# bayesml/BayesML

Hardware: AMD Instinct MI355X
Metric: GMM-VB E+M samples/sec at K=64,D=128,N=1e7; 1/2/4/8-GPU scaling (higher is better)
Workload: dtype f64; 1 GPU; GMM-VB K=64 D=128 N=10000000 rows/GPU x 1 GPU, x stored f32, one VB iteration per step (c3 of BASELINE.json configs); classes=64, degree=128, rows_per_gpu=10000000, rows_total=10000000, x_storage=f32, parallelism=rows1, row_tiles=1

## Files before the change

bayesml_amd/_engine.py:

```python
from __future__ import annotations

import ctypes
import os

import torch

_HERE = os.path.dirname(os.path.abspath(__file__))
LIB_PATH = os.environ.get("BAYESML_AMD_LIB") or os.path.join(_HERE, "csrc", "libgmmvb.so")

GMMVB_F32, GMMVB_F64 = 0, 1
POLICY_LEN = 16
_STATUS = {0: "GMMVB_OK", 1: "GMMVB_EINVAL", 2: "GMMVB_EUNSUPPORTED", 3: "GMMVB_EHIP", 4: "GMMVB_ENOMEM",
           5: "GMMVB_ESTATE"}

_vp, _i64, _int = ctypes.c_void_p, ctypes.c_int64, ctypes.c_int
SYMBOLS = {
    "gmmvb_abi_version": (_int, []),
    "gmmvb_last_error": (ctypes.c_char_p, []),
    "gmmvb_stats_len": (_i64, [_int, _int]),
    "gmmvb_workspace_create": (_int, [_int, _int, _int, _i64, ctypes.POINTER(_vp)]),
    "gmmvb_workspace_create_tile": (_int, [_vp, _i64, ctypes.POINTER(_vp)]),
    "gmmvb_workspace_destroy": (_int, [_vp]),
    "gmmvb_workspace_bytes": (_i64, [_vp]),
    "gmmvb_set_pivot": (_int, [_vp, _vp, _vp]),
    "gmmvb_set_params": (_int, [_vp, _vp, _vp, _vp, _vp]),
    "gmmvb_set_drift": (_int, [_vp, _vp, _vp, _vp, ctypes.c_double, _vp]),
    "gmmvb_forget": (_int, [_vp]),
    "gmmvb_regroup_count": (_i64, [_vp]),
    "gmmvb_debug_record": (_int, [_vp, _i64, ctypes.POINTER(ctypes.c_double)]),
    "gmmvb_debug_proof": (_int, [_vp, _int, _i64, _vp, _vp, _vp]),
    "gmmvb_wants_drift": (_int, [_vp, _i64]),
    "gmmvb_prepare_rows": (_int, [_vp, _vp, _i64, _i64, _vp]),
    "gmmvb_estep": (_int, [_vp, _vp, _i64, _i64, _vp]),
    "gmmvb_load_responsibilities": (_int, [_vp, _vp, _i64, _vp]),
    "gmmvb_mstep": (_int, [_vp, _vp, _i64, _i64, _vp, _vp]),
    "gmmvb_estep_mstep": (_int, [_vp, _vp, _i64, _i64, _vp, _vp]),
    "gmmvb_responsibilities": (_int, [_vp, _i64, _i64, _vp, _vp]),
    "gmmvb_ln_rho": (_int, [_vp, _i64, _i64, _vp, _vp]),
    "gmmvb_argmax": (_int, [_vp, _i64, _i64, _vp, _vp]),
    "gmmvb_last_launch_info": (ctypes.c_char_p, [_vp]),
    "gmmvb_pass_counts": (_int, [_vp, ctypes.POINTER(_i64)]),
    "gmmvb_kside_factor": (_int, [_int, _int, _vp, _vp, _vp, _vp, _vp]),
    "gmmvb_kside_step": (_int, [_int, _int, _vp, _vp, _vp, _vp, _vp, _vp, _vp, _vp, _vp, _int, _vp, _vp, _vp, _vp, _vp, _vp]),
    "gmmvb_kside_drift": (_int, [_int, _int, _vp, _vp, _vp, _vp, _vp, _vp, _int, _int, _vp, _vp, _vp, _vp, _vp]),
    "gmmvb_last_sparsity": (ctypes.c_int, [_vp, _vp, ctypes.POINTER(ctypes.c_double), ctypes.POINTER(ctypes.c_double)]),
    "gmmvb_last_work": (ctypes.c_int, [_vp, ctypes.POINTER(ctypes.c_double)]),
    "gmmvb_comm_unique_id": (_int, [_vp]),
    "gmmvb_comm_create": (_int, [_vp, _int, _int, ctypes.POINTER(_vp)]),
    "gmmvb_comm_destroy": (_int, [_vp]),
    "gmmvb_allreduce_stats": (_int, [_vp, _vp, _i64, _vp]),
    "gmmvb_stats_packed_len": (_i64, [_int, _int]),
    "gmmvb_stats_pack": (_int, [_int, _int, _vp, _vp, _vp]),
    "gmmvb_stats_unpack": (_int, [_int, _int, _vp, _vp, _vp]),
    "gmmvb_set_shard": (_int, [_vp, _i64, _int]),
    "gmmvb_policy_export": (_int, [_vp, _vp, _vp]),
    "gmmvb_policy_import": (_int, [_vp, _vp, _vp]),
    "gmmvb_small_supported": (_int, [_int, _int, _i64]),
    "gmmvb_small_out_len": (_i64, [_int, _int, _int]),
    "gmmvb_small_fit": (_int, [_int, _int, _int, _vp, _i64, _i64, _vp, _vp, _int, _int, _vp, _int, ctypes.c_double, _vp, _vp, _vp]),
    "hmmvb_kside_dirichlet": (_int, [_int, _vp, _vp, ctypes.c_double, ctypes.c_double] + [_vp] * 18),
    "hmmvb_out_len": (_i64, [_int]),
    "hmmvb_enable": (_int, [_vp]),
    "hmmvb_forward_backward": (_int, [_vp, _i64, _vp, _vp, _vp, _vp]),
    "hmmvb_debug_readout": (_int, [_vp, _int, _i64, _i64, _vp, _vp]),
    "hmmvb_readout": (_int, [_vp, _int, _i64, _i64, _vp, _vp, _vp]),
    "hmmvb_emission_target": (_int, [_vp, _int, _vp]),
    "hmmvb_skip_h": (_int, [_vp, _int]),
    "hmmvb_last_boundary_pass": (_int, [_vp]),
    "hmmvb_last_viterbi_pass": (_int, [_vp]),
    "hmmvb_viterbi": (_int, [_vp, _i64, _vp, _vp, _vp, _vp]),
    "gmmvb_profile_enable": (_int, [_vp, _int]),
    "gmmvb_profile_last_ms": (_int, [_vp, ctypes.POINTER(ctypes.c_float), ctypes.POINTER(ctypes.c_float)]),
    "gmmvb_profile_spans": (_int, [_vp, ctypes.POINTER(ctypes.c_float), ctypes.POINTER(_int)]),
    "gmmvb_profile_span_name": (ctypes.c_char_p, [_int]),
    "gmmvb_policy_calibrate": (_int, [_vp, _int]),
    "gmmvb_policy_table": (_int, [_vp, ctypes.POINTER(ctypes.c_double)]),
    "gmmvb_sample_latent": (_int, [_int, _vp, ctypes.c_uint64, _i64, _i64, _vp, _vp]),
    "gmmvb_sample_chain_work_bytes": (_i64, [_int, _i64]),
    "gmmvb_sample_chain": (_int, [_int, _vp, _vp, ctypes.c_uint64, _i64, _vp, _vp, _i64, _vp]),
    "gmmvb_sample_emissions_work_bytes": (_i64, [_int, _i64]),
    "gmmvb_sample_emissions": (_int, [_int, _int, _vp, _vp, _vp, ctypes.c_uint64, _i64, _i64, _int, _vp, _i64, _vp, _i64, _vp]),
}


class EngineUnavailableError(RuntimeError):
    """The HIP extension or the GPU is missing; the product path has no fallback."""


class EngineError(RuntimeError):
    """A C-ABI call returned a non-zero status."""


class EngineLimitError(ValueError):
    """The model's shape is outside what this version of the engine supports (the reference has no such limit)."""


MAX_MFMA_DEGREE = 128
MAX_HMM_FAST_CLASSES = 64
MAX_HMM_CLASSES = 16 * 255
MAX_DEGREE = 19200


def check_limits(c_degree: int, c_num_classes: int = 1, hmm: bool = False):
    if c_degree > MAX_DEGREE:
        raise EngineLimitError(f"bayesml_amd supports c_degree <= {MAX_DEGREE} in this version (got {c_degree}); "
                               "bayesml itself has no such limit")
    if hmm and c_num_classes > MAX_HMM_CLASSES:
        raise EngineLimitError(f"bayesml_amd.hiddenmarkovnormal supports c_num_classes <= {MAX_HMM_CLASSES} in this "
                               f"version (got {c_num_classes}); bayesml itself has no such limit")


_lib = None


def load_library(path: str = LIB_PATH) -> ctypes.CDLL:
    global _lib
    if _lib is not None and path == LIB_PATH:
        return _lib
    if not os.path.exists(path):
        raise EngineUnavailableError(
            f"{path} not found: build it with `python -c 'import __graft_entry__ as g; g.build()'` "
            "(or `make -C bayesml_amd/csrc`). bayesml_amd has no CPU fallback for the data pass.")
    lib = ctypes.CDLL(path)
    for name, (res, args) in SYMBOLS.items():
        fn = getattr(lib, name)
        fn.restype = res
        fn.argtypes = args
    if path == LIB_PATH:
        _lib = lib
    return lib


def _check(lib, rc, what):
    if rc != 0:
        msg = lib.gmmvb_last_error()
        raise EngineError(f"{what}: {_STATUS.get(rc, rc)}: {msg.decode() if msg else ''}")


def _f64(t: torch.Tensor, shape, device) -> torch.Tensor:
    t = torch.as_tensor(t, dtype=torch.float64, device=device).contiguous()
    if tuple(t.shape) != tuple(shape):
        raise ValueError(f"expected shape {tuple(shape)}, got {tuple(t.shape)}")
    return t


class RcclComm:

    def __init__(self, rank: int, world: int, device, bootstrap=None, group=None):
        self.lib = load_library()
        self.device = torch.device(device)
        buf = (ctypes.c_ubyte * 128)()
        if rank == 0:
            _check(self.lib, self.lib.gmmvb_comm_unique_id(buf), "gmmvb_comm_unique_id")
        if bootstrap is None:
            import torch.distributed as dist
            t = torch.tensor(list(buf), dtype=torch.uint8)
            if dist.get_backend(group) == "nccl":
                t = t.to(self.device)
            dist.broadcast(t, src=dist.get_global_rank(group, 0) if group is not None else 0, group=group)
            raw = bytes(t.cpu().tolist())
        else:
            raw = bootstrap(bytes(buf))
        buf = (ctypes.c_ubyte * 128).from_buffer_copy(raw)
        handle = _vp()
        with torch.cuda.device(self.device):
            _check(self.lib, self.lib.gmmvb_comm_create(buf, int(world), int(rank), ctypes.byref(handle)), "gmmvb_comm_create")
        self._comm = handle

    def all_reduce_(self, t: torch.Tensor) -> torch.Tensor:
        if t.dtype != torch.float64 or not t.is_contiguous() or t.device != self.device:
            raise ValueError("the statistics block must be a contiguous float64 tensor on the communicator's device")
        with torch.cuda.device(self.device):
            st = _vp(torch.cuda.current_stream(self.device).cuda_stream)
            _check(self.lib, self.lib.gmmvb_allreduce_stats(self._comm, t.data_ptr(), t.numel(), st), "gmmvb_allreduce_stats")
        return t

    def close(self):
        if getattr(self, "_comm", None):
            torch.cuda.synchronize(self.device)
            self.lib.gmmvb_comm_destroy(self._comm)
            self._comm = None

    def __del__(self):
# ... 109 lines not shown
                rc = self.lib.gmmvb_workspace_create_tile(tile_of._ws, self.max_rows, ctypes.byref(handle))
            else:
                rc = self.lib.gmmvb_workspace_create(self.K, self.D, GMMVB_F64 if x_dtype == torch.float64 else GMMVB_F32,
                                                     self.max_rows, ctypes.byref(handle))
        _check(self.lib, rc, "gmmvb_workspace_create_tile" if tile_of is not None else "gmmvb_workspace_create")
        self._ws = handle
        self.emission_fused = False
        self._keep = []

    def close(self):
        if getattr(self, "_ws", None):
            torch.cuda.synchronize(self.device)
            self.lib.gmmvb_workspace_destroy(self._ws)
            self._ws = None

    def __del__(self):
        try:
            self.close()
        except Exception:
            pass

    def _stream(self):
        return _vp(torch.cuda.current_stream(self.device).cuda_stream)

    def _x(self, x: torch.Tensor):
        if x.device != self.device or x.dtype != self.x_dtype or x.dim() != 2 or x.shape[1] != self.D:
            raise ValueError(f"x must be a [{'*'}, {self.D}] {self.x_dtype} tensor on {self.device}")
        if x.stride(1) != 1:
            x = x.contiguous()
        return x, int(x.stride(0)) if x.shape[0] > 1 else self.D

    @property
    def workspace_bytes(self) -> int:
        return int(self.lib.gmmvb_workspace_bytes(self._ws))

    @property
    def launch_info(self) -> str:
        s = self.lib.gmmvb_last_launch_info(self._ws)
        return s.decode() if s else ""

    PASS_NAMES = ("estep_dense", "estep_bound", "estep_carried", "estep_fell_back_dense", "estep_sweep",
                  "mstep_dense", "mstep_list", "estep_gather")

    def pass_counts(self) -> dict:
        out = (_i64 * 8)()
        _check(self.lib, self.lib.gmmvb_pass_counts(self._ws, out), "gmmvb_pass_counts")
        return dict(zip(self.PASS_NAMES, (int(v) for v in out)))

    def sparsity(self):
        a, e = ctypes.c_double(), ctypes.c_double()
        with torch.cuda.device(self.device):
            _check(self.lib, self.lib.gmmvb_last_sparsity(self._ws, self._stream(), ctypes.byref(a), ctypes.byref(e)),
                   "gmmvb_last_sparsity")
        return float(a.value), float(e.value)

    def work(self) -> dict:
        out = (ctypes.c_double * 8)()
        _check(self.lib, self.lib.gmmvb_last_work(self._ws, out), "gmmvb_last_work")
        tiles = (self.rows + 255) // 256 if getattr(self, "rows", 0) else 0
        share = float(out[6]) / (tiles * self.K) if out[6] >= 0 and tiles else -1.0
        return dict(active=float(out[0]), evaluated=float(out[1]), accumulated=float(out[2]), settled_rows=float(out[3]),
                    early_exits=float(out[4]), proof_pairs=float(out[5]), sweep_share=share, table_left=float(out[7]))

    def policy_table(self) -> dict:
        out = (ctypes.c_double * 16)()
        _check(self.lib, self.lib.gmmvb_policy_table(self._ws, out), "gmmvb_policy_table")
        keys = ("dense_e_ns", "dense_m_ns", "bound_ns", "exact_ns", "proof_ns", "list_m_ns", "literal_dense_e_ns",
                "literal_dense_m_ns", "literal_bound_ns", "prune_below", "dense_again_above", "list_m_below")
        d = {k: float(out[i]) for i, k in enumerate(keys)}
        d.update(measured=int(out[12]), discarded=int(out[13]), calibrating=bool(out[14]))
        return d

    def profile(self, on: bool = True):
        _check(self.lib, self.lib.gmmvb_profile_enable(self._ws, int(on)), "gmmvb_profile_enable")

    def last_kernel_ms(self):
        e, m = ctypes.c_float(), ctypes.c_float()
        _check(self.lib, self.lib.gmmvb_profile_last_ms(self._ws, ctypes.byref(e), ctypes.byref(m)),
               "gmmvb_profile_last_ms")
        return float(e.value), float(m.value)

    def kernel_spans(self) -> dict:
        ms, cnt = (ctypes.c_float * 8)(), (_int * 8)()
        _check(self.lib, self.lib.gmmvb_profile_spans(self._ws, ms, cnt), "gmmvb_profile_spans")
        out = {}
        for i in range(8):
            name = self.lib.gmmvb_profile_span_name(i).decode()
            if name and cnt[i]:
                out[name] = (float(ms[i]), int(cnt[i]))
        return out

    def set_pivot(self, pivot):
        p = _f64(pivot, (self.D,), self.device)
        with torch.cuda.device(self.device):
            _check(self.lib, self.lib.gmmvb_set_pivot(self._ws, p.data_ptr(), self._stream()), "gmmvb_set_pivot")
        self.pivot = p

    def prepare_rows(self, x: torch.Tensor):
        x, ldx = self._x(x)
        with torch.cuda.device(self.device):
            _check(self.lib, self.lib.gmmvb_prepare_rows(self._ws, x.data_ptr(), ldx, x.shape[0], self._stream()),
                   "gmmvb_prepare_rows")

    def set_params(self, c, m, u):
        c = _f64(c, (self.K,), self.device)
        m = _f64(m, (self.K, self.D), self.device)
        u = _f64(u, (self.K, self.D, self.D), self.device)
        with torch.cuda.device(self.device):
            _check(self.lib, self.lib.gmmvb_set_params(self._ws, c.data_ptr(), m.data_ptr(), u.data_ptr(),
                                                       self._stream()), "gmmvb_set_params")
        self._keep = [c, m, u]

    def set_shard(self, global_rows: int, n_ranks: int):
        _check(self.lib, self.lib.gmmvb_set_shard(self._ws, int(global_rows), int(n_ranks)), "gmmvb_set_shard")

    def policy_export(self, tail: torch.Tensor):
        with torch.cuda.device(self.device):
            _check(self.lib, self.lib.gmmvb_policy_export(self._ws, tail.data_ptr(), self._stream()), "gmmvb_policy_export")

    def policy_import(self, tail: torch.Tensor):
        with torch.cuda.device(self.device):
            _check(self.lib, self.lib.gmmvb_policy_import(self._ws, tail.data_ptr(), self._stream()), "gmmvb_policy_import")

    def wants_drift(self, n_rows: int) -> bool:
        return bool(self.lib.gmmvb_wants_drift(self._ws, int(n_rows)))

    def set_drift(self, gamma, delta, big_gamma, typical_gamma: float = -1.0):
        g = _f64(gamma, (self.K,), self.device)
        d = _f64(delta, (self.K,), self.device)
        G = _f64(big_gamma, (self.K,), self.device)
        with torch.cuda.device(self.device):
            _check(self.lib, self.lib.gmmvb_set_drift(self._ws, g.data_ptr(), d.data_ptr(), G.data_ptr(),
                                                      float(typical_gamma), self._stream()), "gmmvb_set_drift")

    @property
    def regroup_count(self) -> int:
        return int(self.lib.gmmvb_regroup_count(self._ws))

    def debug_record(self, row: int) -> dict:
        out = (ctypes.c_double * 26)()
        _check(self.lib, self.lib.gmmvb_debug_record(self._ws, int(row), out), "gmmvb_debug_record")
        v = list(out)
        return dict(k=[int(x) for x in v[:8]], d=[round(x, 3) for x in v[8:16]], B=v[16], exact=int(v[17]), sel=int(v[18]),
                    flags=int(v[19]), khat=int(v[20]), lse=v[21], masks=[int(x) for x in v[22:26]])

    def debug_proof(self, k: int, n_rows: int):
        ub = torch.empty(n_rows, dtype=torch.float32, device=self.device)
        lb = torch.empty(n_rows, dtype=torch.float64, device=self.device)
        with torch.cuda.device(self.device):
            _check(self.lib, self.lib.gmmvb_debug_proof(self._ws, int(k), int(n_rows), ub.data_ptr(), lb.data_ptr(),
                                                        self._stream()), "gmmvb_debug_proof")
        return ub, lb

    def forget(self):
        _check(self.lib, self.lib.gmmvb_forget(self._ws), "gmmvb_forget")

    def estep(self, x: torch.Tensor):
        x, ldx = self._x(x)
        with torch.cuda.device(self.device):
            _check(self.lib, self.lib.gmmvb_estep(self._ws, x.data_ptr(), ldx, x.shape[0], self._stream()),
                   "gmmvb_estep")
        self.rows = x.shape[0]

    def load_responsibilities(self, r: torch.Tensor):
        r = torch.as_tensor(r, dtype=torch.float64, device=self.device).contiguous()
        if r.dim() != 2 or r.shape[1] != self.K:
            raise ValueError("r must be [n, K]")
        with torch.cuda.device(self.device):
            _check(self.lib, self.lib.gmmvb_load_responsibilities(self._ws, r.data_ptr(), r.shape[0], self._stream()),
                   "gmmvb_load_responsibilities")
        self.rows = r.shape[0]
        self._keep.append(r)

    def _stats_out(self, out):
        if out is None:
            return torch.empty(self.stats_len, dtype=torch.float64, device=self.device)
        if out.dtype != torch.float64 or out.numel() != self.stats_len or not out.is_contiguous() or out.device != self.device:
            raise ValueError("out must be a contiguous float64 tensor of stats_len elements on the engine's device")
        return out

    def mstep(self, x: torch.Tensor, out: torch.Tensor = None) -> torch.Tensor:
        x, ldx = self._x(x)
        stats = self._stats_out(out)
        with torch.cuda.device(self.device):
            _check(self.lib, self.lib.gmmvb_mstep(self._ws, x.data_ptr(), ldx, x.shape[0], stats.data_ptr(),
                                                  self._stream()), "gmmvb_mstep")
        return stats

    def estep_mstep(self, x: torch.Tensor, out: torch.Tensor = None) -> torch.Tensor:
        x, ldx = self._x(x)
        stats = self._stats_out(out)
        with torch.cuda.device(self.device):
            _check(self.lib, self.lib.gmmvb_estep_mstep(self._ws, x.data_ptr(), ldx, x.shape[0], stats.data_ptr(),
                                                        self._stream()), "gmmvb_estep_mstep")
        self.rows = x.shape[0]
        return stats

    def enable_hmm(self):
        with torch.cuda.device(self.device):
            _check(self.lib, self.lib.hmmvb_enable(self._ws), "hmmvb_enable")

    def hmm_skip_h(self, skip: bool = True):
        _check(self.lib, self.lib.hmmvb_skip_h(self._ws, 1 if skip else 0), "hmmvb_skip_h")

    def last_boundary_pass(self) -> int:
        return int(self.lib.hmmvb_last_boundary_pass(self._ws))

    def last_viterbi_pass(self) -> int:
        return int(self.lib.hmmvb_last_viterbi_pass(self._ws))

    def emission_target(self, fused: bool) -> bool:
        eff = ctypes.c_int(0)
        _check(self.lib, self.lib.hmmvb_emission_target(self._ws, 1 if fused else 0, ctypes.byref(eff)),
               "hmmvb_emission_target")
        self.emission_fused = bool(eff.value)
        return self.emission_fused

    def forward_backward(self, pi_tilde, a_tilde, out: torch.Tensor = None):
        K = self.K
        pi = _f64(pi_tilde, (K,), self.device)
        a = _f64(a_tilde, (K, K), self.device)
        n_out = int(self.lib.hmmvb_out_len(K))
        if out is None:
            out = torch.empty(n_out, dtype=torch.float64, device=self.device)
        elif out.dtype != torch.float64 or out.numel() != n_out or not out.is_contiguous() or out.device != self.device:
            raise ValueError("out must be a contiguous float64 tensor of hmmvb_out_len(K) elements on the engine's device")
        with torch.cuda.device(self.device):
            _check(self.lib, self.lib.hmmvb_forward_backward(self._ws, self.rows, pi.data_ptr(), a.data_ptr(),
                                                             out.data_ptr(), self._stream()), "hmmvb_forward_backward")
        self._keep = self._keep[-3:] + [pi, a]
        return out[:K * K].view(K, K), out[K * K:K * K + K], out[K * K + K:K * K + 2 * K], out[K * K + 2 * K]

    def viterbi(self, ln_pi_tilde, ln_a_tilde) -> torch.Tensor:
        K = self.K
        pi = _f64(ln_pi_tilde, (K,), self.device)
        a = _f64(ln_a_tilde, (K, K), self.device)
        z = torch.empty(self.rows, dtype=torch.int32, device=self.device)
        with torch.cuda.device(self.device):
            _check(self.lib, self.lib.hmmvb_viterbi(self._ws, self.rows, pi.data_ptr(), a.data_ptr(), z.data_ptr(),
                                                    self._stream()), "hmmvb_viterbi")
        torch.cuda.current_stream(self.device).synchronize()
        return z

    def hmm_readout(self, what: str, row0=0, n=None, a_tilde=None) -> torch.Tensor:
        code = {"alpha": 0, "beta": 1, "xi": 3}[what]
        n = self.rows - row0 if n is None else n
        K = self.K
        out = torch.empty((n, K, K) if code == 3 else (n, K), dtype=torch.float64, device=self.device)
        a = _f64(a_tilde, (K, K), self.device) if code == 3 else None
        with torch.cuda.device(self.device):
            _check(self.lib, self.lib.hmmvb_readout(self._ws, code, row0, n, a.data_ptr() if a is not None else None,
                                                    out.data_ptr(), self._stream()), "hmmvb_readout")
        if a is not None:
            torch.cuda.current_stream(self.device).synchronize()
        return out

    def hmm_debug(self, what, row0=0, n=None):
        n = self.rows - row0 if n is None else n
        Kp = 16 * ((self.K + 15) // 16)
        out = torch.empty((n, Kp) if what == 0 else (n,), dtype=torch.float64, device=self.device)
        with torch.cuda.device(self.device):
            _check(self.lib, self.lib.hmmvb_debug_readout(self._ws, what, row0, n, out.data_ptr(), self._stream()),
                   "hmmvb_debug_readout")
        if what == 0:
            pos = [(s & ~15) + 4 * ((s & 15) & 3) + ((s & 15) >> 2) for s in range(self.K)]
            out = out[:, pos]
        return out

    def split_stats(self, stats: torch.Tensor):
        K, D = self.K, self.D
        return (stats[:K], stats[K:2 * K], stats[2 * K:2 * K + K * D].view(K, D),
                stats[2 * K + K * D:].view(K, D, D))

    def _readout(self, fn, name, row0, n, dtype=torch.float64, cols=None):
        n = self.rows - row0 if n is None else n
        out = torch.empty((n, self.K) if cols is None else (n,), dtype=dtype, device=self.device)
        with torch.cuda.device(self.device):
            _check(self.lib, fn(self._ws, row0, n, out.data_ptr(), self._stream()), name)
        return out

    def responsibilities(self, row0=0, n=None) -> torch.Tensor:
        return self._readout(self.lib.gmmvb_responsibilities, "gmmvb_responsibilities", row0, n)

    def ln_rho(self, row0=0, n=None) -> torch.Tensor:
        return self._readout(self.lib.gmmvb_ln_rho, "gmmvb_ln_rho", row0, n)

    def argmax(self, row0=0, n=None) -> torch.Tensor:
        return self._readout(self.lib.gmmvb_argmax, "gmmvb_argmax", row0, n, dtype=torch.int32, cols=1)


class TiledDataPass:

    def __init__(self, K, D, x_dtype, n_rows, device, tile_rows, resident=False):
        self.K, self.D, self.x_dtype, self.max_rows = int(K), int(D), x_dtype, int(n_rows)
        self.tile_rows = int(min(tile_rows, n_rows))
        self.n_tiles = (self.max_rows + self.tile_rows - 1) // self.tile_rows
        self.resident = bool(resident)
        self.inner = DataPass(K, D, x_dtype, self.tile_rows, device)
        self.tiles = [self.inner]
        self.device, self.lib, self.stats_len = self.inner.device, self.inner.lib, self.inner.stats_len
        try:
            if self.resident:
                for t in range(1, self.n_tiles):
                    lo, hi = self._tile(t)
                    self.tiles.append(DataPass(K, D, x_dtype, hi - lo, device, tile_of=self.inner))
            self._tmp = torch.zeros(self.stats_len, dtype=torch.float64, device=self.device)
# ... 302 lines not shown
```

bayesml_amd/csrc/aux_kernels.h:

```cpp
#pragma once
#include "common.h"
#include "rec_common.h"

namespace gmmvb {

static __device__ __forceinline__ void pack_f64_image(const double* uk, int ld, const double* mk, int D, int T, int img_len,
                                                      double* __restrict__ im) {
    const int P = tri_pairs(T);
    for (int e = threadIdx.x; e < P * 256; e += blockDim.x) {
        const int p = e >> 8, h = (e >> 7) & 1, lane = (e >> 1) & 63, ee = e & 1;
        int jt = 0;
        while (tri_pairs(jt + 1) <= p) ++jt;
        const int b = p - tri_pairs(jt);
        const int jj = 16 * jt + (lane & 15), ii = 16 * b + 4 * (lane >> 4) + 2 * h + ee;
        im[e] = (jj < D && ii < D && ii <= jj) ? uk[(int64_t)jj * ld + ii] : 0.0;
    }
    for (int jj = threadIdx.x; jj < 16 * T; jj += blockDim.x) {
        double s = 0.0;
        if (jj < D)
            for (int ii = 0; ii <= jj; ++ii) s = fma(uk[(int64_t)jj * ld + ii], mk[ii], s);
        const int jt = jj >> 4, w = jj & 15, g = w & 3, r = w >> 2;
        im[P * 256 + (jt * 4 + g) * 4 + r] = -s;
    }
    for (int e = P * 256 + 16 * T + threadIdx.x; e < img_len; e += blockDim.x) im[e] = 0.0;
// ... 10 lines not shown
    pack_f64_image(u + (int64_t)k * D * D, D, m + (int64_t)k * D, D, T, img_len, img + (int64_t)k * img_len);
}

template <typename XT>
__global__ void center_rows_kernel(const XT* __restrict__ x, int64_t ldx, int64_t n_rows, int64_t pad_rows, int D,
                                   int Dp, const double* __restrict__ pivot, double* __restrict__ xc) {
    const int64_t e = (int64_t)blockIdx.x * blockDim.x + threadIdx.x;
    if (e >= pad_rows * Dp) return;
    const int64_t n = e / Dp;
    const int f = (int)(e - n * Dp);
    xc[e] = (n < n_rows && f < D) ? (double)x[n * ldx + f] - pivot[f] : 0.0;
}

constexpr int kLseRows = 1024;
static __global__ __launch_bounds__(256) void row_lse_kernel(const double* __restrict__ lnrho, int64_t npad, int64_t n_rows,
                                                      int K, double* __restrict__ lse, double* __restrict__ dpart,
                                                      double* __restrict__ apart, int stride) {
    __shared__ double wmax[4];
    __shared__ int wcnt[4];
    int active = 0;
    const int64_t base = (int64_t)blockIdx.x * stride * kLseRows + threadIdx.x;
    double l[4];
#pragma unroll
    for (int q = 0; q < 4; ++q) {
        const int64_t n = base + 256 * q;
        l[q] = 0.0;
        if (n >= n_rows) continue;
        double mx = lnrho[n], s = 1.0;
        for (int k = 1; k < K; ++k) {
            const double v = lnrho[(int64_t)k * npad + n];
            if (v > mx) {
                s = fma(s, exp(mx - v), 1.0);
                mx = v;
            } else {
                s += exp(v - mx);
            }
        }
        l[q] = mx + log(s);
        lse[n] = l[q];
    }
    if (!dpart) return;
    const double ninf = -__builtin_huge_val();
    for (int k = 0; k < K; ++k) {
        double d = ninf;
#pragma unroll
        for (int q = 0; q < 4; ++q) {
            const int64_t n = base + 256 * q;
            if (n < n_rows) {
                const double v = lnrho[(int64_t)k * npad + n] - l[q];
                d = (v > d || v != v) ? v : d;
                active += !(v < -kRelevanceNats);
            }
        }
#pragma unroll
        for (int o = 32; o > 0; o >>= 1) {
            const double v = __shfl_xor(d, o);
            d = (v > d || v != v) ? v : d;
        }
        if ((threadIdx.x & 63) == 0) wmax[threadIdx.x >> 6] = d;
        __syncthreads();
        if (threadIdx.x == 0) {
#pragma unroll
            for (int w = 1; w < 4; ++w) d = (wmax[w] > d || wmax[w] != wmax[w]) ? wmax[w] : d;
            dpart[(int64_t)blockIdx.x * K + k] = d;
        }
        __syncthreads();
    }
#pragma unroll
    for (int o = 32; o > 0; o >>= 1) active += __shfl_xor(active, o);
    if ((threadIdx.x & 63) == 0) wcnt[threadIdx.x >> 6] = active;
    __syncthreads();
    if (threadIdx.x == 0 && apart) apart[blockIdx.x] = (double)(wcnt[0] + wcnt[1] + wcnt[2] + wcnt[3]);
}

static __global__ __launch_bounds__(256) void thr_kernel(const double* __restrict__ dpart, const double* __restrict__ apart,
                                                  int blocks, int K, double* __restrict__ thr,
                                                  double* __restrict__ act_total) {
    __shared__ double part[256];
    const int k = blockIdx.x;
    if (k == K) {
        if (!apart) return;
        double a = 0.0;
        for (int b = threadIdx.x; b < blocks; b += 256) a += apart[b];
        part[threadIdx.x] = a;
        __syncthreads();
        if (threadIdx.x == 0) {
            double t = 0.0;
            for (int i = 0; i < 256; ++i) t += part[i];
            *act_total = t;
        }
        return;
    }
    if (!dpart) return;
    double d = -__builtin_huge_val();
    for (int b = threadIdx.x; b < blocks; b += 256) {
        const double v = dpart[(int64_t)b * K + k];
        d = (v > d || v != v) ? v : d;
    }
    part[threadIdx.x] = d;
    __syncthreads();
    if (threadIdx.x == 0) {
        for (int i = 1; i < 256; ++i) d = (part[i] > d || part[i] != part[i]) ? part[i] : d;
        thr[k] = d - kRelevanceNats;
    }
}

template <int MODE>
__global__ __launch_bounds__(kSelRows) void select_mask_kernel(const double* __restrict__ u, int64_t npad, int64_t n_rows,
                                                               int K, int* __restrict__ khat,
                                                               unsigned long long* __restrict__ masks ,
                                                               int* __restrict__ blk_cnt ) {
    static_assert(MODE == 0 || MODE == 3, "only the best-component modes exist");
    __shared__ int wcnt[4][256];
    const int64_t n = (int64_t)blockIdx.x * kSelRows + threadIdx.x;
    const bool valid = n < n_rows;
    const int W = (K + 63) / 64;
    const int wave = threadIdx.x >> 6;
    for (int k = threadIdx.x & 63; k < K; k += 64) wcnt[wave][k] = 0;
    int kh = -1;
    if (MODE == 3 && valid) kh = khat[n];
    if (MODE == 0) {
        int arg = 0;
        if (valid) {
            double best = u[n];
            for (int k = 1; k < K; ++k) {
                const double v = u[(int64_t)k * npad + n];
                const bool up = v > best;
                best = up ? v : best;
                arg = up ? k : arg;
            }
            khat[n] = arg;
        }
        kh = arg;
    }
    for (int w = 0; w < W; ++w) {
        unsigned long long mk = 0;
        if (valid) {
            if ((kh >> 6) == w) mk = 1ull << (kh & 63);
            masks[(int64_t)w * npad + n] = mk;
        }
        unsigned long long present = wave_or(mk);
        while (present) {
            const int b = __builtin_ctzll(present);
            present &= present - 1;
            const int c = __builtin_popcountll(__ballot((mk >> b) & 1ull));
            if ((threadIdx.x & 63) == 0) wcnt[wave][64 * w + b] = c;
        }
    }
    __syncthreads();
    for (int k = threadIdx.x; k < K; k += kSelRows)
        blk_cnt[blk_at(k, blockIdx.x, K)] = wcnt[0][k] + wcnt[1][k] + wcnt[2][k] + wcnt[3][k];
}

constexpr int kScanParts = 1024;
constexpr int kScanChunk = 32;

static __global__ __launch_bounds__(256) void scan_parts_kernel(const int* __restrict__ blk, int blocks, int K, int* __restrict__ parts) {
    __shared__ int sh[256];
    const int p = blockIdx.x;
    const int R = K <= 256 ? 256 / K : 1;
    const int t = threadIdx.x, k = t % K, r = t / K;
    const int per = (blocks + kScanParts - 1) / kScanParts;
    const int b0 = p * per, b1 = b0 + per < blocks ? b0 + per : blocks;
    int s = 0;
    if (t < R * K)
        for (int b = b0 + r; b < b1; b += R) s += blk[blk_at(k, b, K)];
    sh[t] = s;
    __syncthreads();
    if (t < K) {
        int tot = 0;
        for (int q = 0; q < R; ++q) tot += sh[q * K + t];
        parts[p * K + t] = tot;
    }
}

static __global__ __launch_bounds__(256) void scan_mid_kernel(int* __restrict__ parts, int K, int* __restrict__ counts) {
    static_assert(kScanParts == 32 * kScanChunk, "256 threads = 8 components x 32 chunks");
    __shared__ int sh[32][8];
    const int t = threadIdx.x, kk = t & 7, c = t >> 3;
    const int k = blockIdx.x * 8 + kk;
    int v[kScanChunk];
    int s = 0;
#pragma unroll
    for (int i = 0; i < kScanChunk; ++i) {
        v[i] = k < K ? parts[(int64_t)(c * kScanChunk + i) * K + k] : 0;
        s += v[i];
    }
    sh[c][kk] = s;
    __syncthreads();
    int run = 0;
    for (int q = 0; q < c; ++q) run += sh[q][kk];
    if (k < K) {
#pragma unroll
        for (int i = 0; i < kScanChunk; ++i) {
            parts[(int64_t)(c * kScanChunk + i) * K + k] = run;
            run += v[i];
        }
        if (c == 31) counts[k] = run;
    }
}

static __global__ __launch_bounds__(256) void scan_apply_kernel(int* __restrict__ blk, int blocks, int K, const int* __restrict__ parts) {
    __shared__ int sh[256];
    const int p = blockIdx.x;
    const int R = K <= 256 ? 256 / K : 1;
    const int t = threadIdx.x, k = t % K, r = t / K;
    const bool on = t < R * K;
    const int per = (blocks + kScanParts - 1) / kScanParts;
    const int b0 = p * per, b1 = b0 + per < blocks ? b0 + per : blocks;
    int run = on ? parts[p * K + k] : 0;
    if (R == 1) {
        for (int c0 = b0; c0 < b1; c0 += 8) {
            int v[8];
#pragma unroll
            for (int i = 0; i < 8; ++i) v[i] = (on && c0 + i < b1) ? blk[blk_at(k, c0 + i, K)] : 0;
#pragma unroll
            for (int i = 0; i < 8; ++i) {
                if (on && c0 + i < b1) blk[blk_at(k, c0 + i, K)] = run;
                run += v[i];
            }
        }
        return;
    }
    for (int c0 = b0; c0 < b1; c0 += R) {
        const int b = c0 + r;
        const int v = (on && b < b1) ? blk[blk_at(k, b, K)] : 0;
        __syncthreads();
        sh[t] = v;
        __syncthreads();
        if (on) {
            int before = 0, all = 0;
            for (int q = 0; q < R; ++q) {
                const int w = sh[q * K + k];
                before += q < r ? w : 0;
                all += w;
            }
            if (b < b1) blk[blk_at(k, b, K)] = run + before;
            run += all;
        }
    }
}

inline void launch_scan_counts(hipStream_t st, int* blk, int blocks, int K, int* counts, int* parts ) {
    hipLaunchKernelGGL(scan_parts_kernel, dim3(kScanParts), dim3(256), 0, st, blk, blocks, K, parts);
    hipLaunchKernelGGL(scan_mid_kernel, dim3((K + 7) / 8), dim3(256), 0, st, parts, K, counts);
    hipLaunchKernelGGL(scan_apply_kernel, dim3(kScanParts), dim3(256), 0, st, blk, blocks, K, parts);
}

static __global__ __launch_bounds__(kSelRows) void fill_lists_kernel(const unsigned long long* __restrict__ masks, int64_t npad,
                                                              int64_t n_rows, int K, const int* __restrict__ blk_base,
                                                              int* __restrict__ lists, int64_t cap,
                                                              unsigned char* __restrict__ lock = nullptr,
                                                              const unsigned char* __restrict__ lcomp = nullptr,
                                                              const double* __restrict__ block_total = nullptr
                                                              ) {
    if (block_total != nullptr && block_total[blockIdx.x] == 0.0) return;
    __shared__ int wcnt[4][256];
    const int64_t n = (int64_t)blockIdx.x * kSelRows + threadIdx.x;
    const bool valid = n < n_rows;
    const int W = (K + 63) / 64;
    const int wave = threadIdx.x >> 6, lane = threadIdx.x & 63;
    for (int k = lane; k < K; k += 64) wcnt[wave][k] = 0;
    const int base_pre = (int)threadIdx.x < K ? blk_base[blk_at((int)threadIdx.x, blockIdx.x, K)] : 0;
    unsigned long long mkw[4] = {0ull, 0ull, 0ull, 0ull}, prw[4] = {0ull, 0ull, 0ull, 0ull};
#pragma unroll
    for (int w = 0; w < 4; ++w) {
        if (w >= W) break;
        const unsigned long long mk = valid ? masks[(int64_t)w * npad + n] : 0ull;
        mkw[w] = mk;
        unsigned long long present = wave_or(mk);
        prw[w] = present;
        while (present) {
            const int b = __builtin_ctzll(present);
            present &= present - 1;
            const int c = __builtin_popcountll(__ballot((mk >> b) & 1ull));
            if (lane == 0) wcnt[wave][64 * w + b] = c;
        }
    }
    __syncthreads();
    for (int k = threadIdx.x; k < K; k += kSelRows) {
        const int c0 = wcnt[0][k], c1 = wcnt[1][k], c2 = wcnt[2][k], c3 = wcnt[3][k];
        if (c0 + c1 + c2 + c3 > 0) {
            const int base = k == (int)threadIdx.x ? base_pre : blk_base[blk_at(k, blockIdx.x, K)];
            wcnt[0][k] = base;
            wcnt[1][k] = base + c0;
            wcnt[2][k] = base + c0 + c1;
            wcnt[3][k] = base + c0 + c1 + c2;
        }
    }
    __syncthreads();
    const unsigned lk0 = (lock && valid) ? lock[n] : 0u;
    const int kh0 = (lock && valid) ? (int)lcomp[n] : 0;
    if (lk0 >= 2u) lock[n] = lk0 == 2u ? 0 : 1;
#pragma unroll
    for (int w = 0; w < 4; ++w) {
        if (w >= W) break;
        const unsigned long long mk = mkw[w];
        unsigned long long present = prw[w];
        while (present) {
            const int b = __builtin_ctzll(present);
            present &= present - 1;
            const int k = 64 * w + b;
            const unsigned long long bal = __ballot((mk >> b) & 1ull);
            const int off = wcnt[wave][k];
            if ((mk >> b) & 1ull) {
                int entry = (int)n;
                if (lock) {
                    const bool leaves = lk0 == 2u || (lk0 == 4u && kh0 != k);
                    entry = leaves ? (int)((unsigned)entry | 0x80000000u) : entry;
                }
                lists[(int64_t)k * cap + off + __builtin_popcountll(bal & ((1ull << lane) - 1ull))] = entry;
            }
        }
    }
}

static __global__ __launch_bounds__(kSelRows) void lse_mask_kernel(const double* __restrict__ lnrho, int64_t npad, int64_t n_rows,
                                                            int K, const double* __restrict__ thr, double* __restrict__ lse,
                                                            unsigned long long* __restrict__ masks,
                                                            int* __restrict__ blk_cnt, double* __restrict__ apart,
                                                            int* __restrict__ khat ) {
    __shared__ int wcnt[4][256];
    __shared__ int wact[4];
    const int64_t n = (int64_t)blockIdx.x * kSelRows + threadIdx.x;
    const bool valid = n < n_rows;
    const int W = (K + 63) / 64;
    const int wave = threadIdx.x >> 6;
    for (int k = threadIdx.x & 63; k < K; k += 64) wcnt[wave][k] = 0;
    double l = 0.0;
    if (valid) {
        double mx = lnrho[n], s = 1.0;
        int arg = 0;
        for (int k = 1; k < K; ++k) {
            const double v = lnrho[(int64_t)k * npad + n];
            if (v > mx) {
                s = fma(s, exp(mx - v), 1.0);
                mx = v;
                arg = k;
            } else {
                s += exp(v - mx);
            }
        }
        l = mx + log(s);
        lse[n] = l;
        if (khat) khat[n] = arg;
    }
    int active = 0;
    for (int w = 0; w < W; ++w) {
        unsigned long long mk = 0;
        if (valid) {
            const int kend = K - 64 * w < 64 ? K - 64 * w : 64;
            for (int b = 0; b < kend; ++b) {
                const double t = lnrho[(int64_t)(64 * w + b) * npad + n] - l;
                mk |= (unsigned long long)(!(t < thr[64 * w + b])) << b;
                active += !(t < -kRelevanceNats);
            }
            masks[(int64_t)w * npad + n] = mk;
        }
        unsigned long long present = wave_or(mk);
        while (present) {
            const int b = __builtin_ctzll(present);
            present &= present - 1;
            const int c = __builtin_popcountll(__ballot((mk >> b) & 1ull));
            if ((threadIdx.x & 63) == 0) wcnt[wave][64 * w + b] = c;
        }
    }
#pragma unroll
    for (int o = 32; o > 0; o >>= 1) active += __shfl_xor(active, o);
    if ((threadIdx.x & 63) == 0) wact[wave] = active;
    __syncthreads();
    for (int k = threadIdx.x; k < K; k += kSelRows)
        blk_cnt[blk_at(k, blockIdx.x, K)] = wcnt[0][k] + wcnt[1][k] + wcnt[2][k] + wcnt[3][k];
    if (threadIdx.x == 0) apart[blockIdx.x] = (double)(wact[0] + wact[1] + wact[2] + wact[3]);
}

static __global__ void load_r_kernel(const double* __restrict__ r, int64_t n_rows, int K, double* __restrict__ buf,
                              int64_t npad, double* __restrict__ lse, const int* __restrict__ iperm) {
    const int64_t n = (int64_t)blockIdx.x * blockDim.x + threadIdx.x;
    if (n >= n_rows) return;
    const int64_t m = iperm ? iperm[n] : n;
    for (int k = 0; k < K; ++k) buf[(int64_t)k * npad + m] = r[n * K + k];
    lse[m] = 0.0;
}

static __global__ void readout_kernel(const double* __restrict__ buf, const double* __restrict__ lse, int64_t npad,
                               int64_t row0, int64_t n_rows, int K, int mode, int direct_r,
                               double* __restrict__ out, const int* __restrict__ iperm) {
    const int64_t e = (int64_t)blockIdx.x * blockDim.x + threadIdx.x;
    if (e >= n_rows * K) return;
    const int64_t n = e / K;
    const int k = (int)(e - n * K);
    const int64_t m = iperm ? iperm[row0 + n] : row0 + n;
    const double v = buf[(int64_t)k * npad + m];
    out[e] = (mode == 0 || direct_r) ? v : exp(v - lse[m]);
}

static __global__ void gather_int_kernel(const int* __restrict__ src, int64_t row0, int64_t n_rows, const int* __restrict__ iperm,
                                  int32_t* __restrict__ z) {
    const int64_t n = (int64_t)blockIdx.x * blockDim.x + threadIdx.x;
    if (n < n_rows) z[n] = src[iperm ? iperm[row0 + n] : row0 + n];
}

static __global__ void argmax_kernel(const double* __restrict__ buf, int64_t npad, int64_t row0, int64_t n_rows, int K,
                              int32_t* __restrict__ z, const int* __restrict__ iperm) {
    const int64_t n = (int64_t)blockIdx.x * blockDim.x + threadIdx.x;
    if (n >= n_rows) return;
    const int64_t m = iperm ? iperm[row0 + n] : row0 + n;
    double best = buf[m];
    int arg = 0;
    for (int k = 1; k < K; ++k) {
        const double v = buf[(int64_t)k * npad + m];
        if (v > best) {
            best = v;
            arg = k;
        }
    }
    z[n] = arg;
}

static __global__ void reduce_stats_kernel(const double* __restrict__ slabs, int S, int K, int D, int T,
                                    double* __restrict__ stats) {
    const int k = blockIdx.y;
    const int e = blockIdx.x * blockDim.x + threadIdx.x;
    const int P = tri_pairs(T);
    const int L = slab_len(T);
    if (e >= P * 256 + 16 * T + 2) return;
    double v = 0.0;
    int s = 0;
    for (; s + 16 <= S; s += 16) {
        double t[16];
#pragma unroll
        for (int u = 0; u < 16; ++u) t[u] = slabs[((int64_t)(s + u) * K + k) * L + e];
#pragma unroll
        for (int u = 0; u < 16; ++u) v += t[u];
    }
    for (; s < S; ++s) v += slabs[((int64_t)s * K + k) * L + e];
    double* ns = stats;
    double* h = stats + K;
    double* a = stats + 2 * (int64_t)K;
    double* B = a + (int64_t)K * D;
    if (e < P * 256) {
        const int p = e >> 8, r = (e >> 6) & 3, lane = e & 63;
        int t2 = 0;
        while (tri_pairs(t2 + 1) <= p) ++t2;
        const int t1 = p - tri_pairs(t2);
        const int col = lane & 15, row = (lane >> 4) + 4 * r;
        const int f1 = T * row + t1, f2 = T * col + t2;
        if (f1 >= D || f2 >= D) return;
        if (t1 == t2 && row > col) return;
        B[((int64_t)k * D + f1) * D + f2] = v;
        B[((int64_t)k * D + f2) * D + f1] = v;
    } else if (e < P * 256 + 16 * T) {
        const int f = e - P * 256;
        if (f < D) a[(int64_t)k * D + f] = v;
    } else if (e == P * 256 + 16 * T) {
        ns[k] = v;
    } else {
        h[k] = v;
    }
}

static __global__ void reduce_chunks_kernel(const double* __restrict__ slabs, const int* __restrict__ plan, int K, int D, int T,
                                     double* __restrict__ stats, int accumulate = 0, const double* __restrict__ add = nullptr,
                                     const int* __restrict__ counts = nullptr, int runs = 0) {
// ... 140 lines not shown
```

bayesml_amd/csrc/capi.hip:

```cpp
#include "capi_internal.h"

namespace {
thread_local std::string g_err;
}

namespace gmmvb {
int fail(int code, const char* what, hipError_t e) {
    g_err = what;
    if (e != hipSuccess) {
        g_err += ": ";
        g_err += hipGetErrorString(e);
    }
    return code;
}
}

namespace {
KernelSizes kernel_sizes(int K, int D) {
    KernelSizes ks;
    ks.max_tiles = kMaxTiles;
    ks.t1_splits = GMMVB_T1_SPLITS;
    ks.sel_rows = kSelRows;
    ks.lse_rows = kLseRows;
    ks.scan_parts = kScanParts;
// ... 153 lines not shown
            hipError_t rc = hipEventCreate(&e);
            if (rc != hipSuccess) return fail(GMMVB_EHIP, "hipEventCreate", rc);
        }
        for (auto& e : ws->span_ev) {
            hipError_t rc = hipEventCreate(&e);
            if (rc != hipSuccess) return fail(GMMVB_EHIP, "hipEventCreate", rc);
        }
    }
    ws->prof = on != 0;
    ws->prof_light = on == 2;
    ws->span_open = false;
    ws->ev_e = ws->ev_m = false;
    ws->n_spans = 0;
    return GMMVB_OK;
}

const char* gmmvb_profile_span_name(int slot) { return (slot >= 0 && slot < kSpanSlots) ? kSpanNames[slot] : ""; }

int gmmvb_profile_spans(gmmvb_workspace* ws, float* ms , int* launches ) {
    if (!ws || !ms || !launches) return fail(GMMVB_EINVAL, "null argument");
    for (int i = 0; i < kSpanSlots; ++i) {
        ms[i] = 0.0f;
        launches[i] = 0;
    }
    for (int i = 0; i < ws->n_spans; ++i) {
        float t = 0.0f;
        hipError_t rc = hipEventSynchronize(ws->span_ev[2 * i + 1]);
        if (rc == hipSuccess) rc = hipEventElapsedTime(&t, ws->span_ev[2 * i], ws->span_ev[2 * i + 1]);
        if (rc != hipSuccess) return fail(GMMVB_EHIP, "event timing (span)", rc);
        ms[ws->span_slot[i]] += t;
        ++launches[ws->span_slot[i]];
    }
    return GMMVB_OK;
}

int gmmvb_profile_last_ms(gmmvb_workspace* ws, float* estep_ms, float* mstep_ms) {
    if (!ws || !estep_ms || !mstep_ms) return fail(GMMVB_EINVAL, "null argument");
    *estep_ms = *mstep_ms = -1.0f;
    if (ws->ev_e) {
        hipError_t rc = hipEventSynchronize(ws->ev[1]);
        if (rc == hipSuccess) rc = hipEventElapsedTime(estep_ms, ws->ev[0], ws->ev[1]);
        if (rc != hipSuccess) return fail(GMMVB_EHIP, "event timing (estep)", rc);
    }
    if (ws->ev_m) {
        hipError_t rc = hipEventSynchronize(ws->ev[3]);
        if (rc == hipSuccess) rc = hipEventElapsedTime(mstep_ms, ws->ev[2], ws->ev[3]);
        if (rc != hipSuccess) return fail(GMMVB_EHIP, "event timing (mstep)", rc);
    }
    return GMMVB_OK;
}

int gmmvb_set_pivot(gmmvb_workspace* ws, const double* pivot_dev, void* stream) {
    if (!ws || !pivot_dev) return fail(GMMVB_EINVAL, "null argument");
    hipError_t e = hipMemcpyAsync(ws->pivot, pivot_dev, (size_t)ws->D * sizeof(double), hipMemcpyDeviceToDevice,
                                  (hipStream_t)stream);
    if (e != hipSuccess) return fail(GMMVB_EHIP, "hipMemcpyAsync(pivot)", e);
    ws->xc_src = nullptr;
    ws->xq_src = nullptr;
    ++ws->pivot_gen;
    drop_settled_rows(ws);
    return GMMVB_OK;
}

int gmmvb_wants_drift(const gmmvb_workspace* ws, int64_t n_rows) {
    if (!ws || ws->prune == 0 || ws->estep_variant != kEstepLds8 || ws->hmm != nullptr || !ws->rec_k) return 0;
    if (ws->opt_carry_off) return 0;
    if (ws->sharded) n_rows = ws->shard_rows / ws->shard_ranks;
    return (ws->prune == 2 || n_rows * (int64_t)ws->K >= (int64_t(1) << 23)) ? 1 : 0;
}

namespace {
__global__ void set_drift_kernel(const double* __restrict__ gamma, const double* __restrict__ delta, const double* __restrict__ big_gamma,
                                 const double* __restrict__ cvec, int K, double* __restrict__ drift) {
    const int k = blockIdx.x * blockDim.x + threadIdx.x;
    if (k >= K) return;
    drift[k] = gamma[k];
    drift[K + k] = delta[k];
    drift[2 * K + k] = cvec[k];
    drift[3 * K + k] = big_gamma[k];
}
}

int gmmvb_set_drift(gmmvb_workspace* ws, const double* gamma_dev, const double* delta_dev, const double* big_gamma_dev,
                    double typical_gamma, void* stream) {
    if (!ws || !gamma_dev || !delta_dev || !big_gamma_dev) return fail(GMMVB_EINVAL, "null argument");
    ws->typical_gamma = typical_gamma;
    hipStream_t st = (hipStream_t)stream;
    hipLaunchKernelGGL(set_drift_kernel, dim3((unsigned)((ws->K + 255) / 256)), dim3(256), 0, st, gamma_dev, delta_dev, big_gamma_dev,
                       ws->cvec, ws->K, ws->drift);
    const hipError_t e = hipGetLastError();
    if (e != hipSuccess) return fail(GMMVB_EHIP, "set_drift_kernel", e);
    ws->have_drift = ws->have_params && ws->params_used;
    return GMMVB_OK;
}

int gmmvb_debug_record(gmmvb_workspace* ws, int64_t row, double* out ) {
    if (!ws || !out || !ws->rec_k || row < 0 || row >= ws->npad) return fail(GMMVB_EINVAL, "bad argument");
    hipError_t e = hipDeviceSynchronize();
    auto get = [&e](void* dst, const void* src, size_t n) {
        if (e == hipSuccess) e = hipMemcpy(dst, src, n, hipMemcpyDeviceToHost);
    };
    for (int j = 0; j < kRecSlots; ++j) {
        unsigned short k = 0;
        float d = 0.0f;
        get(&k, ws->rec_k + (int64_t)j * ws->npad + row, sizeof(k));
        get(&d, ws->rec_d + (int64_t)j * ws->npad + row, sizeof(d));
        out[j] = k == kRecEmpty ? -1.0 : (double)k;
        out[8 + j] = d;
    }
    float B = 0.0f;
    unsigned char ex = 0, sel = 0, fl = 0;
    int kh = 0;
    get(&B, ws->rec_B + row, sizeof(B));
    get(&ex, ws->rec_exact + row, 1);
    get(&sel, ws->rec_sel + row, 1);
    get(&fl, ws->rec_flags + row, 1);
    get(&kh, ws->khat + row, sizeof(kh));
    get(out + 21, ws->lse + row, sizeof(double));
    out[16] = B;
    out[17] = ex;
    out[18] = sel;
    out[19] = fl;
    out[20] = kh;
    for (int w = 0; w < 4; ++w) {
        unsigned long long m = 0;
        if (w < (ws->K + 63) / 64) get(&m, ws->masks + (int64_t)w * ws->npad + row, sizeof(m));
        out[22 + w] = (double)m;
    }
    if (e != hipSuccess) return fail(GMMVB_EHIP, "reading a record back", e);
    return GMMVB_OK;
}

int64_t gmmvb_regroup_count(const gmmvb_workspace* ws) { return ws ? ws->sorts : -1; }

namespace {
__global__ void debug_all_rows_kernel(int* __restrict__ list, int* __restrict__ counts, int K, int k, int64_t n_rows) {
    const int64_t i = (int64_t)blockIdx.x * blockDim.x + threadIdx.x;
    if (i < n_rows) list[i] = (int)i;
    if (i < K) counts[i] = (int)(i == k ? n_rows : 0);
}
}

int gmmvb_debug_proof(gmmvb_workspace* ws, int k, int64_t n_rows, float* ub_dev, double* lb_dev, void* stream) {
    if (!ws || !ub_dev || !lb_dev || k < 0 || k >= ws->K) return fail(GMMVB_EINVAL, "bad argument");
    if (!ws->xq || !ws->img_i8b || ws->xq_src == nullptr || ws->xq_rows != n_rows || ws->xq_gen != ws->img_gen || !ws->have_params)
        return fail(GMMVB_ESTATE, "no digit planes for these rows: gmmvb_set_pivot, gmmvb_prepare_rows, gmmvb_set_params first");
    claim_scratch(ws);
    hipStream_t st = (hipStream_t)stream;
    ws->tmeta_valid = false;
    drop_settled_rows(ws);
    const unsigned grid = (unsigned)((std::max<int64_t>(n_rows, ws->K) + 255) / 256);
    hipLaunchKernelGGL(debug_all_rows_kernel, dim3(grid), dim3(256), 0, st, ws->lists + (int64_t)k * ws->npad, ws->counts, ws->K, k,
                       n_rows);
    hipLaunchKernelGGL(gather_plan_kernel, dim3(1), dim3(64), 0, st, ws->counts, ws->K, estep_i8_pairs_per_chunk(), ws->plan);
    hipError_t e = launch_estep_i8_proof(ws->D, ws->num_cu, st, ws->xq, ws->xqe, ws->img_i8b, ws->cvec, ws->K, ws->lists, ws->npad,
                                         ws->counts, ws->plan, ws->ub32, ws->lnrho, ws->npad);
    if (e == hipSuccess) e = hipMemcpyAsync(ub_dev, ws->ub32 + (int64_t)k * ws->npad, (size_t)n_rows * sizeof(float),
                                            hipMemcpyDeviceToDevice, st);
    if (e == hipSuccess) e = hipMemcpyAsync(lb_dev, ws->lnrho + (int64_t)k * ws->npad, (size_t)n_rows * sizeof(double),
                                            hipMemcpyDeviceToDevice, st);
    if (e != hipSuccess) return fail(GMMVB_EHIP, "proof kernel (diagnostic)", e);
    ws->e_state = 0;
    ws->lost_estep = false;
    ws->bounds_rows = 0;
    ws->rec_valid = ws->dense_valid = ws->rec_live = false;
    ws->active_lists = ws->blk_fresh = false;
    ws->lag.valid = false;
    return GMMVB_OK;
}

int gmmvb_forget(gmmvb_workspace* ws) {
    if (!ws) return fail(GMMVB_EINVAL, "null argument");
    ws->forget = true;
    ws->have_drift = false;
    drop_settled_rows(ws);
    return GMMVB_OK;
}

int gmmvb_set_params(gmmvb_workspace* ws, const double* c_dev, const double* m_dev, const double* u_dev,
                     void* stream) {
    if (!ws || !c_dev || !m_dev || !u_dev) return fail(GMMVB_EINVAL, "null argument");
    hipStream_t st = (hipStream_t)stream;
    hipError_t e = hipSuccess;
    if (ws->generic) {
        e = hipMemcpyAsync(ws->cvec, c_dev, (size_t)ws->K * sizeof(double), hipMemcpyDeviceToDevice, st);
        if (e != hipSuccess) return fail(GMMVB_EHIP, "hipMemcpyAsync(c)", e);
        e = hipMemcpyAsync(ws->gen_m, m_dev, (size_t)ws->K * ws->D * sizeof(double), hipMemcpyDeviceToDevice, st);
        if (e == hipSuccess)
            e = hipMemcpyAsync(ws->gen_u, u_dev, (size_t)ws->K * ws->D * ws->D * sizeof(double), hipMemcpyDeviceToDevice, st);
        if (e != hipSuccess) return fail(GMMVB_EHIP, "hipMemcpyAsync(m, u)", e);
        ws->have_params = true;
        ws->params_used = false;
        return GMMVB_OK;
    }
    if (ws->wide) {
        if (ws->pivot_i8) return fail(GMMVB_EUNSUPPORTED, "gmmvb_set_params: int8 images past D = 128");
        hipLaunchKernelGGL(pack_params_kernel, dim3(ws->K), dim3(256), 0, st, u_dev, m_dev, ws->K, ws->D, ws->T, ws->img_len, ws->img,
                           c_dev, ws->cvec, nullptr, nullptr);
        e = hipGetLastError();
        if (e != hipSuccess) return fail(GMMVB_EHIP, "pack_params_kernel", e);
    } else {
        e = launch_pack_images(u_dev, m_dev, c_dev, ws->pivot, ws->K, ws->D, ws->T, ws->img_len, ws->img, ws->cvec, ws->pivot_i8,
                               ws->pivot_i8 ? ws->img_i8 : nullptr, ws->pivot_i8 ? ws->img_i8b : nullptr, st);
        if (e != hipSuccess) return fail(GMMVB_EHIP, "pack_images_kernel", e);
        if (ws->pivot_i8) ws->img_gen = ws->pivot_gen;
    }
    if (ws->tri) {
        e = launch_pack_tri16(u_dev, m_dev, ws->K, ws->D, ws->tri, st);
        if (e != hipSuccess) return fail(GMMVB_EHIP, "pack_tri16_kernel", e);
    }
    ws->proj_table = false;
    if (ws->gimg && ws->opt_project != 0 && ws->sorted && ws->tile_ref_valid && ws->have_drift && ws->xq_gen == ws->pivot_gen &&
        !ws->opt_carry_off) {
        e = launch_proj_table(u_dev, m_dev, c_dev, ws->pivot, ws->K, ws->D, ws->gimg, ws->gconst, st);
        if (e != hipSuccess) return fail(GMMVB_EHIP, "proj_table_kernel", e);
        ws->proj_table = true;
    }
    ws->have_params = true;
    ws->params_used = false;
    return GMMVB_OK;
}

int fetch_counters(gmmvb_workspace* ws) {
    if (ws->ctr_pending) {
        hipError_t e = hipEventSynchronize(ws->ctr_ev);
        if (e != hipSuccess) return fail(GMMVB_EHIP, "waiting for the E-step counters", e);
        ws->lag.act = ws->ctr_host[0];
        if (ws->pend_mode == 0) {
            ws->lag.eval = (double)ws->pend_rows * ws->K;
            ws->lag.over = 0.0;
            ws->lag.settled = 0.0;
            ws->lag.listed = ws->lag.accum = ws->lag.act;
            ws->lag.exits = 0.0;
            ws->lag.cols = -1.0;
            ws->lag.left = -1.0;
            ws->lag_quiet = ws->lag_skipped = -1.0;
            ws->lag.proof = 0.0;
            ws->lag.moved = 0.0;
        } else {
            ws->lag.proof = ws->ctr_host[7];
            ws->lag.exits = (ws->exit_host && ws->gather_exit) ? (double)ws->exit_host[0] : 0.0;
            ws->lag.cols = (ws->exit_host && ws->pend_lazy) ? (double)ws->exit_host[1] : -1.0;
            ws->lag.left = (ws->exit_host && ws->pend_proj) ? (double)ws->exit_host[2] : -1.0;
            ws->lag_quiet = (ws->exit_host && ws->pend_quiet) ? (double)(ws->exit_host[3] & 0xFFFFFFFFull) : -1.0;
            ws->lag_skipped = (ws->exit_host && ws->pend_quiet) ? (double)(ws->exit_host[3] >> 32) : -1.0;
            ws->lag.settled = ws->ctr_host[4];
            ws->lag.listed = ws->ctr_host[5];
            ws->lag.accum = ws->ctr_host[6];
            ws->lag.eval = ws->ctr_host[1] + ((ws->pend_mode == 1 || ws->pend_mode == 3) ? ws->pend_round0 : 0.0);
            ws->lag.over = ws->ctr_host[2];
            ws->lag.moved = ws->ctr_host[3];
            if (!ws->sharded && ws->sorted && !ws->pend_first_sorted) ws->moved_since_sort += ws->lag.moved;
        }
        ws->lag.rows = (double)ws->pend_rows;
        ws->lag.mode = ws->pend_mode;
        ws->lag.valid = true;
        ws->ctr_pending = false;
    }
    return GMMVB_OK;
}

void poll_counters(gmmvb_workspace* ws) {
    if (ws->ctr_pending && hipEventQuery(ws->ctr_ev) == hipSuccess) (void)fetch_counters(ws);
}

namespace {
__global__ void policy_export_kernel(const double* __restrict__ ctr, const unsigned long long* __restrict__ exits, int mode,
                                     double rows, int K, double round0, int counted, int use_exits, double* __restrict__ out) {
    if (threadIdx.x != 0 || blockIdx.x != 0) return;
    const bool dense = mode == 0;
    const double act = counted ? ctr[0] : 0.0;
    out[0] = act;
    out[1] = dense ? rows * K : ctr[1] + ((mode == 1 || mode == 3) ? round0 : 0.0);
    out[2] = dense ? 0.0 : ctr[2];
    out[3] = dense ? 0.0 : ctr[3];
    out[4] = dense ? 0.0 : ctr[4];
    out[5] = dense ? act : ctr[5];
    out[6] = dense ? act : ctr[6];
    out[7] = dense ? 0.0 : ctr[7];
    out[8] = (dense || !use_exits || !exits) ? 0.0 : (double)*exits;
    out[9] = rows;
    out[10] = 1.0;
    out[11] = counted ? 1.0 : 0.0;
    out[12] = (double)mode;
    for (int i = 13; i < GMMVB_POLICY_LEN; ++i) out[i] = 0.0;
}
}

int gmmvb_set_shard(gmmvb_workspace* ws, int64_t global_rows, int n_ranks) {
    if (!ws || global_rows < 1 || n_ranks < 1) return fail(GMMVB_EINVAL, "bad argument");
    ws->sharded = n_ranks > 1;
    ws->shard_rows = global_rows;
    ws->shard_ranks = n_ranks;
    ws->pol.valid = false;
    if (ws->sharded && !ws->pol_host) {
        hipError_t e = hipHostMalloc((void**)&ws->pol_host, GMMVB_POLICY_LEN * sizeof(double), hipHostMallocDefault);
        if (e == hipSuccess) e = hipEventCreateWithFlags(&ws->pol_ev, hipEventDisableTiming);
        if (e != hipSuccess) return fail(GMMVB_EHIP, "policy buffers", e);
    }
    return GMMVB_OK;
}

int gmmvb_policy_export(gmmvb_workspace* ws, double* out_dev, void* stream) {
    if (!ws || !out_dev) return fail(GMMVB_EINVAL, "null argument");
    if (ws->e_state != 1) return fail(GMMVB_ESTATE, "no E-step output in the workspace");
    hipLaunchKernelGGL(policy_export_kernel, dim3(1), dim3(64), 0, (hipStream_t)stream, ws->ctr, ws->exit_ctr, ws->prev_pass,
                       (double)ws->e_rows, ws->K, ws->pend_round0, ws->exp_counted ? 1 : 0, ws->gather_exit ? 1 : 0, out_dev);
    hipError_t e = hipGetLastError();
    if (e != hipSuccess) return fail(GMMVB_EHIP, "policy export", e);
    return GMMVB_OK;
}

int gmmvb_policy_import(gmmvb_workspace* ws, const double* in_dev, void* stream) {
    if (!ws || !in_dev) return fail(GMMVB_EINVAL, "null argument");
    if (!ws->sharded) return GMMVB_OK;
    hipStream_t st = (hipStream_t)stream;
    hipError_t e = hipMemcpyAsync(ws->pol_host, in_dev, GMMVB_POLICY_LEN * sizeof(double), hipMemcpyDeviceToHost, st);
    if (e == hipSuccess) e = hipEventRecord(ws->pol_ev, st);
    if (e != hipSuccess) return fail(GMMVB_EHIP, "policy import", e);
    ws->pol_pending = true;
    ws->pol_mode = ws->prev_pass;
// ... 148 lines not shown
```

bayesml_amd/csrc/capi_estep.hip:

```cpp
#include "capi_internal.h"

namespace {

struct Pass {
    gmmvb_workspace* ws;
    const void* x_dev;
    int64_t ldx, n_rows;
    hipStream_t st;
    int is64;
    bool vec;
    int sel_grid;
    double pairs;
    EstepArgs a{};
    EstepI8Args a8{};
    RecArrays rec{};
    bool i8 = false;
    bool prunable = false;
    bool prev_lists = false, can_project = false, own_known = false, tmeta_was_valid = false;
    bool quiet_was_valid = false;
    int mode = kPassDense;
    bool settle = false, proof_capable = false;
    double skip_margin = -1.0;
    bool counted = false, proof_ran = false, tmeta_kept = false, projected = false, filtered = false, emission_to_hmm = false,
         sorted_now = false;
    bool quiet_swept = false;
    bool phase_closed = false;
    const char* name = "";
    int rpw = 0;
    int64_t grid = 0;

    PassFacts facts();
    int apply(const PassFacts& f, const PassPlan& plan);
    int run_generic();
    int run_dense();
    int run_bound();
    int run_sweep();
    int run_sweep_over_lists();
    int run_sweep_from_best();
    int sweep_bounds(bool proof, bool own_round);
    int run_candidates();
    int finish(const char* latch_what);
};

hipError_t regroup_rows(gmmvb_workspace* ws, const void* x_dev, int64_t ldx, int64_t n_rows, hipStream_t st, bool keep_state,
                        bool margin_ok) {
    const int sel_grid = (int)((n_rows + kSelRows - 1) / kSelRows);
    const unsigned cgrid = (unsigned)((n_rows + 255) / 256);
    const int* key = ws->khat;
    const int* perm_in = ws->sorted ? ws->perm : nullptr;
    const bool by_margin = ws->opt_regroup_margin && margin_ok && ws->K >= kMarginBuckets;
    if (by_margin) {
        int* bucket = ws->perm_tmp;
        hipLaunchKernelGGL(margin_bucket_kernel, dim3(cgrid), dim3(256), 0, st, ws->lnrho, ws->npad, n_rows, ws->lse, ws->khat,
                           keep_state ? ws->lock : nullptr, bucket);
        hipLaunchKernelGGL(select_mask_kernel<3>, dim3(sel_grid), dim3(kSelRows), 0, st, ws->lnrho, ws->npad, n_rows,
                           kMarginBuckets, bucket, ws->masks, ws->blk);
        scan_and_fill(ws, st, ws->masks, ws->blk, sel_grid, n_rows, kMarginBuckets);
        int* key1 = reinterpret_cast<int*>(ws->rec_d);
        hipLaunchKernelGGL(perm_compose_kernel, dim3(cgrid, kMarginBuckets), dim3(256), 0, st, ws->lists, ws->npad, ws->counts,
                           ws->khat, key1);
        hipLaunchKernelGGL(perm_compose_kernel, dim3(cgrid, kMarginBuckets), dim3(256), 0, st, ws->lists, ws->npad, ws->counts,
                           perm_in, ws->perm_tmp);
        key = key1;
        perm_in = ws->perm_tmp;
    }
    hipLaunchKernelGGL(select_mask_kernel<3>, dim3(sel_grid), dim3(kSelRows), 0, st, ws->lnrho, ws->npad, n_rows, ws->K,
                       const_cast<int*>(key), ws->masks, ws->blk);
    scan_and_fill(ws, st, ws->masks, ws->blk, sel_grid, n_rows, ws->K);
    ws->tile_ref_valid = false;
    if (ws->tile_ref) {
        if (launch_proj_tile_ref(ws->counts, ws->K, sel_grid, ws->tile_ref, st) == hipSuccess) ws->tile_ref_valid = true;
    }
    if (by_margin) {
        hipLaunchKernelGGL(perm_compose_kernel, dim3(cgrid, ws->K), dim3(256), 0, st, ws->lists, ws->npad, ws->counts, perm_in,
                           ws->khat);
        int* new_perm = ws->khat;
        ws->khat = ws->perm_tmp;
        ws->perm_tmp = ws->perm;
        ws->perm = new_perm;
    } else {
        hipLaunchKernelGGL(perm_compose_kernel, dim3(cgrid, ws->K), dim3(256), 0, st, ws->lists, ws->npad, ws->counts, perm_in,
                           ws->perm_tmp);
        std::swap(ws->perm, ws->perm_tmp);
    }
    if (keep_state) {
        hipLaunchKernelGGL(regroup_state_kernel, dim3((unsigned)((n_rows + 255) / 256)), dim3(256), 0, st, ws->perm,
                           ws->sorted ? ws->iperm : nullptr, n_rows, ws->lock, ws->lcomp, ws->dlock, ws->rec_sel, ws->rec_flags,
                           ws->rthr);
        std::swap(ws->lock, ws->rec_sel);
        std::swap(ws->lcomp, ws->rec_flags);
        std::swap(ws->dlock, ws->rthr);
    }
    hipLaunchKernelGGL(perm_invert_kernel, dim3((unsigned)((n_rows + 255) / 256)), dim3(256), 0, st, ws->perm, n_rows, ws->iperm);
    const int64_t total = n_rows * ws->D;
    const unsigned pg = (unsigned)((total + 255) / 256);
    const int64_t esz = ws->x_dtype == GMMVB_F64 ? 8 : 4;
    if ((ws->D * esz) % 16 == 0 && (ldx * esz) % 16 == 0 && (uintptr_t)x_dev % 16 == 0) {
        const int p16 = (int)(ws->D * esz / 16);
        hipLaunchKernelGGL(permute_rows16_kernel, dim3((unsigned)((n_rows * p16 + 255) / 256)), dim3(256), 0, st,
                           (const uint4*)x_dev, ldx * esz / 16, n_rows, p16, ws->perm, (uint4*)ws->xp);
    } else if (ws->x_dtype == GMMVB_F64)
        hipLaunchKernelGGL(permute_rows_kernel<double>, dim3(pg), dim3(256), 0, st, (const double*)x_dev, ldx, n_rows, ws->D,
                           ws->perm, (double*)ws->xp);
    else
        hipLaunchKernelGGL(permute_rows_kernel<float>, dim3(pg), dim3(256), 0, st, (const float*)x_dev, ldx, n_rows, ws->D,
                           ws->perm, (float*)ws->xp);
    ws->xc_stale = ws->xc != nullptr;
    if (ws->xq && ws->xq_src == x_dev) {
        hipError_t eq = launch_x_digits(ws->xp, ws->x_dtype == GMMVB_F64, ws->D, n_rows, ws->D, ws->pivot, ws->xq, ws->xqe, st);
        if (eq != hipSuccess) return eq;
        ws->xq_gen = ws->pivot_gen;
    }
    ws->sorted = true;
    ++ws->sorts;
    return hipGetLastError();
}

hipError_t launch_bound_pass(gmmvb_workspace* ws, const EstepI8Args& a8, int is64, bool vec, hipStream_t st,
                             const char** name, int* rpw_out, int64_t* grid_out) {
    const int rpw = estep_i8_rows_per_wg();
    int64_t grid = (a8.n_rows + rpw - 1) / rpw;
    if (grid > (1 << 20)) grid = 1 << 20;
    *rpw_out = rpw;
    *grid_out = grid;
    EstepI8Args ab = a8;
    ab.img = ws->img_i8b;
    ab.khat = ws->khat;
    ab.ub = ws->ub32;
    return launch_estep_i8_bound(is64, vec, ws->bound.tb, (int)grid, st, ab, name);
}

hipError_t lists_and_gather(gmmvb_workspace* ws, const EstepArgs& a, int is64, bool vec, int sel_grid, hipStream_t st,
                            const float* thr = nullptr, const double* block_total = nullptr ) {
    if (thr) {
        hipError_t em = hipMemsetAsync(ws->exit_ctr, 0, sizeof(unsigned long long), st);
        if (em != hipSuccess) return em;
    }
    span_begin(ws, kSpanSelect, st);
    scan_and_fill(ws, st, ws->masks, ws->blk, sel_grid, a.n_rows, ws->K, block_total);
    hipLaunchKernelGGL(gather_plan_kernel, dim3(1), dim3(64), 0, st, ws->counts, ws->K,
                       estep_gather_rows_per_wg(ws->T, is64), ws->plan);
    hipError_t e = hipGetLastError();
    span_end(ws, st);
    if (e != hipSuccess) return e;
    span_begin(ws, kSpanGather, st);
    e = launch_estep_gather_dev(ws->T, is64, vec, 2 * ws->num_cu, st, a, ws->lists, ws->npad, ws->counts, ws->plan, thr,
                                thr ? ws->exit_ctr : nullptr, 0.0f);
    span_end(ws, st);
    ++ws->passes[7];
    return e;
}

}

extern "C" {


bool cal_wanted(gmmvb_workspace* ws, int what, double pairs) {
    return ws->opt_calibrate && ws->cal_ev[0] != nullptr && !((ws->pt.measured >> what) & 1) && ws->cal_pairs[what] == 0.0 &&
           pairs >= (double)(int64_t(1) << 23) && ws->hmm == nullptr;
}
void cal_mark(gmmvb_workspace* ws, int what, double pairs, hipStream_t st) {
    note_hip(ws, hipEventRecord(ws->cal_ev[2 * what + 1], st));
    ws->cal_pairs[what] = pairs;
}
void cal_poll(gmmvb_workspace* ws) {
    for (int what = 0; what < 3; ++what) {
        if (ws->cal_pairs[what] <= 0.0 || hipEventQuery(ws->cal_ev[2 * what + 1]) != hipSuccess) continue;
        float ms = 0.0f;
        if (hipEventElapsedTime(&ms, ws->cal_ev[2 * what], ws->cal_ev[2 * what + 1]) == hipSuccess) {
            double ns = (double)ms * 1e6 / ws->cal_pairs[what];
            if (what == 2) ns += 0.010 * tri_pairs(ws->T) / 36.0;
            const bool took = ws->pt.take(what, ns);
            if (ws->opt_debug)
                std::fprintf(stderr, "[gmmvb] policy table: %s %.4f ns per pair %s (prune below %.3f, dense again above %.3f, list M below %.3f)\n",
                             what == 0 ? "dense E" : (what == 1 ? "dense M" : "bound pass"), ns, took ? "taken" : "out of range: literal kept",
                             ws->pt.prune_below(), ws->pt.dense_again_above(), ws->pt.list_m_below());
            if (!took) ws->pt.measured |= 8 << what;
            ws->cal_pairs[what] = (took || ++ws->cal_tries[what] >= 3) ? -1.0 : 0.0;
        } else {
            ws->cal_pairs[what] = -1.0;
        }
    }
}

}

namespace {

hipError_t proof_round(gmmvb_workspace* ws, hipStream_t st, const int* blk_base, int sel_grid, int64_t n_rows, float* ub) {
    if (ws->opt_proof_blocked && ws->slabs &&
        estep_i8_proof_work_bytes(ws->K, n_rows) <= ws->scratch->bytes[kBuf_slabs])
        return launch_estep_i8_proof_blocked(ws->D, ws->num_cu, st, ws->xq, ws->xqe, ws->img_i8b, ws->cvec, ws->K, ws->lists,
                                             ws->npad, ws->counts, blk_base, sel_grid, ws->slabs, ub, ws->lnrho, ws->npad);
    hipLaunchKernelGGL(gather_plan_kernel, dim3(1), dim3(64), 0, st, ws->counts, ws->K, estep_i8_pairs_per_chunk(), ws->plan);
    return launch_estep_i8_proof(ws->D, ws->num_cu, st, ws->xq, ws->xqe, ws->img_i8b, ws->cvec, ws->K, ws->lists, ws->npad,
                                 ws->counts, ws->plan, ub, ws->lnrho, ws->npad);
}

int Pass::run_generic() {
    const int R = generic_rows(ws->D);
    const dim3 g((unsigned)((n_rows + R - 1) / R), (unsigned)ws->K);
    const size_t lds = (size_t)ws->D * R * sizeof(double);
    span_begin(ws, kSpanEstepMain, st);
    if (is64)
        hipLaunchKernelGGL(estep_generic_kernel<double>, g, dim3(64), lds, st, (const double*)x_dev, ldx, n_rows, ws->D,
                           ws->gen_u, ws->gen_m, ws->cvec, R, ws->lnrho, ws->npad);
    else
        hipLaunchKernelGGL(estep_generic_kernel<float>, g, dim3(64), lds, st, (const float*)x_dev, ldx, n_rows, ws->D,
                           ws->gen_u, ws->gen_m, ws->cvec, R, ws->lnrho, ws->npad);
    span_end(ws, st);
    if (phase_events(ws)) {
        note_hip(ws, hipEventRecord(ws->ev[1], st));
        ws->ev_e = true;
    }
    phase_closed = true;
    span_begin(ws, kSpanLse, st);
    hipLaunchKernelGGL(row_lse_kernel, dim3((unsigned)((n_rows + kLseRows - 1) / kLseRows)), dim3(256), 0, st, ws->lnrho,
                       ws->npad, n_rows, ws->K, ws->lse, nullptr, nullptr, 1);
    span_end(ws, st);
    hipError_t eg = hipGetLastError();
    if (eg != hipSuccess) return fail(GMMVB_EHIP, "estep_generic launch", eg);
    ++ws->passes[0];
    ws->rec_live = ws->rec_valid = false;
    ws->evaluated = pairs;
    std::snprintf(ws->info, sizeof(ws->info), "estep_generic_f64<D=%d> grid=%ux%ux64 rows/workgroup=%d", ws->D, g.x, g.y, R);
    name = nullptr;
    return GMMVB_OK;
}

int Pass::run_dense() {
    const bool valu16 = ws->estep_variant == kEstepValu16 && ws->tri != nullptr;
    emission_to_hmm = ws->T == 1 && !ws->wide && !i8 && !ws->sorted && hmm_fused_emission(ws->hmm);
    rpw = ws->wide ? estep_rows_rows_per_wg()
                     : (i8 ? estep_i8_rows_per_wg() : (valu16 ? estep_rows16_rows_per_wg() : estep_rows_per_wg(ws->estep_variant, ws->T, is64)));
    grid = (n_rows + rpw - 1) / rpw;
    if (grid > (1 << 20)) grid = 1 << 20;
    span_begin(ws, kSpanEstepMain, st);
    const bool cal_e = !ws->wide && !i8 && !emission_to_hmm && !valu16 && cal_wanted(ws, 0, pairs);
    if (cal_e) note_hip(ws, hipEventRecord(ws->cal_ev[0], st));
    hipError_t e = ws->wide ? launch_estep_rows(ws->T, is64, (int)grid, st, a, &name)
                            : (i8 ? launch_estep_i8(is64, vec, (int)grid, st, a8, &name)
                                  : (emission_to_hmm ? hmm_launch_emission16(ws->hmm, is64, vec, st, a, &name)
                                     : (valu16 ? launch_estep_rows16(is64, vec, (int)grid, st, a, ws->tri, &name)
                                            : launch_estep(ws->estep_variant, ws->T, is64, vec, (int)grid, st, a, &name))));
    if (cal_e) cal_mark(ws, 0, pairs, st);
    span_end(ws, st);
    if (e != hipSuccess) return fail(GMMVB_EHIP, "estep launch", e);
    ++ws->passes[0];
    const int lse_blocks = (int)((n_rows + kLseRows - 1) / kLseRows);
    const bool count_pairs = ws->sparse && ws->masks && ws->hmm == nullptr && n_rows * (int64_t)ws->K >= (int64_t(1) << 18);
    span_begin(ws, kSpanLse, st);
    if (count_pairs) {
        const int stride = lse_blocks >= 64 ? 16 : 1;
        const int sampled = (lse_blocks + stride - 1) / stride;
        hipLaunchKernelGGL(row_lse_kernel, dim3((unsigned)sampled), dim3(256), 0, st, ws->lnrho, ws->npad, n_rows, ws->K,
                           ws->lse, ws->dpart, nullptr, stride);
        hipLaunchKernelGGL(thr_kernel, dim3((unsigned)ws->K), dim3(256), 0, st, ws->dpart, nullptr, sampled, ws->K, ws->thr,
                           ws->ctr);
        hipLaunchKernelGGL(lse_mask_kernel, dim3((unsigned)sel_grid), dim3(kSelRows), 0, st, ws->lnrho, ws->npad, n_rows,
                           ws->K, ws->thr, ws->lse, ws->masks, ws->blk, ws->apart, ws->khat);
        hipLaunchKernelGGL(sum_parts_kernel, dim3(1), dim3(1024), 0, st, ws->apart, nullptr, nullptr, nullptr, nullptr, nullptr,
                           nullptr, nullptr, sel_grid, ws->ctr);
        if (prunable)
            hipLaunchKernelGGL(rec_build_kernel<false>, dim3((unsigned)((n_rows + 255) / 256)), dim3(256), 0, st, ws->lnrho,
                               ws->npad, n_rows, ws->K, ws->cvec, nullptr, rec, ws->ub32);
        e = hipGetLastError();
        if (e != hipSuccess) return fail(GMMVB_EHIP, "row_lse / lse_mask launch", e);
        counted = true;
        ws->rec_valid = prunable;
    } else if (ws->hmm != nullptr) {
        ws->lse_stale = true;
        ws->rec_valid = false;
    } else {
        hipLaunchKernelGGL(row_lse_kernel, dim3((unsigned)lse_blocks), dim3(256), 0, st, ws->lnrho, ws->npad, n_rows, ws->K,
                           ws->lse, nullptr, nullptr, 1);
        e = hipGetLastError();
        if (e != hipSuccess) return fail(GMMVB_EHIP, "row_lse launch", e);
        ws->rec_valid = false;
    }
    span_end(ws, st);
    ws->rec_live = false;
    ws->evaluated = pairs;
    return GMMVB_OK;
}

int Pass::run_bound() {
    span_begin(ws, kSpanEstepMain, st);
    const bool cal_b = ws->bound.tb == (ws->D + 31) / 32 && cal_wanted(ws, 2, pairs);
    if (cal_b) note_hip(ws, hipEventRecord(ws->cal_ev[4], st));
    hipError_t e = launch_bound_pass(ws, a8, is64, vec, st, &name, &rpw, &grid);
    if (cal_b) cal_mark(ws, 2, pairs, st);
    span_end(ws, st);
    if (e != hipSuccess) return fail(GMMVB_EHIP, "estep_bound launch", e);
    ++ws->passes[1];
    span_begin(ws, kSpanSelect, st);
    hipLaunchKernelGGL(select_mask_kernel<3>, dim3(sel_grid), dim3(kSelRows), 0, st, ws->lnrho, ws->npad, n_rows, ws->K, ws->khat,
                       ws->masks, ws->blk);
    span_end(ws, st);
    e = lists_and_gather(ws, a, is64, vec, sel_grid, st);
    if (e != hipSuccess) return fail(GMMVB_EHIP, "E-step best-component evaluation", e);
    span_begin(ws, kSpanSelect, st);
    hipLaunchKernelGGL(rec_build_kernel<true>, dim3((unsigned)((n_rows + 255) / 256)), dim3(256), 0, st, ws->lnrho, ws->npad,
                       n_rows, ws->K, ws->cvec, ws->khat, rec, ws->ub32);
    hipLaunchKernelGGL(rec_select_kernel, dim3(sel_grid), dim3(kSelRows), 0, st, rec, n_rows, ws->K, ws->cvec, ws->masks,
                       ws->npad, ws->blk, ws->epart, ws->opart, ws->rthr);
    if (proof_capable) {
        scan_and_fill(ws, st, ws->masks, ws->blk, sel_grid, n_rows, ws->K, ws->epart);
        span_end(ws, st);
        span_begin(ws, kSpanProof, st);
        e = proof_round(ws, st, ws->blk, sel_grid, n_rows, ws->ub32);
        span_end(ws, st);
        if (e != hipSuccess) return fail(GMMVB_EHIP, "proof round (bound pass)", e);
        span_begin(ws, kSpanSelect, st);
        hipLaunchKernelGGL(rec_prune_kernel, dim3(sel_grid), dim3(kSelRows), 0, st, rec, ws->masks, ws->npad, n_rows, ws->K,
                           ws->cvec, ws->ub32, ws->rthr, ws->blk, ws->epart, ws->ppart);
        proof_ran = true;
    }
    span_end(ws, st);
    return GMMVB_OK;
}

int Pass::sweep_bounds(bool proof, bool own_round) {
    unsigned char* lock = settle ? ws->lock : nullptr;
    unsigned long long* pmask = proof ? ws->rmask : nullptr;
    const int proof_all = ws->opt_proof_all ? 1 : 0, own_fresh = own_round ? 1 : 0;
    int* tile_loose = can_project ? nullptr : ws->tile_loose();
    unsigned long long* quiet_ctr = (tile_loose && ws->opt_debug) ? ws->exit_ctr + 3 : nullptr;
    if (quiet_ctr) note_hip(ws, hipMemsetAsync(quiet_ctr, 0, sizeof(unsigned long long), st));
    if (can_project && ws->opt_project == 2) {
        note_hip(ws, hipMemsetAsync(ws->exit_ctr + 2, 0, sizeof(unsigned long long), st));
        hipError_t e = launch_rec_project(sel_grid, st, project_args(ws, n_rows, lock, pmask, proof_all, own_fresh));
        if (e != hipSuccess) return fail(GMMVB_EHIP, "rec_project launch", e);
        name = "estep_sweep_projected";
        projected = true;
    } else if (ws->tmeta) {
        note_hip(ws, hipMemsetAsync(ws->exit_ctr + 1, 0, sizeof(unsigned long long), st));
        const int run = sweep_run_length(ws->K, ws->opt_sweep_run);
        dispatch_mask_words(ws->K, [&](auto wc) {
            dispatch_sweep_run(run, [&](auto rr) {
                constexpr int WC = decltype(wc)::value, R = WC <= 2 ? decltype(rr)::value : 1;
                hipLaunchKernelGGL((rec_sweep_kernel<true, true, WC, R>), dim3((sel_grid + R - 1) / R), dim3(kSelRows), 0, st,
                                   ws->ub32, ws->lnrho, ws->npad, n_rows, ws->K, ws->drift, ws->cvec, ws->khat, rec, ws->masks,
                                   ws->blk, ws->epart, ws->opart, lock, ws->dlock, ws->rthr, ws->lcomp, pmask, ws->rblk, proof_all,
                                   own_fresh, ws->tmeta, tmeta_was_valid ? 0 : 1, ws->exit_ctr + 1, ws->ppart, tile_loose, quiet_ctr);
            });
        });
        tmeta_kept = true;
        quiet_swept = tile_loose != nullptr;
    } else {
        hipLaunchKernelGGL(rec_sweep_kernel<true>, dim3(sel_grid), dim3(kSelRows), 0, st, ws->ub32, ws->lnrho, ws->npad, n_rows,
                           ws->K, ws->drift, ws->cvec, ws->khat, rec, ws->masks, ws->blk, ws->epart, ws->opart, lock, ws->dlock,
                           ws->rthr, ws->lcomp, pmask, ws->rblk, proof_all, own_fresh, nullptr, 0, nullptr, ws->ppart, tile_loose,
                           quiet_ctr);
        quiet_swept = tile_loose != nullptr;
    }
    return GMMVB_OK;
}

int Pass::run_sweep_over_lists() {
    span_begin(ws, kSpanSelect, st);
    if (!ws->active_lists)
        scan_and_fill(ws, st, ws->masks, ws->blk, sel_grid, n_rows, ws->K, ws->prev_pass != 0 ? ws->gpart : nullptr);
    hipLaunchKernelGGL(gather_plan_kernel, dim3(1), dim3(64), 0, st, ws->counts, ws->K, estep_gather_rows_per_wg(ws->T, is64),
                       ws->plan);
    span_end(ws, st);
    span_begin(ws, kSpanGather, st);
    hipError_t e = launch_estep_gather_dev(ws->T, is64, vec, 2 * ws->num_cu, st, a, ws->lists, ws->npad, ws->counts, ws->plan);
    span_end(ws, st);
    ++ws->passes[7];
    if (e != hipSuccess) return fail(GMMVB_EHIP, "E-step active-pair evaluation", e);
    const bool proof = proof_capable && (ws->skip_used || ws->opt_proof_all);
    const bool own_round = proof && ws->skip_used && !(ws->typical_gamma >= ws->pt.own_round_below);
    if (own_round) {
        span_begin(ws, kSpanSelect, st);
        hipLaunchKernelGGL(settled_mask_kernel, dim3(sel_grid), dim3(kSelRows), 0, st, ws->lock, ws->masks, ws->lcomp, ws->npad,
                           n_rows, ws->K, ws->rmask, ws->rblk, ws->drift, ws->spart, quiet_was_valid ? ws->tile_quiet() : nullptr);
        scan_and_fill(ws, st, ws->rmask, ws->rblk, sel_grid, n_rows, ws->K, ws->spart);
        span_end(ws, st);
        span_begin(ws, kSpanProof, st);
        e = proof_round(ws, st, ws->rblk, sel_grid, n_rows, nullptr);
        span_end(ws, st);
        if (e != hipSuccess) return fail(GMMVB_EHIP, "proof round (settled rows' own pairs)", e);
    }
    span_begin(ws, kSpanSelect, st);
    int rc = sweep_bounds(proof, own_round);
    if (rc) return rc;
    if (proof && can_project && !projected) {
        note_hip(ws, hipMemsetAsync(ws->exit_ctr + 2, 0, sizeof(unsigned long long), st));
        e = launch_proj_filter(sel_grid, st, project_args(ws, n_rows, ws->lock, ws->rmask, 0, 0));
        if (e != hipSuccess) return fail(GMMVB_EHIP, "proj_filter launch", e);
        filtered = true;
    }
    if (proof) {
        scan_and_fill(ws, st, ws->rmask, ws->rblk, sel_grid, n_rows, ws->K, projected ? nullptr : ws->ppart);
        span_end(ws, st);
        span_begin(ws, kSpanProof, st);
        e = proof_round(ws, st, ws->rblk, sel_grid, n_rows, ws->ub32);
        span_end(ws, st);
        if (e != hipSuccess) return fail(GMMVB_EHIP, "proof round", e);
        span_begin(ws, kSpanSelect, st);
        hipLaunchKernelGGL(rec_proof_decide_kernel, dim3(sel_grid), dim3(kSelRows), 0, st, rec, ws->rmask, ws->masks, ws->npad,
                           n_rows, ws->K, ws->cvec, ws->ub32, ws->lnrho, ws->lcomp, ws->dlock, ws->rthr, ws->blk, ws->epart,
                           ws->ppart, own_round ? ws->spart : nullptr, quiet_swept ? ws->tile_loose() : nullptr);
        proof_ran = true;
    }
    span_end(ws, st);
    return GMMVB_OK;
}

int Pass::run_sweep_from_best() {
    span_begin(ws, kSpanSelect, st);
    hipLaunchKernelGGL(select_mask_kernel<3>, dim3(sel_grid), dim3(kSelRows), 0, st, ws->lnrho, ws->npad, n_rows, ws->K, ws->khat,
                       ws->masks, ws->blk);
    span_end(ws, st);
    hipError_t e = lists_and_gather(ws, a, is64, vec, sel_grid, st);
    if (e != hipSuccess) return fail(GMMVB_EHIP, "E-step best-component evaluation", e);
    span_begin(ws, kSpanSelect, st);
    hipLaunchKernelGGL(rec_sweep_kernel<false>, dim3(sel_grid), dim3(kSelRows), 0, st, ws->ub32, ws->lnrho, ws->npad, n_rows, ws->K,
                       ws->drift, ws->cvec, ws->khat, rec, ws->masks, ws->blk, ws->epart, ws->opart,
                       settle ? ws->lock : nullptr, ws->dlock, ws->rthr, ws->lcomp, nullptr, nullptr, 0, 0, nullptr, 0);
    span_end(ws, st);
    return GMMVB_OK;
}

int Pass::run_sweep() {
    rpw = kSelRows;
    grid = sel_grid;
    name = "estep_sweep_bounds";
    ++ws->passes[4];
    ++ws->sweeps;
    const int rc = prev_lists ? run_sweep_over_lists() : run_sweep_from_best();
    if (rc) return rc;
    ws->sweep_prev = prev_lists;
    return GMMVB_OK;
}

int Pass::run_candidates() {
    hipError_t e = lists_and_gather(ws, a, is64, vec, sel_grid, st, ws->gather_exit ? ws->rthr : nullptr, ws->epart);
    if (e != hipSuccess) return fail(GMMVB_EHIP, "E-step candidate evaluation", e);
    span_begin(ws, kSpanLse, st);
    hipLaunchKernelGGL(rec_finish_kernel, dim3(sel_grid), dim3(kSelRows), 0, st, rec, ws->lnrho, ws->npad, n_rows, ws->K,
                       ws->cvec, ws->lse, ws->khat, ws->masks, ws->blk, ws->apart, ws->mpart, ws->ub32,
                       settle ? ws->lock : nullptr, ws->dlock, skip_margin, settle ? ws->dmask : nullptr,
                       settle ? ws->dblk : nullptr, ws->mmask, ws->mblk, ws->spart, ws->gpart, ws->qpart, ws->rthr, ws->lcomp,
                       quiet_swept ? ws->tile_loose() : nullptr, quiet_swept ? ws->tile_quiet() : nullptr, quiet_was_valid ? 1 : 0,
                       (quiet_swept && ws->opt_debug) ? ws->exit_ctr + 3 : nullptr);
    if (!proof_ran) note_hip(ws, hipMemsetAsync(ws->ctr + 7, 0, sizeof(double), st));
    hipLaunchKernelGGL(sum_parts_kernel, dim3(proof_ran ? 8 : 7), dim3(1024), 0, st, ws->apart, ws->epart, ws->opart, ws->mpart,
                       ws->spart, ws->gpart, ws->qpart, ws->ppart, sel_grid, ws->ctr);
    e = hipGetLastError();
    span_end(ws, st);
    if (e != hipSuccess) return fail(GMMVB_EHIP, "rec_finish launch", e);
    counted = true;
    ws->rec_valid = true;
    ws->rec_live = true;
    ws->evaluated = -1.0;
    ws->quiet_valid = quiet_swept;
    if (settle) {
        ws->lock_live = true;
        ws->delta_pending = true;
    }
    return GMMVB_OK;
}

int Pass::finish(const char* latch_what) {
    ws->tmeta_valid = tmeta_kept;
    ws->pend_lazy = tmeta_kept;
    ws->pend_proj = projected || filtered;
    ws->pend_quiet = quiet_swept && ws->opt_debug;
    if (!phase_closed && phase_events(ws)) {
        note_hip(ws, hipEventRecord(ws->ev[1], st));
        ws->ev_e = true;
    }
    if (counted) {
        hipError_t e = hipMemcpyAsync(ws->ctr_host, ws->ctr, 8 * sizeof(double), hipMemcpyDeviceToHost, st);
        if (e == hipSuccess && ws->exit_ctr && mode != kPassDense)
            e = hipMemcpyAsync(ws->exit_host, ws->exit_ctr, 4 * sizeof(unsigned long long), hipMemcpyDeviceToHost, st);
        if (e == hipSuccess) e = hipEventRecord(ws->ctr_ev, st);
        if (e != hipSuccess) return fail(GMMVB_EHIP, "E-step counters", e);
        ws->ctr_pending = true;
        ws->pend_mode = mode;
        ws->pend_rows = n_rows;
        ws->pend_first_sorted = sorted_now;
        ws->pend_round0 = (mode == kPassSweep && ws->sweep_prev && own_known) ? ws->lag.listed : (double)n_rows;
        ws->act_rows = n_rows;
    } else {
        ws->ctr_pending = false;
        ws->lag.valid = false;
        ws->act_rows = 0;
    }
    ws->exp_counted = counted;
    ws->pol.valid = false;
    ws->act_host = -1.0;
    ws->active_lists = false;
    ws->mlists_done = ws->mlists_lost = false;
    if (skip_margin >= 0.0) ws->skip_used = true;
    ws->blk_fresh = counted;
    ws->e_state = emission_to_hmm ? 4 : 1;
    ws->hmm_no_lnrho = emission_to_hmm;
    ws->lost_estep = false;
    ws->e_rows = n_rows;
    ws->params_used = true;
    ws->have_drift = false;
    ws->bounds_rows = n_rows;
    ws->bounds_x = x_dev;
    ws->bounds_ldx = ldx;
    ws->prev_pass = mode;
    ws->dense_valid = !projected;
    if (mode == kPassDense || mode == kPassBound) ws->sweeps = 0;
    if (name)
        std::snprintf(ws->info, sizeof(ws->info), "%s grid=%lldx%d rows/workgroup=%d", name, (long long)grid,
                      (i8 || mode != kPassDense) ? 512 : estep_threads(ws->estep_variant), rpw);
    return take_hip(ws, latch_what);
}

PassFacts Pass::facts() {
    PassFacts f;
    f.L = ws->sharded ? ws->pol : ws->lag;
    f.prune = ws->prune;
    f.xc_of_x = xc_is_of(ws, x_dev, ldx, n_rows);
    f.has_xc = ws->xc != nullptr;
    f.can_prune = ws->prune != 0 && ws->estep_variant == kEstepLds8 && ws->hmm == nullptr && ws->rec_k != nullptr && f.has_xc &&
                  f.xc_of_x;
    const int64_t size_rows = ws->sharded ? ws->shard_rows / ws->shard_ranks : n_rows;
    f.big = ws->prune == 2 || size_rows * (int64_t)ws->K >= (int64_t(1) << 23);
    f.same_rows = ws->bounds_rows == n_rows && ws->bounds_x == x_dev && ws->bounds_ldx == ldx;
    f.known = f.L.valid && (ws->sharded || (f.L.rows == (double)n_rows && !ws->ctr_pending));
    own_known = ws->lag.valid && ws->lag.rows == (double)n_rows && !ws->ctr_pending;
    f.after_estep = ws->e_state == 1 || ws->lost_estep;
    f.prev_lists = (ws->active_lists || ws->blk_fresh) && f.after_estep && ws->act_rows == n_rows && f.same_rows;
    f.xq_of_x = xq_is_of(ws, x_dev, ldx, n_rows);
    f.can_project = ws->proj_table && ws->gimg != nullptr && ws->sorted && ws->tile_ref_valid && f.prev_lists && f.xq_of_x &&
                    ws->xq_gen == ws->pivot_gen && ws->lock != nullptr;
    f.forget = ws->forget;
    f.have_drift = ws->have_drift;
    f.opt_carry_off = ws->opt_carry_off;
    f.dense_valid = ws->dense_valid;
    f.opt_project = ws->opt_project;
    f.typical_gamma = ws->typical_gamma;
    f.bound_fail_act = ws->bound_fail_act;
    f.bound_tb = ws->bound.tb;
    f.T = ws->T, f.K = ws->K, f.D = ws->D;
    f.n_rows = n_rows;
    f.sort_rows = ws->sort_rows, f.has_xp = ws->xp != nullptr, f.sorted = ws->sorted;
    f.sorts = ws->sorts;
    f.moved_since_sort = ws->moved_since_sort;
    f.hmm = ws->hmm != nullptr;
    f.has_lock = ws->lock != nullptr, f.lock_reset = ws->lock_reset, f.lock_live = ws->lock_live;
    f.delta_pending = ws->delta_pending, f.cache_on = ws->cache_on, f.sparse = ws->sparse, f.has_masks = ws->masks != nullptr;
    f.opt_proof = ws->opt_proof, f.has_bound_images = ws->img_i8b != nullptr, f.xq_current = ws->xq_gen == ws->img_gen;
    f.settle_margin = ws->settle_margin;
    prunable = f.can_prune && f.big;
    prev_lists = f.prev_lists;
    can_project = f.can_project;
    return f;
}

int Pass::apply(const PassFacts& f, const PassPlan& plan) {
    if (plan.spare_set) ws->spare_last = plan.spare_last;
    if (plan.fell_back) ++ws->passes[3];
    ws->bound_fail_act = plan.bound_fail_act;
    ws->forget = false;
    if (ws->lock) {
        if (plan.reset_cache) {
            hipError_t e = hipMemsetAsync(ws->lock, 0, (size_t)ws->npad, st);
            if (e == hipSuccess) e = hipMemsetAsync(ws->cache, 0, (size_t)gmmvb_stats_len(ws->K, ws->D) * sizeof(double), st);
            if (e != hipSuccess) return fail(GMMVB_EHIP, "resetting the cache of single-component rows", e);
            ws->lock_live = false;
            ws->skip_used = false;
            ws->quiet_valid = false;
        }
        ws->lock_reset = false;
        ws->delta_pending = false;
    }
    ws->settled_fresh = false;
    mode = plan.mode;
    settle = plan.settle;
    proof_capable = plan.proof_capable;
    skip_margin = plan.skip_margin;
    if (ws->opt_debug) {
        const gmmvb_pass_counters& L = f.L;
        const double rows_l = f.rows_l();
        std::fprintf(stderr, "[gmmvb] estep: mode=%d known=%d lag(mode=%d act=%.3g eval=%.3g over=%.3g settled=%.3g listed=%.3g) gamma=%.3f rec_valid=%d drift=%d settle=%d quiet=%.0f/%lld skipped=%.0f\n",
                     plan.mode, (int)f.known, L.mode, L.act / rows_l, L.eval / rows_l, L.over / rows_l, L.settled / rows_l,
                     L.listed / rows_l, ws->typical_gamma, (int)ws->rec_valid, (int)ws->have_drift, (int)plan.settle,
                     ws->lag.valid ? ws->lag_quiet : -1.0, (long long)((n_rows + kSelRows - 1) / kSelRows),
                     ws->lag.valid ? ws->lag_skipped : -1.0);
    }
    const bool wants_drift = gmmvb_wants_drift(ws, n_rows) != 0;
    ws->bound.choose(plan.mode, ws->img_i8b != nullptr, f.L, f.known, wants_drift && ws->have_drift, wants_drift, ws->pt, ws->T,
                     ws->D, ws->K);
    return GMMVB_OK;
}

}

extern "C" {

int gmmvb_estep(gmmvb_workspace* ws, const void* x_dev, int64_t ldx, int64_t n_rows, void* stream) {
    bool vec = false;
    int rc = check_x(ws, x_dev, ldx, n_rows, &vec);
    if (rc) return rc;
// ... 59 lines not shown
```

bayesml_amd/csrc/capi_internal.h:

```cpp
#pragma once
#include "workspace.h"

#include <cstdio>
#include <algorithm>
#include <cstdlib>
#include <cstring>
#include <new>
#include <string>
#include <type_traits>

#include "aux_kernels.h"
#include "generic.h"
#include "launch.h"
#include "records.h"

using namespace gmmvb;

#ifndef GMMVB_T1_SPLITS
#define GMMVB_T1_SPLITS 24
#endif

template <int W = 1, typename F>
static inline void dispatch_mask_words(int K, F&& f) {
    if constexpr (W < 4) {
        if ((K + 63) / 64 == W) return f(std::integral_constant<int, W>{});
        return dispatch_mask_words<W + 1>(K, f);
    } else {
        return f(std::integral_constant<int, 4>{});
    }
}

extern "C" {

enum { kSpanEstepMain = 0, kSpanSelect = 1, kSpanGather = 2, kSpanLse = 3, kSpanLists = 4, kSpanMstepMain = 5,
       kSpanReduce = 6, kSpanProof = 7, kSpanSlots = 8 };
static const char* const kSpanNames[kSpanSlots] = {"estep_main", "estep_select", "estep_gather", "estep_lse_mask",
                                                   "mstep_lists", "mstep_main", "mstep_reduce", "estep_proof"};
static inline void note_hip(gmmvb_workspace* ws, hipError_t e) {
    if (e != hipSuccess && ws->hip_err == hipSuccess) ws->hip_err = e;
}
static inline int take_hip(gmmvb_workspace* ws, const char* what) {
    if (ws->hip_err == hipSuccess) return GMMVB_OK;
    const hipError_t e = ws->hip_err;
    ws->hip_err = hipSuccess;
    return fail(GMMVB_EHIP, what, e);
}
static inline bool span_kept(const gmmvb_workspace* ws, int slot) {
    return !ws->prof_light || slot == kSpanEstepMain || slot == kSpanGather || slot == kSpanMstepMain;
}
static inline void span_begin(gmmvb_workspace* ws, int slot, hipStream_t st) {
    ws->span_open = false;
    if (!ws->prof || ws->n_spans >= gmmvb_workspace::kMaxSpans || !span_kept(ws, slot)) return;
    ws->span_slot[ws->n_spans] = slot;
    ws->span_open = true;
    note_hip(ws, hipEventRecord(ws->span_ev[2 * ws->n_spans], st));
}
static inline void span_end(gmmvb_workspace* ws, hipStream_t st) {
    if (!ws->span_open) return;
    ws->span_open = false;
    note_hip(ws, hipEventRecord(ws->span_ev[2 * ws->n_spans + 1], st));
    ++ws->n_spans;
}
static inline bool phase_events(const gmmvb_workspace* ws) { return ws->prof && !ws->prof_light; }
static inline void drop_settled_rows(gmmvb_workspace* ws) {
    ws->quiet_valid = false;
    if (ws->lock_live) {
        ws->lock_live = false;
        ws->lock_reset = true;
    }
}

static inline bool xc_is_of(const gmmvb_workspace* ws, const void* x_dev, int64_t ldx, int64_t n_rows) {
    return ws->xc_src == x_dev && ws->xc_rows == n_rows && ws->xc_ldx == ldx;
}
static inline bool xq_is_of(const gmmvb_workspace* ws, const void* x_dev, int64_t ldx, int64_t n_rows) {
    return ws->xq != nullptr && ws->xq_src == x_dev && ws->xq_rows == n_rows && ws->xq_ldx == ldx;
}
static inline void scan_and_fill(gmmvb_workspace* ws, hipStream_t st, const unsigned long long* masks, int* blk, int nblk,
                                 int64_t n_rows, int K, const double* block_total = nullptr, unsigned char* lock = nullptr,
                                 const unsigned char* lcomp = nullptr) {
    launch_scan_counts(st, blk, nblk, K, ws->counts, ws->scan_parts);
    hipLaunchKernelGGL(fill_lists_kernel, dim3(nblk), dim3(kSelRows), 0, st, masks, ws->npad, n_rows, K, blk, ws->lists, ws->npad,
                       lock, lcomp, block_total);
}
static inline ProjectArgs project_args(const gmmvb_workspace* ws, int64_t n_rows, unsigned char* lock, unsigned long long* pmask,
                                       int proof_all, int own_fresh) {
    return ProjectArgs{ws->xq, ws->xqe, ws->gimg, ws->gconst, ws->tile_ref, ws->lnrho, ws->npad, n_rows, ws->K, ws->D, ws->drift,
                       ws->cvec, ws->rec_k, ws->rec_d, ws->rec_B, ws->rec_exact, ws->rec_sel, ws->rec_flags, ws->masks, ws->blk,
                       ws->epart, ws->opart, lock, ws->dlock, ws->rthr, ws->lcomp, pmask, ws->rblk, proof_all, own_fresh,
                       ws->exit_ctr + 2};
}

static inline void yield_scratch(gmmvb_workspace* w) {
    w->quiet_valid = false;
    w->lost_estep = w->e_state == 1;
    w->e_state = 0;
    w->active_lists = false;
    if (w->mlists_done) w->mlists_lost = true;
    w->mlists_done = false;
    w->rec_live = false;
    w->settled_fresh = false;
    if (w->xc_src) w->xc_stale = true;
}
static inline void claim_scratch(gmmvb_workspace* ws) {
    gmmvb_scratch* s = ws->scratch;
    if (!s || s->owner == ws) return;
    if (s->owner) yield_scratch(s->owner);
    s->owner = ws;
}
int fetch_counters(gmmvb_workspace* ws);
void poll_counters(gmmvb_workspace* ws);
int take_policy(gmmvb_workspace* ws);
int check_x(const gmmvb_workspace* ws, const void* x_dev, int64_t ldx, int64_t n_rows, bool* vec);
hipError_t recenter_rows(gmmvb_workspace* ws, int64_t n_rows, hipStream_t st);
bool cal_wanted(gmmvb_workspace* ws, int what, double pairs);
void cal_mark(gmmvb_workspace* ws, int what, double pairs, hipStream_t st);
void cal_poll(gmmvb_workspace* ws);

}
```

bayesml_amd/csrc/capi_readout.hip:

```cpp
#include "capi_internal.h"

extern "C" {

static int refresh_settled(gmmvb_workspace* ws, hipStream_t st) {
    if (!ws->params_used) return fail(GMMVB_ESTATE, "the parameters changed after the E-step whose settled rows are read");
    const int64_t n_rows = ws->e_rows;
    const int sel_grid = (int)((n_rows + kSelRows - 1) / kSelRows);
    if (!ws->rmask || !ws->rblk) return fail(GMMVB_ESTATE, "the list buffers of the pruned E-step are not allocated");
    const int is64 = ws->x_dtype == GMMVB_F64;
    bool vec = false;
    int rc = check_x(ws, ws->bounds_x, ws->bounds_ldx, n_rows, &vec);
    if (rc) return rc;
    EstepArgs a{ws->bounds_x, ws->bounds_ldx, n_rows, ws->D, ws->img, ws->cvec, ws->K, ws->lnrho, ws->npad};
    if (ws->sorted) {
        a.x = ws->xp;
        a.ldx = ws->D;
        vec = ws->D % 16 == 0;
    }
    hipLaunchKernelGGL(settled_mask_kernel, dim3(sel_grid), dim3(kSelRows), 0, st, ws->lock, ws->masks, ws->lcomp, ws->npad, n_rows,
                       ws->K, ws->rmask, ws->rblk);
    scan_and_fill(ws, st, ws->rmask, ws->rblk, sel_grid, n_rows, ws->K);
    hipLaunchKernelGGL(gather_plan_kernel, dim3(1), dim3(64), 0, st, ws->counts, ws->K, estep_gather_rows_per_wg(ws->T, is64),
                       ws->plan);
    hipError_t e = launch_estep_gather_dev(ws->T, is64, vec, 2 * ws->num_cu, st, a, ws->lists, ws->npad, ws->counts, ws->plan);
    if (e != hipSuccess) return fail(GMMVB_EHIP, "settled-row evaluation", e);
    hipLaunchKernelGGL(settled_lse_kernel, dim3((unsigned)((n_rows + 255) / 256)), dim3(256), 0, st, ws->lock, ws->masks, ws->lcomp,
                       ws->lnrho, ws->npad, n_rows, ws->K, ws->lse);
    e = hipGetLastError();
    if (e != hipSuccess) return fail(GMMVB_EHIP, "settled-row read-out", e);
    ws->active_lists = false;
    if (ws->mlists_done) ws->mlists_lost = true;
    ws->mlists_done = false;
    ws->settled_fresh = true;
    return GMMVB_OK;
}

static int readout(gmmvb_workspace* ws, int64_t row0, int64_t n_rows, double* out, void* stream, int mode) {
    if (!ws || !out) return fail(GMMVB_EINVAL, "null argument");
    if (ws->e_state == 0 || ws->e_state == 4) return fail(GMMVB_ESTATE, "no E-step output in the workspace");
    if (row0 < 0 || n_rows < 1 || row0 + n_rows > ws->e_rows) return fail(GMMVB_EINVAL, "row range outside the last E-step");
    if (mode == 0 && ws->e_state == 2) return fail(GMMVB_ESTATE, "ln rho is undefined after gmmvb_load_responsibilities");
    if (mode == 0 && ws->e_state == 3 && ws->hmm_no_lnrho)
        return fail(GMMVB_ESTATE, "the last gmmvb_estep formed no ln rho array (hmmvb_emission_target 1)");
    const int64_t total = n_rows * ws->K;
    const bool hmm_gamma = ws->e_state == 3 && mode == 1;
    if (ws->e_state == 1 && ws->rec_live) {
        if (ws->lock_live && ws->skip_used && !ws->settled_fresh) {
            const int rc = refresh_settled(ws, (hipStream_t)stream);
            if (rc) return rc;
        }
        const RecArrays rec{ws->rec_k, ws->rec_d, ws->rec_B, ws->rec_exact, ws->rec_sel, ws->rec_flags, ws->npad};
        hipLaunchKernelGGL(rec_readout_kernel, dim3((unsigned)((total + 255) / 256)), dim3(256), 0, (hipStream_t)stream, rec,
                           ws->masks, ws->lnrho, ws->lse, ws->cvec, ws->npad, row0, n_rows, ws->K, mode, out,
                           ws->sorted ? ws->iperm : nullptr, ws->lock_live ? ws->lock : nullptr, ws->lcomp);
        hipError_t er = hipGetLastError();
        if (er != hipSuccess) return fail(GMMVB_EHIP, "rec_readout launch", er);
        return GMMVB_OK;
    }
    if (ws->lse_stale && mode == 1 && ws->e_state == 1) {
        hipLaunchKernelGGL(row_lse_kernel, dim3((unsigned)((ws->e_rows + kLseRows - 1) / kLseRows)), dim3(256), 0,
                           (hipStream_t)stream, ws->lnrho, ws->npad, ws->e_rows, ws->K, ws->lse, nullptr, nullptr, 1);
        ws->lse_stale = false;
    }
    if (hmm_gamma && hmm_ensure_gamma_cm(ws->hmm, (hipStream_t)stream) != hipSuccess) return fail(GMMVB_EHIP, "gamma transpose launch");
    hipLaunchKernelGGL(readout_kernel, dim3((unsigned)((total + 255) / 256)), dim3(256), 0, (hipStream_t)stream,
                       hmm_gamma ? hmm_gamma_cm(ws->hmm) : ws->lnrho, ws->lse, ws->npad, row0, n_rows, ws->K, mode,
                       (ws->e_state == 2 || hmm_gamma) ? 1 : 0, out, ws->sorted ? ws->iperm : nullptr);
    hipError_t e = hipGetLastError();
    if (e != hipSuccess) return fail(GMMVB_EHIP, "readout launch", e);
    return GMMVB_OK;
}

int gmmvb_responsibilities(gmmvb_workspace* ws, int64_t row0, int64_t n_rows, double* r_dev, void* stream) {
    return readout(ws, row0, n_rows, r_dev, stream, 1);
}

int gmmvb_ln_rho(gmmvb_workspace* ws, int64_t row0, int64_t n_rows, double* out_dev, void* stream) {
    return readout(ws, row0, n_rows, out_dev, stream, 0);
}

int gmmvb_argmax(gmmvb_workspace* ws, int64_t row0, int64_t n_rows, int32_t* z_dev, void* stream) {
    if (!ws || !z_dev) return fail(GMMVB_EINVAL, "null argument");
    if (ws->e_state == 0 || ws->e_state == 4) return fail(GMMVB_ESTATE, "no E-step output in the workspace");
    if (row0 < 0 || n_rows < 1 || row0 + n_rows > ws->e_rows) return fail(GMMVB_EINVAL, "row range outside the last E-step");
    hipError_t e;
    const int* iperm = ws->sorted ? ws->iperm : nullptr;
    if (ws->e_state == 1 && ws->rec_live) {
        hipLaunchKernelGGL(gather_int_kernel, dim3((unsigned)((n_rows + 255) / 256)), dim3(256), 0, (hipStream_t)stream,
                           ws->khat, row0, n_rows, iperm, z_dev);
        e = hipGetLastError();
        if (e != hipSuccess) return fail(GMMVB_EHIP, "argmax read-out", e);
        return GMMVB_OK;
    }
    if (ws->e_state == 3 && hmm_ensure_gamma_cm(ws->hmm, (hipStream_t)stream) != hipSuccess) return fail(GMMVB_EHIP, "gamma transpose launch");
    hipLaunchKernelGGL(argmax_kernel, dim3((unsigned)((n_rows + 255) / 256)), dim3(256), 0, (hipStream_t)stream,
                       ws->e_state == 3 ? hmm_gamma_cm(ws->hmm) : ws->lnrho, ws->npad, row0, n_rows, ws->K, z_dev, iperm);
    e = hipGetLastError();
    if (e != hipSuccess) return fail(GMMVB_EHIP, "argmax launch", e);
    return GMMVB_OK;
}

}
```

bayesml_amd/csrc/records.h:

```cpp
#pragma once
#include <type_traits>
#include "aux_kernels.h"

namespace gmmvb {

__device__ __forceinline__ void rec_insert(float (&ds)[kRecSlots], unsigned short (&ks)[kRecSlots], float (&vs)[kRecSlots],
                                           float& rest, float cd, unsigned short ck, float cv) {
    if (!(cd < ds[kRecSlots - 1])) {
        if (ck != kRecEmpty && !(ck & kRecListed)) rest = (cv > rest || cv != cv) ? cv : rest;
        return;
    }
#pragma unroll
    for (int j = 0; j < kRecSlots; ++j) {
        const bool lt = cd < ds[j];
        const float td = lt ? ds[j] : cd, tv = lt ? vs[j] : cv;
        const unsigned short tk = lt ? ks[j] : ck;
        ds[j] = lt ? cd : ds[j];
        vs[j] = lt ? cv : vs[j];
        ks[j] = lt ? ck : ks[j];
        cd = td;
        cv = tv;
        ck = tk;
    }
    if (ck != kRecEmpty && !(ck & kRecListed)) rest = (cv > rest || cv != cv) ? cv : rest;
// ... 770 lines not shown
                        if (!((double)uf[q] < thr)) {
                            kept[w] |= 1ull << b[q];
                            any = true;
                        } else {
                            done_max = fmaxf(done_max, uf[q]);
                        }
                    }
                }
            }
            if (!any && l > -__builtin_huge_val()) {
                rec.flags[n] = 4;
                back = true;
                dlock[n] = f32_up(dist_of(cvec[kset], l) * (1.0 + 1e-9));
            } else {
                kept[kset >> 6] |= 1ull << (kset & 63);
                unsigned sel = 0;
                int in_slots = 0, total = 0;
#pragma unroll
                for (int j = 0; j < kRecSlots; ++j) {
                    const unsigned short k = rec.k[(int64_t)j * rec.npad + n];
                    if (k != kRecEmpty && ((kept[k >> 6] >> (k & 63)) & 1ull)) {
                        sel |= 1u << j;
                        ++in_slots;
                    }
                }
                for (int w = 0; w < W; ++w) {
                    mk[w] = kept[w];
                    total += __builtin_popcountll(kept[w]);
                    masks[(int64_t)w * npad + n] = kept[w];
                }
                rec.sel[n] = (unsigned char)sel;
                rec.exact[n] = 0;
                rec.flags[n] = (unsigned char)(total > in_slots ? 2 : 0);
                const float Bn = rec.B[n];
                if (done_max > Bn) rec.B[n] = done_max;
                rthr[n] = -__builtin_huge_valf();
            }
        }
        for (int w = 0; w < W; ++w) {
            mk[w] &= ~old[w];
            listed += __builtin_popcountll(mk[w]);
        }
    }
    for (int w = 0; w < W; ++w) count_word(mk[w], w, wave, wcnt);
    const int back_w = __builtin_popcountll(__builtin_amdgcn_ballot_w64(back));
#pragma unroll
    for (int o = 32; o > 0; o >>= 1) {
        listed += __shfl_xor(listed, o);
        proved += __shfl_xor(proved, o);
    }
    if ((tid & 63) == 0) {
        wsum[0][wave] = listed;
        wsum[1][wave] = proved;
        wsum[2][wave] = back_w;
    }
    __syncthreads();
    const int joined = wsum[0][0] + wsum[0][1] + wsum[0][2] + wsum[0][3];
    if (joined != 0)
        for (int k = tid; k < K; k += kSelRows) {
            const int c = wcnt[0][k] + wcnt[1][k] + wcnt[2][k] + wcnt[3][k];
            if (c != 0) blk_cnt[blk_at(k, blockIdx.x, K)] += c;
        }
    if (tid == 0) {
        if (joined != 0) epart[blockIdx.x] += (double)joined;
        ppart[blockIdx.x] = (double)(wsum[1][0] + wsum[1][1] + wsum[1][2] + wsum[1][3]) + (own_part ? own_part[blockIdx.x] : 0.0);
        const int returned = wsum[2][0] + wsum[2][1] + wsum[2][2] + wsum[2][3];
        if (tile_loose && returned != 0) tile_loose[blockIdx.x] -= returned;
    }
}

static __global__ __launch_bounds__(kSelRows) void rec_prune_kernel(RecArrays rec, unsigned long long* __restrict__ masks, int64_t npad,
                                                             int64_t n_rows, int K, const double* __restrict__ cvec,
                                                             const float* __restrict__ ub32, const float* __restrict__ rthr,
                                                             int* __restrict__ blk_cnt, double* __restrict__ epart,
                                                             double* __restrict__ ppart) {
    __shared__ int wcnt[4][256];
    __shared__ int wsum[2][4];
    const int tid = threadIdx.x, wave = tid >> 6;
    const int W = (K + 63) / 64;
    for (int k = tid & 63; k < K; k += 64) wcnt[wave][k] = 0;
    const int64_t n = (int64_t)blockIdx.x * kSelRows + tid;
    const bool valid = n < n_rows;
    unsigned long long mk[4] = {0ull, 0ull, 0ull, 0ull};
    int listed = 0, proved = 0;
    if (valid) {
        for (int w = 0; w < W; ++w) mk[w] = masks[(int64_t)w * npad + n];
        const unsigned fl = rec.flags[n];
        if (fl != 1u && (mk[0] | mk[1] | mk[2] | mk[3]) != 0ull) {
            const double thr = (double)rthr[n];
            unsigned long long inslot[4] = {0ull, 0ull, 0ull, 0ull};
            unsigned sel = rec.sel[n];
            float rest = rec.B[n];
            bool changed = false;
#pragma unroll
            for (int j = 0; j < kRecSlots; ++j) {
                const unsigned short k = rec.k[(int64_t)j * rec.npad + n];
                if (k == kRecEmpty) continue;
                inslot[k >> 6] |= 1ull << (k & 63);
                if (!((sel >> j) & 1u)) continue;
                const float u = ub32[(int64_t)k * npad + n];
                if ((double)u < thr) {
                    sel &= ~(1u << j);
                    mk[k >> 6] &= ~(1ull << (k & 63));
                    rec.d[(int64_t)j * rec.npad + n] = dist_lower_f32(cvec[k], (double)u);
                    changed = true;
                }
                ++proved;
            }
            int extra = 0;
            for (int w = 0; w < W; ++w) {
                unsigned long long m = mk[w] & ~inslot[w];
                while (m) {
                    const int b = __builtin_ctzll(m);
                    m &= m - 1;
                    const float u = ub32[(int64_t)(64 * w + b) * npad + n];
                    ++proved;
                    if ((double)u < thr) {
                        mk[w] &= ~(1ull << b);
                        rest = (u > rest) ? u : rest;
                        changed = true;
                    } else {
                        ++extra;
                    }
                }
            }
            if (changed) {
                for (int w = 0; w < W; ++w) masks[(int64_t)w * npad + n] = mk[w];
                rec.sel[n] = (unsigned char)sel;
                rec.B[n] = rest;
                rec.flags[n] = (unsigned char)(extra > 0 ? 2 : 0);
            }
        }
        for (int w = 0; w < W; ++w) listed += __builtin_popcountll(mk[w]);
    }
    for (int w = 0; w < W; ++w) count_word(mk[w], w, wave, wcnt);
#pragma unroll
    for (int o = 32; o > 0; o >>= 1) {
        listed += __shfl_xor(listed, o);
        proved += __shfl_xor(proved, o);
    }
    if ((tid & 63) == 0) {
        wsum[0][wave] = listed;
        wsum[1][wave] = proved;
    }
    __syncthreads();
    for (int k = tid; k < K; k += kSelRows)
        blk_cnt[blk_at(k, blockIdx.x, K)] = wcnt[0][k] + wcnt[1][k] + wcnt[2][k] + wcnt[3][k];
    if (tid == 0) {
        epart[blockIdx.x] = (double)(wsum[0][0] + wsum[0][1] + wsum[0][2] + wsum[0][3]);
        ppart[blockIdx.x] = (double)(wsum[1][0] + wsum[1][1] + wsum[1][2] + wsum[1][3]);
    }
}

static __global__ void gather_plan_kernel(const int* __restrict__ counts, int K, int per_wg, int* __restrict__ first) {
    __shared__ int sc[1025];
    if (blockIdx.x != 0) return;
    if (K > 1024) {
        if (threadIdx.x != 0) return;
        int total = 0;
        for (int k = 0; k < K; ++k) {
            first[k] = total;
            total += (counts[k] + per_wg - 1) / per_wg;
        }
        first[K] = total;
        return;
    }
    for (int k = threadIdx.x; k < K; k += blockDim.x) sc[k] = (counts[k] + per_wg - 1) / per_wg;
    __syncthreads();
    if (threadIdx.x == 0) {
        int total = 0;
        for (int k = 0; k < K; ++k) {
            const int c = sc[k];
            sc[k] = total;
            total += c;
        }
        sc[K] = total;
    }
    __syncthreads();
    for (int k = threadIdx.x; k <= K; k += blockDim.x) first[k] = sc[k];
}

static __global__ __launch_bounds__(kSelRows) void rec_finish_kernel(RecArrays rec, const double* __restrict__ lnrho, int64_t npad,
                                                              int64_t n_rows, int K, const double* __restrict__ cvec,
                                                              double* __restrict__ lse, int* __restrict__ khat,
                                                              unsigned long long* __restrict__ masks,
                                                              int* __restrict__ blk_cnt, double* __restrict__ apart,
                                                              double* __restrict__ mpart ,
                                                              float* __restrict__ ub32 ,
                                                              unsigned char* __restrict__ lock ,
                                                              float* __restrict__ dlock, double settle_margin ,
                                                              unsigned long long* __restrict__ dmask, int* __restrict__ dblk,
                                                              unsigned long long* __restrict__ mmask, int* __restrict__ mblk,
                                                              double* __restrict__ spart, double* __restrict__ gpart,
                                                              double* __restrict__ qpart ,
                                                              const float* __restrict__ rthr ,
                                                              unsigned char* __restrict__ lcomp ,
                                                              const int* __restrict__ tile_loose = nullptr ,
                                                              int* __restrict__ tile_quiet = nullptr ,
                                                              int quiet_valid = 0 ,
                                                              unsigned long long* __restrict__ quiet_ctr = nullptr ) {
    __shared__ int wcnt[4][256];
    __shared__ int dcnt[4][256];
    __shared__ int mcnt[4][256];
    __shared__ int wact[4], wmov[4], wset[4], wlist[4], wacc[4];
    const int tid = threadIdx.x, wave = tid >> 6;
    const int loose = tile_loose ? tile_loose[blockIdx.x] : -1;
    if (quiet_valid && loose == 0 && tile_quiet[blockIdx.x] == 1) {
        for (int k = tid; k < K; k += kSelRows) {
            blk_cnt[blk_at(k, blockIdx.x, K)] = 0;
            if (dblk) dblk[blk_at(k, blockIdx.x, K)] = mblk[blk_at(k, blockIdx.x, K)] = 0;
        }
        if (tid == 0) {
            const int64_t left = n_rows - (int64_t)blockIdx.x * kSelRows;
            const double rows = (double)(left < kSelRows ? left : (int64_t)kSelRows);
            apart[blockIdx.x] = spart[blockIdx.x] = rows;
            mpart[blockIdx.x] = gpart[blockIdx.x] = qpart[blockIdx.x] = 0.0;
            if (quiet_ctr) atomicAdd(quiet_ctr, 1ull << 32);
        }
        return;
    }
    const int W = (K + 63) / 64;
    for (int k = tid & 63; k < K; k += 64) wcnt[wave][k] = dcnt[wave][k] = mcnt[wave][k] = 0;
    const int64_t n = (int64_t)blockIdx.x * kSelRows + tid;
    const bool valid = n < n_rows;
    unsigned long long mk[4] = {0ull, 0ull, 0ull, 0ull};
    unsigned long long dm[4] = {0ull, 0ull, 0ull, 0ull};
    int active = 0, settled_i = 0;
    const int khat_before = valid ? khat[n] : 0;
    const unsigned fl = valid ? rec.flags[n] : 0u;
    double row_l = 0.0, row_best = 0.0, row_second = __builtin_huge_val();
    int row_arg = -1;
    const double thr_row = valid ? (double)rthr[n] : 0.0;
    if (valid && fl == 4u) {
        active = 1;
        settled_i = 1;
    } else if (valid && fl == 2u) {
        const unsigned live = (unsigned)rec.sel[n] | (unsigned)rec.exact[n];
        float ds[kRecSlots], vs[kRecSlots];
        unsigned short ks[kRecSlots];
#pragma unroll
        for (int j = 0; j < kRecSlots; ++j) {
            ds[j] = __builtin_huge_valf();
            vs[j] = -__builtin_huge_valf();
            ks[j] = kRecEmpty;
        }
        float rest = rec.B[n];
        unsigned long long cand[4] = {0ull, 0ull, 0ull, 0ull}, ev[4] = {0ull, 0ull, 0ull, 0ull};
        for (int w = 0; w < W; ++w) cand[w] = masks[(int64_t)w * npad + n];
        double mx = -__builtin_huge_val(), ssum = 0.0;
        int arg = 0x7fffffff;
        bool nan = false;
        auto take_exact = [&](int k) {
            const double x = lnrho[(int64_t)k * npad + n];
            ub32[(int64_t)k * npad + n] = f32_up(x);
            ev[k >> 6] |= 1ull << (k & 63);
            nan = nan || x != x;
            if (x > mx) {
                ssum = fma(ssum, exp(mx - x), 1.0);
                arg = k;
                mx = x;
            } else {
                if (x == mx && k < arg) arg = k;
                ssum += exp(x - mx);
            }
            rec_insert(ds, ks, vs, rest, f32_down(dist_of(cvec[k], x)),
                       (unsigned short)(k | (x < thr_row ? 0 : kRecExactBit)), f32_up(x));
        };
#pragma unroll
        for (int j = 0; j < kRecSlots; ++j) {
            const unsigned short k = rec.k[(int64_t)j * rec.npad + n];
            if (k == kRecEmpty) continue;
            cand[k >> 6] &= ~(1ull << (k & 63));
            if ((live >> j) & 1u) {
                take_exact(k);
            } else {
                const float d = rec.d[(int64_t)j * rec.npad + n];
                rec_insert(ds, ks, vs, rest, d, k, f32_up(cvec[k] - 0.5 * (double)d * (double)d));
            }
        }
        for (int w = 0; w < W; ++w) {
            unsigned long long m = cand[w];
            while (m) {
                const int b = __builtin_ctzll(m);
                m &= m - 1;
                take_exact(64 * w + b);
            }
        }
        double l = mx + log(ssum);
        if (nan) l = __builtin_nan("");
        lse[n] = l;
        khat[n] = arg == 0x7fffffff ? 0 : arg;
        unsigned ex = 0;
#pragma unroll
        for (int j = 0; j < kRecSlots; ++j) {
            const bool e1 = ks[j] != kRecEmpty && (ks[j] & kRecExactBit);
            rec.k[(int64_t)j * rec.npad + n] = ks[j] == kRecEmpty ? kRecEmpty : (unsigned short)(ks[j] & kRecCompMask);
            rec.d[(int64_t)j * rec.npad + n] = ds[j];
            ex |= e1 ? (1u << j) : 0u;
        }
        rec.B[n] = rest;
        rec.exact[n] = (unsigned char)ex;
        for (int w = 0; w < W; ++w) {
            unsigned long long m = ev[w];
            while (m) {
                const int b = __builtin_ctzll(m);
                m &= m - 1;
                const double t = lnrho[(int64_t)(64 * w + b) * npad + n] - l;
                if (!(t < -kRelNats)) {
                    mk[w] |= 1ull << b;
                    ++active;
                }
            }
        }
        if (!nan) {
            float sec = rest;
#pragma unroll
            for (int j = 0; j < kRecSlots; ++j)
                if (ks[j] != kRecEmpty && (int)(ks[j] & kRecCompMask) != arg) sec = (vs[j] > sec || vs[j] != vs[j]) ? vs[j] : sec;
            row_l = l;
            row_best = mx;
            row_arg = arg == 0x7fffffff ? -1 : arg;
            row_second = (double)sec;
        }
    } else if (valid && fl == 0u) {
        unsigned live = (unsigned)rec.sel[n] | (unsigned)rec.exact[n];
        unsigned bounds_only = 0;
        double v[kRecSlots];
        unsigned short kk[kRecSlots];
        double mx = -__builtin_huge_val();
        int arg = 0x7fffffff;
        bool nan = false;
#pragma unroll
// ... 34 lines not shown
                ++active;
            }
        }
        if (!nan) {
            row_l = l;
            row_best = mx;
            row_arg = arg == 0x7fffffff ? -1 : arg;
        }
        if (!nan && active == 1 && settle_margin >= 0.0 && lock != nullptr) {
            double sec = (double)rec.B[n];
#pragma unroll
            for (int j = 0; j < kRecSlots; ++j) {
                if (kk[j] == kRecEmpty || (int)kk[j] == arg) continue;
                double o = v[j];
                if (!((live >> j) & 1u)) {
                    const double d = (double)rec.d[(int64_t)j * rec.npad + n];
                    o = cvec[kk[j]] - 0.5 * d * d * (1.0 - 1e-6);
                }
                sec = (o > sec || o != o) ? o : sec;
            }
            row_second = sec;
        }
    } else if (valid) {
        float ds[kRecSlots], vs[kRecSlots];
        unsigned short ks[kRecSlots];
#pragma unroll
        for (int j = 0; j < kRecSlots; ++j) {
            ds[j] = __builtin_huge_valf();
            vs[j] = -__builtin_huge_valf();
            ks[j] = kRecEmpty;
        }
        float rest = -__builtin_huge_valf();
        double mx = lnrho[n], s = 1.0;
        int arg = 0;
        ub32[n] = f32_up(mx);
        rec_insert(ds, ks, vs, rest, f32_down(dist_of(cvec[0], mx)), 0, f32_up(mx));
        for (int k = 1; k < K; ++k) {
            const double x = lnrho[(int64_t)k * npad + n];
            ub32[(int64_t)k * npad + n] = f32_up(x);
            rec_insert(ds, ks, vs, rest, f32_down(dist_of(cvec[k], x)), (unsigned short)k, f32_up(x));
            if (x > mx) {
                s = fma(s, exp(mx - x), 1.0);
                mx = x;
                arg = k;
            } else {
                s += exp(x - mx);
            }
        }
        const double l = mx + log(s);
        lse[n] = l;
        khat[n] = arg;
        row_l = l;
        row_best = mx;
        row_arg = (l == l) ? arg : -1;
        unsigned ex = 0;
#pragma unroll
        for (int j = 0; j < kRecSlots; ++j) {
            rec.k[(int64_t)j * rec.npad + n] = ks[j];
            rec.d[(int64_t)j * rec.npad + n] = ds[j];
            ex |= (ks[j] != kRecEmpty) ? (1u << j) : 0u;
        }
        rec.B[n] = rest;
        rec.exact[n] = (unsigned char)ex;
        rec.sel[n] = (unsigned char)ex;
        for (int k = 0; k < K; ++k) {
            const double t = lnrho[(int64_t)k * npad + n] - l;
            if (!(t < -kRelNats)) {
                mk[k >> 6] |= 1ull << (k & 63);
                ++active;
            }
        }
    }
    unsigned long long mm[4] = {mk[0], mk[1], mk[2], mk[3]};
    int in_lists = 0, m_pairs = 0;
    if (valid && lock != nullptr && fl != 4u) {
        const unsigned lk = lock[n];
        const bool single = row_arg >= 0 && active == 1;
        if (lk == 1u) {
            const int was = lcomp[n];
            if (!(single && row_arg == was)) {
                dm[was >> 6] |= 1ull << (was & 63);
                if (single) dm[row_arg >> 6] |= 1ull << (row_arg & 63);
                lock[n] = single ? 4 : 2;
            }
        } else if (single) {
            dm[row_arg >> 6] |= 1ull << (row_arg & 63);
            lock[n] = 3;
        }
        if (single) {
            lcomp[n] = (unsigned char)row_arg;
            mm[row_arg >> 6] &= ~(1ull << (row_arg & 63));
            if (settle_margin >= 1e300 || (settle_margin >= 0.0 && row_second < row_l - kRelNats - settle_margin)) {
                dlock[n] = f32_up(dist_of(cvec[row_arg], row_best) * (1.0 + 1e-9));
                mk[row_arg >> 6] &= ~(1ull << (row_arg & 63));
            }
        }
    }
    if (valid) {
        for (int w = 0; w < W; ++w) {
            masks[(int64_t)w * npad + n] = mk[w];
            in_lists += __builtin_popcountll(mk[w]);
            m_pairs += __builtin_popcountll(mm[w]) + __builtin_popcountll(dm[w]);
            if (dmask) {
                dmask[(int64_t)w * npad + n] = dm[w];
                mmask[(int64_t)w * npad + n] = mm[w];
            }
        }
    }
    for (int w = 0; w < W; ++w) {
        count_word<false>(mk[w], w, wave, wcnt);
        if (dmask) {
            count_word<false>(dm[w], w, wave, dcnt);
            count_word<false>(mm[w], w, wave, mcnt);
        }
    }
    int moved = (valid && khat[n] != khat_before) ? 1 : 0;
#pragma unroll
    for (int o = 32; o > 0; o >>= 1) {
        active += __shfl_xor(active, o);
        moved += __shfl_xor(moved, o);
        settled_i += __shfl_xor(settled_i, o);
        in_lists += __shfl_xor(in_lists, o);
        m_pairs += __shfl_xor(m_pairs, o);
    }
    if ((tid & 63) == 0) {
        wact[wave] = active;
        wmov[wave] = moved;
        wset[wave] = settled_i;
        wlist[wave] = in_lists;
        wacc[wave] = m_pairs;
    }
    __syncthreads();
    for (int k = tid; k < K; k += kSelRows) {
        blk_cnt[blk_at(k, blockIdx.x, K)] = wcnt[0][k] + wcnt[1][k] + wcnt[2][k] + wcnt[3][k];
        if (dblk) {
            dblk[blk_at(k, blockIdx.x, K)] = dcnt[0][k] + dcnt[1][k] + dcnt[2][k] + dcnt[3][k];
            mblk[blk_at(k, blockIdx.x, K)] = mcnt[0][k] + mcnt[1][k] + mcnt[2][k] + mcnt[3][k];
        }
    }
    if (tid == 0) {
        apart[blockIdx.x] = (double)(wact[0] + wact[1] + wact[2] + wact[3]);
        mpart[blockIdx.x] = (double)(wmov[0] + wmov[1] + wmov[2] + wmov[3]);
        spart[blockIdx.x] = (double)(wset[0] + wset[1] + wset[2] + wset[3]);
        gpart[blockIdx.x] = (double)(wlist[0] + wlist[1] + wlist[2] + wlist[3]);
        qpart[blockIdx.x] = (double)(wacc[0] + wacc[1] + wacc[2] + wacc[3]);
        if (tile_quiet) tile_quiet[blockIdx.x] = loose == 0 ? 1 : 0;
    }
}

static __global__ __launch_bounds__(1024) void sum_parts_kernel(const double* __restrict__ apart, const double* __restrict__ epart,
                                                         const double* __restrict__ opart, const double* __restrict__ mpart,
                                                         const double* __restrict__ spart, const double* __restrict__ gpart,
                                                         const double* __restrict__ qpart, const double* __restrict__ ppart,
                                                         int blocks, double* __restrict__ ctr) {
    __shared__ double part[16];
    const double* src = blockIdx.x == 0 ? apart : (blockIdx.x == 1 ? epart : (blockIdx.x == 2 ? opart :
                        (blockIdx.x == 3 ? mpart : (blockIdx.x == 4 ? spart : (blockIdx.x == 5 ? gpart :
                        (blockIdx.x == 6 ? qpart : ppart))))));
    if (!src) return;
    double a = 0.0;
    for (int b = threadIdx.x; b < blocks; b += 1024) a += src[b];
#pragma unroll
    for (int o = 32; o > 0; o >>= 1) a += __shfl_xor(a, o);
    if ((threadIdx.x & 63) == 0) part[threadIdx.x >> 6] = a;
    __syncthreads();
    if (threadIdx.x == 0) {
        double t = 0.0;
        for (int i = 0; i < 16; ++i) t += part[i];
        ctr[blockIdx.x] = t;
    }
}

__device__ __forceinline__ bool row_settled(const unsigned char* __restrict__ lock,
                                            const unsigned long long* __restrict__ emask, int64_t npad, int W, int64_t n) {
    if (lock[n] != 1) return false;
    unsigned long long any = 0ull;
    for (int w = 0; w < W; ++w) any |= emask[(int64_t)w * npad + n];
    return any == 0ull;
}

static __global__ __launch_bounds__(kSelRows) void settled_mask_kernel(const unsigned char* __restrict__ lock,
                                                                const unsigned long long* __restrict__ emask,
                                                                const unsigned char* __restrict__ lcomp, int64_t npad, int64_t n_rows,
                                                                int K, unsigned long long* __restrict__ masks,
                                                                int* __restrict__ blk_cnt,
                                                                const double* __restrict__ drift = nullptr ,
                                                                double* __restrict__ listed_part = nullptr ,
                                                                const int* __restrict__ tile_quiet = nullptr ) {
    __shared__ int wcnt[4][256];
    const int64_t n = (int64_t)blockIdx.x * kSelRows + threadIdx.x;
    const bool valid = n < n_rows;
    const int W = (K + 63) / 64;
    const int wave = threadIdx.x >> 6;
    for (int k = threadIdx.x & 63; k < K; k += 64) wcnt[wave][k] = 0;
    const int64_t nn = valid ? n : 0;
    const int lc = (int)lcomp[nn];
    unsigned lk = 1u;
    unsigned long long any = 0ull;
    if (!(tile_quiet && tile_quiet[blockIdx.x] == 1)) {
        lk = lock[nn];
        for (int w = 0; w < W; ++w) any |= emask[(int64_t)w * npad + nn];
    }
    int kh = (valid && lk == 1u && any == 0ull) ? lc : -1;
    if (kh >= 0 && drift != nullptr && !own_first(drift[3 * K + kh], drift[K + kh])) kh = -1;
    for (int w = 0; w < W; ++w) {
        const unsigned long long mk = (kh >= 0 && (kh >> 6) == w) ? 1ull << (kh & 63) : 0ull;
        if (valid) masks[(int64_t)w * npad + n] = mk;
        count_word(mk, w, wave, wcnt);
    }
    __syncthreads();
    int tot = 0;
    for (int k = threadIdx.x; k < K; k += kSelRows) {
        const int c = wcnt[0][k] + wcnt[1][k] + wcnt[2][k] + wcnt[3][k];
        blk_cnt[blk_at(k, blockIdx.x, K)] = c;
        tot += c;
    }
    if (listed_part) {
        __shared__ int wtot[4];
#pragma unroll
        for (int o = 32; o > 0; o >>= 1) tot += __shfl_xor(tot, o);
        if ((threadIdx.x & 63) == 0) wtot[wave] = tot;
        __syncthreads();
        if (threadIdx.x == 0) listed_part[blockIdx.x] = (double)(wtot[0] + wtot[1] + wtot[2] + wtot[3]);
    }
}

static __global__ void settled_lse_kernel(const unsigned char* __restrict__ lock, const unsigned long long* __restrict__ emask,
                                   const unsigned char* __restrict__ lcomp, const double* __restrict__ lnrho, int64_t npad,
                                   int64_t n_rows, int K, double* __restrict__ lse) {
    const int64_t n = (int64_t)blockIdx.x * blockDim.x + threadIdx.x;
    if (n < n_rows && row_settled(lock, emask, npad, (K + 63) / 64, n)) lse[n] = lnrho[(int64_t)lcomp[n] * npad + n];
}

static __global__ void rec_readout_kernel(RecArrays rec, const unsigned long long* __restrict__ masks,
                                   const double* __restrict__ lnrho, const double* __restrict__ lse,
                                   const double* __restrict__ cvec, int64_t npad, int64_t row0, int64_t n_rows, int K,
                                   int mode, double* __restrict__ out, const int* __restrict__ iperm,
                                   const unsigned char* __restrict__ lock, const unsigned char* __restrict__ lcomp) {
    const int64_t e = (int64_t)blockIdx.x * blockDim.x + threadIdx.x;
    if (e >= n_rows * K) return;
    const int64_t n = iperm ? iperm[row0 + e / K] : row0 + e / K;
    const int k = (int)(e % K);
    bool exact = ((masks[(int64_t)(k >> 6) * npad + n] >> (k & 63)) & 1ull) != 0 || (rec.flags[n] & 1) != 0;
    if (lock && (lock[n] == 1 || lock[n] >= 3) && (int)lcomp[n] == k) exact = true;
    if (mode == 1) {
        out[e] = exact ? exp(lnrho[(int64_t)k * npad + n] - lse[n]) : 0.0;
        return;
    }
    const bool no_record = rec.flags[n] == 4;
    double ub = no_record ? __builtin_huge_val() : (double)rec.B[n];
    if (!exact && !no_record) {
        const unsigned live = rec.exact[n];
#pragma unroll
        for (int j = 0; j < kRecSlots; ++j) {
            if (rec.k[(int64_t)j * rec.npad + n] == k) {
                exact = (live >> j) & 1u;
                const double d = (double)rec.d[(int64_t)j * rec.npad + n];
                ub = cvec[k] - 0.5 * d * d;
            }
        }
    }
    if (!exact) {
        const double cap = lse[n] - kRelNats;
        ub = cap < ub ? cap : ub;
    }
    out[e] = exact ? lnrho[(int64_t)k * npad + n] : ub;
}

}
```

bayesml_amd/csrc/workspace_plan.h:

```cpp
#pragma once
#include <stdint.h>

#include <algorithm>
#include <cstdlib>
#include <cstring>
#include <type_traits>
#include <vector>

#include "../../include/gmmvb.h"

namespace gmmvb {

enum EstepVariant { kEstepLds = 0, kEstepDirect = 1, kEstepLds8 = 2, kEstepI8 = 3, kEstepValu16 = 4 };
inline int64_t round_up(int64_t v, int64_t m) { return (v + m - 1) / m * m; }

inline bool not_zero(const char* v) { return !(v && std::strcmp(v, "0") == 0); }
inline bool is(const char* v, const char* word) { return v && std::strcmp(v, word) == 0; }
template <typename Lookup>
inline const char* dev_switch(Lookup&& lookup, const char* name) {
    const char* on = lookup("GMMVB_DEBUG");
    return (on && on[0] != '\0' && on[0] != '0') ? lookup(name) : nullptr;
}

struct WorkspaceOptions {
    bool sparse = true;
    int prune = 1;
    int variant_asked = -1;
    bool sort_rows = true;
    double settle_margin = 1e300;
    bool opt_proof = true;
    bool opt_proof_all = true;
    bool opt_proof_blocked = true;
    bool opt_lazy = true;
    int opt_project = 0;
    bool opt_regroup_margin = true;
    bool gather_exit = true;
    bool cache_on = true;
    bool opt_carry_off = false;
    bool opt_hmm_mstep_dense = false;
    bool opt_calibrate = true;
    bool opt_quiet_tiles = true;
    bool opt_mlist_xc = false;
    int opt_mlist_runs = 0;
    int opt_sweep_run = 0;
    bool opt_debug = false;

    template <typename Lookup>
    static WorkspaceOptions read(Lookup&& lookup) {
        auto dev = [&lookup](const char* name) { return dev_switch(lookup, name); };
        WorkspaceOptions o;
        o.sparse = not_zero(lookup("GMMVB_MSTEP_SPARSE"));
        o.prune = is(lookup("GMMVB_ESTEP_PRUNE"), "0") ? 0 : (is(lookup("GMMVB_ESTEP_PRUNE"), "force") ? 2 : 1);
        const char* variant = dev("GMMVB_ESTEP_VARIANT");
        o.variant_asked = is(variant, "lds8") ? kEstepLds8 : is(variant, "direct") ? kEstepDirect : is(variant, "lds4") ? kEstepLds
                          : is(variant, "i8") ? kEstepI8 : -1;
        o.sort_rows = not_zero(dev("GMMVB_SORT_ROWS"));
        if (const char* v = dev("GMMVB_SETTLE_MARGIN")) o.settle_margin = std::atof(v);
        o.opt_proof = not_zero(dev("GMMVB_PROOF"));
        o.opt_proof_all = !is(dev("GMMVB_PROOF"), "settled");
        o.opt_proof_blocked = not_zero(dev("GMMVB_PROOF_BLOCKED"));
        o.opt_lazy = not_zero(dev("GMMVB_SWEEP_LAZY"));
        o.opt_project = is(dev("GMMVB_PROJECT"), "filter") ? 1 : (is(dev("GMMVB_PROJECT"), "only") ? 2 : 0);
        o.opt_regroup_margin = not_zero(dev("GMMVB_REGROUP_MARGIN"));
        o.gather_exit = not_zero(dev("GMMVB_GATHER_EXIT"));
        o.cache_on = not_zero(dev("GMMVB_MSTEP_CACHE"));
        o.opt_carry_off = dev("GMMVB_ESTEP_CARRY_OFF") != nullptr;
        o.opt_hmm_mstep_dense = dev("GMMVB_HMM_MSTEP_DENSE") != nullptr;
        o.opt_calibrate = not_zero(dev("GMMVB_POLICY_CALIBRATE"));
        o.opt_quiet_tiles = not_zero(dev("GMMVB_QUIET_TILES"));
        if (const char* v = dev("GMMVB_MLIST_XC")) o.opt_mlist_xc = v[0] == '1';
        if (const char* v = dev("GMMVB_MLIST_RUNS")) o.opt_mlist_runs = std::max(0, std::atoi(v));
        if (const char* v = dev("GMMVB_SWEEP_RUN")) o.opt_sweep_run = std::max(0, std::atoi(v));
        o.opt_debug = lookup("GMMVB_DEBUG") && lookup("GMMVB_DEBUG")[0] == '2';
        return o;
    }
};

constexpr int kSweepRunDefault = 2;
inline int sweep_run_length(int K, int asked) {
    if (K > 128) return 1;
    const int want = asked > 0 ? asked : kSweepRunDefault;
    return want >= 4 ? 4 : (want >= 2 ? 2 : 1);
}
template <typename F>
inline void dispatch_sweep_run(int run, F&& f) {
    if (run == 4) return f(std::integral_constant<int, 4>{});
    if (run == 2) return f(std::integral_constant<int, 2>{});
    return f(std::integral_constant<int, 1>{});
}

struct KernelSizes {
    int max_tiles = 0, t1_splits = 0, sel_rows = 0, lse_rows = 0, scan_parts = 0, rec_slots = 0;
    int mstep_components_per_wg = 0;
    int slab_len = 0, estep_image_doubles = 0, estep_tri_image_doubles = 0, estep_bound_blocks = 0;
    int estep_i8_image_bytes = 0, estep_i8_bound_image_bytes = 0;
    int64_t estep_i8_digit_row_bytes = 0, proj_image_len = 0, proj_const_len = 0;
    int generic_rows = 0;
};

inline bool wide_features(int D, int max_tiles) { return D > 16 * max_tiles && D <= 32 * max_tiles; }
inline int feature_tiles(int D, int max_tiles) {
    const int T = (D + 15) / 16;
    return wide_features(D, max_tiles) ? 2 * ((T + 1) / 2) : T;
}

struct WorkspaceShape : WorkspaceOptions {
    int K = 0, D = 0, x_dtype = 0, num_cu = 0, T = 0;
    int64_t max_rows = 0, npad = 0;
    bool wide = false;
    bool generic = false;
    int KG = 0, S_cap = 0, img_len = 0, estep_variant = 0, gen_S = 1, img_i8_len = 0, img_i8b_len = 0;
    int64_t split_rows = 0, xc_len = 0;
    bool has_lists = false;
};

inline WorkspaceShape make_shape(int K, int D, int x_dtype, int64_t max_rows, int num_cu, const WorkspaceOptions& opt,
                                 const KernelSizes& ks) {
    WorkspaceShape s;
    s.K = K;
    s.D = D;
    s.x_dtype = x_dtype;
    s.max_rows = max_rows;
    s.num_cu = num_cu;
    s.T = feature_tiles(D, ks.max_tiles);
    s.wide = wide_features(D, ks.max_tiles);
    s.generic = D > 32 * ks.max_tiles;
    s.npad = round_up(max_rows, 64);
    if (s.generic) {
        s.sparse = s.sort_rows = s.cache_on = false;
        s.prune = 0;
        s.gen_S = (int)std::min<int64_t>(64, std::max<int64_t>(1, max_rows / 16384));
        return s;
    }
    static_cast<WorkspaceOptions&>(s) = opt;
    s.KG = (K + ks.mstep_components_per_wg - 1) / ks.mstep_components_per_wg;
    s.S_cap = std::max(8, (int)round_up(((int64_t)(s.T == 1 ? ks.t1_splits : 4) * num_cu + s.KG - 1) / s.KG, 8));
    s.split_rows = round_up(std::max<int64_t>(64, (16 << 20) / (16 * s.T * 8)), 64);
    s.S_cap = (int)std::max<int64_t>(s.S_cap, round_up((max_rows + s.split_rows - 1) / s.split_rows, 8));
    s.img_len = ks.estep_image_doubles;
    s.estep_variant = s.T == 1 ? kEstepValu16 : kEstepLds8;
    if (!s.wide && opt.variant_asked >= 0) s.estep_variant = opt.variant_asked;
    if (max_rows > 2000000000 || s.wide || K == 1) s.sparse = false;
    if (max_rows > 2000000000) s.sort_rows = false;
    if (!s.sparse || ks.estep_bound_blocks == 0 || K > 256) s.prune = 0;
    s.xc_len = (K == 1 && !s.wide) ? 0 : (s.npad + 64) * 16 * (int64_t)s.T;
    s.has_lists = s.sparse && K <= 256;
    if (s.estep_variant == kEstepI8) s.img_i8_len = ks.estep_i8_image_bytes;
    if (s.prune != 0) s.img_i8b_len = ks.estep_i8_bound_image_bytes;
    return s;
}

#define GMMVB_WORKSPACE_BUFFERS(X)                                                                                             \
    X(tri) X(img_i8) X(img_i8b) X(pivot_i8) X(lnrho) X(lse) X(img) X(cvec) X(pivot) X(slabs) X(xc) X(dpart) X(thr) X(apart)     \
    X(ctr) X(drift) X(lists) X(khat) X(counts) X(plan) X(plan_m) X(blk) X(scan_parts) X(masks) X(lock) X(lcomp) X(dlock)       \
    X(rthr) X(exit_ctr) X(exit_host) X(dmask) X(dblk) X(mmask) X(rmask) X(rblk) X(mblk) X(cache) X(spart) X(gpart) X(qpart)    \
    X(epart) X(opart) X(mpart) X(ppart) X(xq) X(xqe) X(gimg) X(gconst) X(tile_ref) X(rec_k) X(rec_d) X(rec_B) X(rec_exact)    \
    X(rec_sel) X(rec_flags) X(ub32) X(tmeta) X(xp) X(perm) X(iperm) X(perm_tmp) X(gen_u) X(gen_m) X(gen_first) X(gen_second)  \
    X(ctr_host)
#define GMMVB_X(name) kBuf_##name,
enum BufferId { GMMVB_WORKSPACE_BUFFERS(GMMVB_X) kBufCount };
#undef GMMVB_X
#define GMMVB_X(name) #name,
inline const char* buffer_name(int id) {
    static const char* const names[kBufCount] = {GMMVB_WORKSPACE_BUFFERS(GMMVB_X)};
    return names[id];
}
#undef GMMVB_X

enum : unsigned {
    kZeroed = 1,
    kZeroedLast = 8,
    kPinned = 2,
    kScratch = 4,
};
struct BufferSpec {
    int id;
    int64_t bytes;
    unsigned flags;
    int code;
    const char* what;
    bool counted() const { return (flags & kPinned) == 0; }
};

struct BufferPlan : std::vector<BufferSpec> {
    int code = GMMVB_ENOMEM;
    const char* what = "";
    void group(int c, const char* w) { code = c, what = w; }
    void add(int id, int64_t bytes, unsigned flags = 0) {
        if (bytes > 0) push_back(BufferSpec{id, bytes, flags, code, what});
    }
    int64_t counted_bytes() const {
        int64_t sum = 0;
        for (const BufferSpec& b : *this) sum += b.counted() ? b.bytes : 0;
        return sum;
    }
};

inline BufferPlan buffer_plan(const WorkspaceShape& s, const KernelSizes& ks, int64_t group_npad = 0) {
    const int64_t K = s.K, D = s.D, np = s.npad, f64 = 8, i32 = 4;
    BufferPlan p;
    if (s.generic) {
        p.group(GMMVB_ENOMEM, "hipMalloc (workspace)");
        p.add(kBuf_lnrho, K * np * f64, kScratch);
        p.add(kBuf_lse, np * f64);
        p.add(kBuf_cvec, K * f64);
        p.add(kBuf_pivot, D * f64, kZeroedLast);
        p.add(kBuf_gen_u, K * D * D * f64);
        p.add(kBuf_gen_m, K * D * f64);
        p.add(kBuf_gen_first, s.gen_S * K * (D + 2) * f64);
        p.add(kBuf_gen_second, s.gen_S * K * (s.T * (s.T + 1) / 2) * 256 * f64);
        p.add(kBuf_ctr, 8 * f64, kZeroedLast);
        p.group(GMMVB_EHIP, "workspace initialisation");
        p.add(kBuf_ctr_host, 8 * f64, kPinned);
        return p;
    }
    const int64_t blocks = (np + ks.sel_rows - 1) / ks.sel_rows, words = (K + 63) / 64;
    p.group(GMMVB_ENOMEM, "hipMalloc (packed triangular images)");
    if (s.estep_variant == kEstepValu16) p.add(kBuf_tri, K * ks.estep_tri_image_doubles * f64);
    p.group(GMMVB_ENOMEM, "hipMalloc (int8 images)");
    p.add(kBuf_img_i8, K * s.img_i8_len);
    p.add(kBuf_img_i8b, K * s.img_i8b_len);
    if (s.img_i8_len || s.img_i8b_len) p.add(kBuf_pivot_i8, D * f64);
    p.group(GMMVB_ENOMEM, "hipMalloc (workspace)");
    p.add(kBuf_lnrho, K * np * f64, kScratch);
    p.add(kBuf_lse, np * f64);
    p.add(kBuf_img, K * s.img_len * f64);
    p.add(kBuf_cvec, K * f64);
    p.add(kBuf_pivot, D * f64, kZeroedLast);
    p.add(kBuf_slabs, s.S_cap * K * ks.slab_len * f64, kScratch);
    p.add(kBuf_xc, s.xc_len * f64, kScratch);
    p.add(kBuf_dpart, (np + ks.lse_rows - 1) / ks.lse_rows * K * f64);
    p.add(kBuf_thr, K * f64);
    p.add(kBuf_apart, blocks * f64);
    p.add(kBuf_ctr, 8 * f64, kZeroedLast);
    p.add(kBuf_drift, 4 * K * f64);
    if (s.has_lists) {
        p.group(GMMVB_ENOMEM, "hipMalloc (sample lists / records)");
        p.add(kBuf_lists, K * (group_npad ? group_npad : np) * i32, kScratch);
        p.add(kBuf_khat, np * i32);
        p.add(kBuf_counts, K * i32);
        p.add(kBuf_plan, (K + 1) * i32);
// ... 95 lines not shown
```

include/gmmvb.h:

```cpp
#ifndef GMMVB_H
#define GMMVB_H

#include <stdint.h>

#ifdef __cplusplus
extern "C" {
#endif

#define GMMVB_ABI_VERSION 8

enum gmmvb_status {
    GMMVB_OK = 0,
    GMMVB_EINVAL = 1,
    GMMVB_EUNSUPPORTED = 2,
    GMMVB_EHIP = 3,
    GMMVB_ENOMEM = 4,
    GMMVB_ESTATE = 5
};

enum gmmvb_dtype { GMMVB_F32 = 0, GMMVB_F64 = 1 };

typedef struct gmmvb_workspace gmmvb_workspace;

int gmmvb_abi_version(void);
const char* gmmvb_last_error(void);

int64_t gmmvb_stats_len(int K, int D);

int gmmvb_workspace_create(int K, int D, int x_dtype, int64_t max_rows, gmmvb_workspace** out);
int gmmvb_workspace_destroy(gmmvb_workspace* ws);
int64_t gmmvb_workspace_bytes(const gmmvb_workspace* ws);

int gmmvb_workspace_create_tile(gmmvb_workspace* first, int64_t max_rows, gmmvb_workspace** out);

int gmmvb_set_pivot(gmmvb_workspace* ws, const double* pivot_dev , void* stream);

int gmmvb_prepare_rows(gmmvb_workspace* ws, const void* x_dev, int64_t ldx, int64_t n_rows, void* stream);

int gmmvb_set_params(gmmvb_workspace* ws, const double* c_dev , const double* m_dev ,
                     const double* u_dev , void* stream);

int gmmvb_estep(gmmvb_workspace* ws, const void* x_dev, int64_t ldx, int64_t n_rows, void* stream);

int gmmvb_load_responsibilities(gmmvb_workspace* ws, const double* r_dev, int64_t n_rows, void* stream);

int gmmvb_mstep(gmmvb_workspace* ws, const void* x_dev, int64_t ldx, int64_t n_rows, double* stats_dev,
                void* stream);

int gmmvb_estep_mstep(gmmvb_workspace* ws, const void* x_dev, int64_t ldx, int64_t n_rows,
                      double* stats_dev, void* stream);

int gmmvb_responsibilities(gmmvb_workspace* ws, int64_t row0, int64_t n_rows, double* r_dev, void* stream);
int gmmvb_ln_rho(gmmvb_workspace* ws, int64_t row0, int64_t n_rows, double* out_dev, void* stream);
int gmmvb_argmax(gmmvb_workspace* ws, int64_t row0, int64_t n_rows, int32_t* z_dev, void* stream);

typedef struct gmmvb_comm gmmvb_comm;
int gmmvb_comm_unique_id(unsigned char* id_out );
int gmmvb_comm_create(const unsigned char* id , int n_ranks, int rank, gmmvb_comm** out);
int gmmvb_comm_destroy(gmmvb_comm* comm);
int gmmvb_allreduce_stats(gmmvb_comm* comm, double* stats_dev, int64_t len, void* stream);

int64_t gmmvb_stats_packed_len(int K, int D);
int gmmvb_stats_pack(int K, int D, const double* stats_dev, double* packed_dev, void* stream);
int gmmvb_stats_unpack(int K, int D, const double* packed_dev, double* stats_dev, void* stream);

#define GMMVB_POLICY_LEN 16
int gmmvb_set_shard(gmmvb_workspace* ws, int64_t global_rows, int n_ranks);
int gmmvb_policy_export(gmmvb_workspace* ws, double* out_dev , void* stream);
int gmmvb_policy_import(gmmvb_workspace* ws, const double* summed_dev , void* stream);

int gmmvb_small_supported(int K, int D, int64_t n_rows);
int64_t gmmvb_small_out_len(int K, int D, int max_itr);
int gmmvb_small_fit(int K, int D, int x_dtype, const void* x_dev, int64_t ldx, int64_t n_rows, const double* pivot_dev ,
                    const double* prior_dev, int n_restarts, int init_type, const double* init_dev, int max_itr,
                    double tolerance, double* out_dev, double* r_dev, void* stream);

int64_t hmmvb_out_len(int K);
int hmmvb_enable(gmmvb_workspace* ws);
int hmmvb_forward_backward(gmmvb_workspace* ws, int64_t n_rows, const double* pi_tilde_dev, const double* a_tilde_dev,
                           double* out_dev, void* stream);
int hmmvb_last_boundary_pass(gmmvb_workspace* ws);
int hmmvb_last_viterbi_pass(gmmvb_workspace* ws);

int hmmvb_skip_h(gmmvb_workspace* ws, int skip);

int hmmvb_emission_target(gmmvb_workspace* ws, int fused, int* in_effect);

int hmmvb_viterbi(gmmvb_workspace* ws, int64_t n_rows, const double* ln_pi_tilde_dev, const double* ln_a_tilde_dev,
                  int32_t* z_dev, void* stream);

int hmmvb_readout(gmmvb_workspace* ws, int what, int64_t row0, int64_t n_rows, const double* a_tilde_dev, double* out_dev,
                  void* stream);

int hmmvb_debug_readout(gmmvb_workspace* ws, int what, int64_t row0, int64_t n_rows, double* out_dev, void* stream);

int gmmvb_profile_enable(gmmvb_workspace* ws, int on);
int gmmvb_profile_last_ms(gmmvb_workspace* ws, float* estep_ms, float* mstep_ms);

int gmmvb_profile_spans(gmmvb_workspace* ws, float* ms , int* launches );
const char* gmmvb_profile_span_name(int slot);

const char* gmmvb_last_launch_info(const gmmvb_workspace* ws);

int gmmvb_kside_factor(int K, int D, const double* w_inv_dev , double* g_dev ,
                       double* g_inv_dev , double* logdet_dev , void* stream);

int gmmvb_kside_drift(int K, int D, const double* u_old_dev, const double* uinv_old_dev, const double* m_old_dev,
                      const double* u_new_dev, const double* uinv_new_dev, const double* m_new_dev, int squarings,
                      int squarings_big, double* gamma_dev , double* delta_dev ,
                      double* big_gamma_dev , double* enorm_dev , void* stream);

typedef struct gmmvb_prior_view {
    const double *alpha, *m, *kappa, *nu, *w_inv, *ln_b_w_nu;
    double ln_c_alpha;
} gmmvb_prior_view;
typedef struct gmmvb_post_view {
    double *alpha, *m, *kappa, *nu, *w_inv, *w, *u, *u_inv;
    double *e_ln_pi, *e_ln_lambda_det, *ln_b_w_nu, *c;
} gmmvb_post_view;
int gmmvb_kside_step(int K, int D, const gmmvb_prior_view* prior, const gmmvb_post_view* q, const gmmvb_post_view* q_next,
                     const double* stats_dev, const double* pivot_dev, double* s_prev_dev, double* ns_dev ,
                     double* x_bar_dev , double* s_dev , int want_drift, double* gamma_dev,
                     double* delta_dev, double* big_gamma_dev, double* scal_dev , double* scratch_dev ,
                     void* stream);

int hmmvb_kside_dirichlet(int K, const double* eta0_dev, const double* zeta0_dev, double ln_c_eta0, double ln_c_zeta0,
                          const double* eta_dev, const double* zeta_dev, const double* ln_pi_dev, const double* ln_a_dev,
                          const double* ln_c_zeta_dev, const double* fb_dev, const double* ns_dev, const double* scal_nw_dev,
                          const double* h_scale_dev, double* eta_next_dev, double* zeta_next_dev, double* ln_pi_next_dev,
                          double* pi_next_dev, double* ln_a_next_dev, double* a_next_dev, double* ln_c_zeta_next_dev,
                          double* scal_dev, void* stream);

int gmmvb_pass_counts(const gmmvb_workspace* ws, int64_t* out );

int gmmvb_set_drift(gmmvb_workspace* ws, const double* gamma_dev , const double* delta_dev ,
                    const double* big_gamma_dev , double typical_gamma, void* stream);
int gmmvb_wants_drift(const gmmvb_workspace* ws, int64_t n_rows);
int gmmvb_forget(gmmvb_workspace* ws);

int64_t gmmvb_regroup_count(const gmmvb_workspace* ws);

int gmmvb_debug_record(gmmvb_workspace* ws, int64_t row, double* out );

int gmmvb_debug_proof(gmmvb_workspace* ws, int k, int64_t n_rows, float* ub_dev , double* lb_dev ,
                      void* stream);

int gmmvb_last_sparsity(gmmvb_workspace* ws, void* stream, double* active_pairs, double* evaluated_pairs);
int gmmvb_last_work(gmmvb_workspace* ws, double* out );

#define GMMVB_POLICY_TABLE_LEN 16
int gmmvb_policy_calibrate(gmmvb_workspace* ws, int on);
int gmmvb_policy_table(gmmvb_workspace* ws, double* out );

int gmmvb_sample_latent(int K, const double* cdf_dev , uint64_t seed, int64_t row0, int64_t n_rows,
                        int64_t* z_dev , void* stream);
int64_t gmmvb_sample_chain_work_bytes(int K, int64_t n_rows);
int gmmvb_sample_chain(int K, const double* cdf_pi_dev , const double* cdf_a_dev ,
                       uint64_t seed, int64_t n_rows, int64_t* z_dev , void* work_dev, int64_t work_bytes,
                       void* stream);
int64_t gmmvb_sample_emissions_work_bytes(int K, int64_t n_rows);
int gmmvb_sample_emissions(int K, int D, const int64_t* z_dev , const double* mu_dev ,
                           const double* a_dev , uint64_t seed, int64_t row0, int64_t n_rows, int x_dtype,
                           void* x_dev, int64_t ldx, void* work_dev, int64_t work_bytes, void* stream);

#ifdef __cplusplus
}
#endif
#endif
```

Baseline: 6.501 billion samples/s.

## Fuse scan-apply into list fill and fold gather plan into fill kernel

Restructures the per-component row-list construction. The separate scan_apply pass over per-tile counts is removed: scan_parts now sums fixed runs of 8 tiles, scan_mid handles arbitrary part counts in one block, and fill_lists processes 8 tiles per workgroup, carrying the running base in registers and optionally writing tile bases back. The gather-plan prefix and the counter zeroing are folded into block 0 of the fill kernel and the sum_parts kernel, which removes separate launches and a memset. In exchange, each fill workgroup does more serial work, and parts are stored in a reused workspace buffer guarded by a size check.

Measured after the change: 6.487 billion samples/s (median of 3 runs). About the same (-0.2%).

```diff
diff --git a/bayesml_amd/_engine.py b/bayesml_amd/_engine.py
--- a/bayesml_amd/_engine.py
+++ b/bayesml_amd/_engine.py
@@ -29,6 +29,7 @@
     "gmmvb_regroup_count": (_i64, [_vp]),
     "gmmvb_debug_record": (_int, [_vp, _i64, ctypes.POINTER(ctypes.c_double)]),
     "gmmvb_debug_proof": (_int, [_vp, _int, _i64, _vp, _vp, _vp]),
+    "gmmvb_debug_lists": (_int, [_vp, _int, _i64, _vp, _vp, _vp, _vp, _vp, _vp, _vp, _vp]),
     "gmmvb_wants_drift": (_int, [_vp, _i64]),
     "gmmvb_prepare_rows": (_int, [_vp, _vp, _i64, _i64, _vp]),
     "gmmvb_estep": (_int, [_vp, _vp, _i64, _i64, _vp]),
@@ -444,6 +445,18 @@
                                                         self._stream()), "gmmvb_debug_proof")
         return ub, lb
 
+    def debug_lists(self, K: int, masks, lock=None, lcomp=None, block_total=None):
+        n = int(masks.shape[1])
+        counts = torch.empty(K, dtype=torch.int32, device=self.device)
+        lists = torch.full((K, n), -1, dtype=torch.int32, device=self.device)
+        bases = torch.empty(((n + 255) // 256, K), dtype=torch.int32, device=self.device)
+        ptr = lambda t: None if t is None else t.data_ptr()
+        with torch.cuda.device(self.device):
+            _check(self.lib, self.lib.gmmvb_debug_lists(self._ws, int(K), n, masks.data_ptr(), ptr(lock), ptr(lcomp),
+                                                        ptr(block_total), counts.data_ptr(), lists.data_ptr(), bases.data_ptr(),
+                                                        self._stream()), "gmmvb_debug_lists")
+        return counts, lists, bases
+
     def forget(self):
         _check(self.lib, self.lib.gmmvb_forget(self._ws), "gmmvb_forget")
 
diff --git a/bayesml_amd/csrc/aux_kernels.h b/bayesml_amd/csrc/aux_kernels.h
--- a/bayesml_amd/csrc/aux_kernels.h
+++ b/bayesml_amd/csrc/aux_kernels.h
@@ -186,164 +186,168 @@
         blk_cnt[blk_at(k, blockIdx.x, K)] = wcnt[0][k] + wcnt[1][k] + wcnt[2][k] + wcnt[3][k];
 }
 
+template <int R>
+static __global__ __launch_bounds__(256) void scan_parts_kernel(const int* __restrict__ blk, int blocks, int K, int nparts,
+                                                                int* __restrict__ parts) {
+    const int64_t i = (int64_t)blockIdx.x * 256 + threadIdx.x;
+    if (i >= (int64_t)nparts * K) return;
+    const int p = (int)(i / K), k = (int)(i - (int64_t)p * K);
+    int s = 0;
+#pragma unroll
+    for (int j = 0; j < R; ++j) {
+        const int b = p * R + j;
+        s += b < blocks ? blk[blk_at(k, b, K)] : 0;
+    }
+    parts[i] = s;
+}
+
 constexpr int kScanParts = 1024;
-constexpr int kScanChunk = 32;
-
-static __global__ __launch_bounds__(256) void scan_parts_kernel(const int* __restrict__ blk, int blocks, int K, int* __restrict__ parts) {
-    __shared__ int sh[256];
-    const int p = blockIdx.x;
-    const int R = K <= 256 ? 256 / K : 1;
-    const int t = threadIdx.x, k = t % K, r = t / K;
-    const int per = (blocks + kScanParts - 1) / kScanParts;
-    const int b0 = p * per, b1 = b0 + per < blocks ? b0 + per : blocks;
-    int s = 0;
-    if (t < R * K)
-        for (int b = b0 + r; b < b1; b += R) s += blk[blk_at(k, b, K)];
-    sh[t] = s;
-    __syncthreads();
-    if (t < K) {
-        int tot = 0;
-        for (int q = 0; q < R; ++q) tot += sh[q * K + t];
-        parts[p * K + t] = tot;
-    }
-}
-
-static __global__ __launch_bounds__(256) void scan_mid_kernel(int* __restrict__ parts, int K, int* __restrict__ counts) {
-    static_assert(kScanParts == 32 * kScanChunk, "256 threads = 8 components x 32 chunks");
-    __shared__ int sh[32][8];
+constexpr int kScanChunk = 40;
+constexpr int kScanChunks = 128;
+static __global__ __launch_bounds__(8 * kScanChunks) void scan_mid_kernel(int* __restrict__ parts, int nparts, int K,
+                                                                          int* __restrict__ counts) {
+    __shared__ int sh[kScanChunks][8];
     const int t = threadIdx.x, kk = t & 7, c = t >> 3;
     const int k = blockIdx.x * 8 + kk;
-    int v[kScanChunk];
-    int s = 0;
-#pragma unroll
-    for (int i = 0; i < kScanChunk; ++i) {
-        v[i] = k < K ? parts[(int64_t)(c * kScanChunk + i) * K + k] : 0;
-        s += v[i];
-    }
-    sh[c][kk] = s;
+    int carry = 0;
+    for (int s0 = 0; s0 < nparts; s0 += kScanChunks * kScanChunk) {
+        const int p0 = s0 + c * kScanChunk;
+        int v[kScanChunk];
+        int s = 0;
+#pragma unroll
+        for (int i = 0; i < kScanChunk; ++i) {
+            v[i] = (k < K && p0 + i < nparts) ? parts[(int64_t)(p0 + i) * K + k] : 0;
+            s += v[i];
+        }
+        __syncthreads();
+        sh[c][kk] = s;
+        __syncthreads();
+        int run = carry, all = carry;
+        for (int q = 0; q < kScanChunks; ++q) {
+            const int w = sh[q][kk];
+            run += q < c ? w : 0;
+            all += w;
+        }
+        carry = all;
+#pragma unroll
+        for (int i = 0; i < kScanChunk; ++i) {
+            if (k < K && p0 + i < nparts) parts[(int64_t)(p0 + i) * K + k] = run;
+            run += v[i];
+        }
+    }
+    if (k < K && c == 0) counts[k] = carry;
+}
+
+struct GatherPlan {
+    int per_wg = 0;
+    int* first = nullptr;
+    unsigned long long* zero0 = nullptr;
+    unsigned long long* zero1 = nullptr;
+};
+
+__device__ __forceinline__ void gather_plan_step(const int* __restrict__ counts, int K, const GatherPlan& gp, int* sc) {
+    for (int k = threadIdx.x; k < K; k += blockDim.x) sc[k] = (counts[k] + gp.per_wg - 1) / gp.per_wg;
     __syncthreads();
-    int run = 0;
-    for (int q = 0; q < c; ++q) run += sh[q][kk];
-    if (k < K) {
-#pragma unroll
-        for (int i = 0; i < kScanChunk; ++i) {
-            parts[(int64_t)(c * kScanChunk + i) * K + k] = run;
-            run += v[i];
-        }
-        if (c == 31) counts[k] = run;
-    }
-}
-
-static __global__ __launch_bounds__(256) void scan_apply_kernel(int* __restrict__ blk, int blocks, int K, const int* __restrict__ parts) {
-    __shared__ int sh[256];
-    const int p = blockIdx.x;
-    const int R = K <= 256 ? 256 / K : 1;
-    const int t = threadIdx.x, k = t % K, r = t / K;
-    const bool on = t < R * K;
-    const int per = (blocks + kScanParts - 1) / kScanParts;
-    const int b0 = p * per, b1 = b0 + per < blocks ? b0 + per : blocks;
-    int run = on ? parts[p * K + k] : 0;
-    if (R == 1) {
-        for (int c0 = b0; c0 < b1; c0 += 8) {
-            int v[8];
-#pragma unroll
-            for (int i = 0; i < 8; ++i) v[i] = (on && c0 + i < b1) ? blk[blk_at(k, c0 + i, K)] : 0;
-#pragma unroll
-            for (int i = 0; i < 8; ++i) {
-                if (on && c0 + i < b1) blk[blk_at(k, c0 + i, K)] = run;
-                run += v[i];
-            }
-        }
-        return;
-    }
-    for (int c0 = b0; c0 < b1; c0 += R) {
-        const int b = c0 + r;
-        const int v = (on && b < b1) ? blk[blk_at(k, b, K)] : 0;
-        __syncthreads();
-        sh[t] = v;
-        __syncthreads();
-        if (on) {
-            int before = 0, all = 0;
-            for (int q = 0; q < R; ++q) {
-                const int w = sh[q * K + k];
-                before += q < r ? w : 0;
-                all += w;
-            }
-            if (b < b1) blk[blk_at(k, b, K)] = run + before;
-            run += all;
-        }
-    }
-}
-
-inline void launch_scan_counts(hipStream_t st, int* blk, int blocks, int K, int* counts, int* parts ) {
-    hipLaunchKernelGGL(scan_parts_kernel, dim3(kScanParts), dim3(256), 0, st, blk, blocks, K, parts);
-    hipLaunchKernelGGL(scan_mid_kernel, dim3((K + 7) / 8), dim3(256), 0, st, parts, K, counts);
-    hipLaunchKernelGGL(scan_apply_kernel, dim3(kScanParts), dim3(256), 0, st, blk, blocks, K, parts);
-}
-
+    if (threadIdx.x == 0) {
+        int total = 0;
+        for (int k = 0; k < K; ++k) {
+            const int c = sc[k];
+            sc[k] = total;
+            total += c;
+        }
+        sc[K] = total;
+        if (gp.zero0) *gp.zero0 = 0ull;
+        if (gp.zero1) *gp.zero1 = 0ull;
+    }
+    __syncthreads();
+    for (int k = threadIdx.x; k <= K; k += blockDim.x) gp.first[k] = sc[k];
+    __syncthreads();
+}
+
+template <int R, int WC >
 static __global__ __launch_bounds__(kSelRows) void fill_lists_kernel(const unsigned long long* __restrict__ masks, int64_t npad,
-                                                              int64_t n_rows, int K, const int* __restrict__ blk_base,
-                                                              int* __restrict__ lists, int64_t cap,
-                                                              unsigned char* __restrict__ lock = nullptr,
-                                                              const unsigned char* __restrict__ lcomp = nullptr,
-                                                              const double* __restrict__ block_total = nullptr
-                                                              ) {
-    if (block_total != nullptr && block_total[blockIdx.x] == 0.0) return;
+                                                              int64_t n_rows, int K, int blocks, const int* __restrict__ parts,
+                                                              int* __restrict__ blk_out, int* __restrict__ lists, int64_t cap,
+                                                              unsigned char* __restrict__ lock, const unsigned char* __restrict__ lcomp,
+                                                              const double* __restrict__ block_total,
+                                                              const int* __restrict__ counts, GatherPlan gp) {
     __shared__ int wcnt[4][256];
-    const int64_t n = (int64_t)blockIdx.x * kSelRows + threadIdx.x;
-    const bool valid = n < n_rows;
-    const int W = (K + 63) / 64;
-    const int wave = threadIdx.x >> 6, lane = threadIdx.x & 63;
-    for (int k = lane; k < K; k += 64) wcnt[wave][k] = 0;
-    const int base_pre = (int)threadIdx.x < K ? blk_base[blk_at((int)threadIdx.x, blockIdx.x, K)] : 0;
-    unsigned long long mkw[4] = {0ull, 0ull, 0ull, 0ull}, prw[4] = {0ull, 0ull, 0ull, 0ull};
-#pragma unroll
-    for (int w = 0; w < 4; ++w) {
-        if (w >= W) break;
-        const unsigned long long mk = valid ? masks[(int64_t)w * npad + n] : 0ull;
-        mkw[w] = mk;
-        unsigned long long present = wave_or(mk);
-        prw[w] = present;
-        while (present) {
-            const int b = __builtin_ctzll(present);
-            present &= present - 1;
-            const int c = __builtin_popcountll(__ballot((mk >> b) & 1ull));
-            if (lane == 0) wcnt[wave][64 * w + b] = c;
-        }
-    }
-    __syncthreads();
-    for (int k = threadIdx.x; k < K; k += kSelRows) {
-        const int c0 = wcnt[0][k], c1 = wcnt[1][k], c2 = wcnt[2][k], c3 = wcnt[3][k];
-        if (c0 + c1 + c2 + c3 > 0) {
-            const int base = k == (int)threadIdx.x ? base_pre : blk_base[blk_at(k, blockIdx.x, K)];
-            wcnt[0][k] = base;
-            wcnt[1][k] = base + c0;
-            wcnt[2][k] = base + c0 + c1;
-            wcnt[3][k] = base + c0 + c1 + c2;
-        }
-    }
-    __syncthreads();
-    const unsigned lk0 = (lock && valid) ? lock[n] : 0u;
-    const int kh0 = (lock && valid) ? (int)lcomp[n] : 0;
-    if (lk0 >= 2u) lock[n] = lk0 == 2u ? 0 : 1;
-#pragma unroll
-    for (int w = 0; w < 4; ++w) {
-        if (w >= W) break;
-        const unsigned long long mk = mkw[w];
-        unsigned long long present = prw[w];
-        while (present) {
-            const int b = __builtin_ctzll(present);
-            present &= present - 1;
-            const int k = 64 * w + b;
-            const unsigned long long bal = __ballot((mk >> b) & 1ull);
-            const int off = wcnt[wave][k];
-            if ((mk >> b) & 1ull) {
-                int entry = (int)n;
-                if (lock) {
-                    const bool leaves = lk0 == 2u || (lk0 == 4u && kh0 != k);
-                    entry = leaves ? (int)((unsigned)entry | 0x80000000u) : entry;
+    if (gp.per_wg != 0 && blockIdx.x == 0) gather_plan_step(counts, K, gp, &wcnt[0][0]);
+    const int tid = threadIdx.x, wave = tid >> 6, lane = tid & 63;
+    const int b0 = blockIdx.x * R;
+    int base = tid < K ? parts[(int64_t)blockIdx.x * K + tid] : 0;
+    bool live[R];
+    bool any = false;
+#pragma unroll
+    for (int i = 0; i < R; ++i) {
+        live[i] = b0 + i < blocks && !(block_total != nullptr && block_total[b0 + i] == 0.0);
+        any = any || live[i];
+    }
+    if (!any && blk_out == nullptr) return;
+    unsigned long long mk[R][WC];
+    unsigned lk[R];
+    int kh[R];
+#pragma unroll
+    for (int i = 0; i < R; ++i) {
+        const int64_t n = (int64_t)(b0 + i) * kSelRows + tid;
+        const bool valid = live[i] && n < n_rows;
+#pragma unroll
+        for (int w = 0; w < WC; ++w) mk[i][w] = valid ? masks[(int64_t)w * npad + n] : 0ull;
+        lk[i] = (lock && valid) ? lock[n] : 0u;
+        kh[i] = (lock && valid) ? (int)lcomp[n] : 0;
+    }
+#pragma unroll
+    for (int i = 0; i < R; ++i) {
+        const int b = b0 + i;
+        if (b >= blocks) break;
+        if (!live[i]) {
+            if (blk_out && tid < K) blk_out[blk_at(tid, b, K)] = base;
+            continue;
+        }
+        for (int k = lane; k < K; k += 64) wcnt[wave][k] = 0;
+        unsigned long long prw[WC];
+#pragma unroll
+        for (int w = 0; w < WC; ++w) {
+            unsigned long long present = wave_or(mk[i][w]);
+            prw[w] = present;
+            while (present) {
+                const int bit = __builtin_ctzll(present);
+                present &= present - 1;
+                const int c = __builtin_popcountll(__ballot((mk[i][w] >> bit) & 1ull));
+                if (lane == 0) wcnt[wave][64 * w + bit] = c;
+            }
+        }
+        __syncthreads();
+        if (tid < K) {
+            const int c0 = wcnt[0][tid], c1 = wcnt[1][tid], c2 = wcnt[2][tid], c3 = wcnt[3][tid];
+            if (blk_out) blk_out[blk_at(tid, b, K)] = base;
+            wcnt[0][tid] = base;
+            wcnt[1][tid] = base + c0;
+            wcnt[2][tid] = base + c0 + c1;
+            wcnt[3][tid] = base + c0 + c1 + c2;
+            base += c0 + c1 + c2 + c3;
+        }
+        __syncthreads();
+        const int64_t n = (int64_t)b * kSelRows + tid;
+        if (lk[i] >= 2u) lock[n] = lk[i] == 2u ? 0 : 1;
+#pragma unroll
+        for (int w = 0; w < WC; ++w) {
+            const unsigned long long m = mk[i][w];
+            unsigned long long present = prw[w];
+            while (present) {
+                const int bit = __builtin_ctzll(present);
+                present &= present - 1;
+                const int k = 64 * w + bit;
+                const unsigned long long bal = __ballot((m >> bit) & 1ull);
+                const int off = wcnt[wave][k];
+                if ((m >> bit) & 1ull) {
+                    int entry = (int)n;
+                    if (lock) {
+                        const bool leaves = lk[i] == 2u || (lk[i] == 4u && kh[i] != k);
+                        entry = leaves ? (int)((unsigned)entry | 0x80000000u) : entry;
+                    }
+                    lists[(int64_t)k * cap + off + __builtin_popcountll(bal & ((1ull << lane) - 1ull))] = entry;
                 }
-                lists[(int64_t)k * cap + off + __builtin_popcountll(bal & ((1ull << lane) - 1ull))] = entry;
             }
         }
     }
diff --git a/bayesml_amd/csrc/capi.hip b/bayesml_amd/csrc/capi.hip
--- a/bayesml_amd/csrc/capi.hip
+++ b/bayesml_amd/csrc/capi.hip
@@ -329,7 +329,8 @@
     const unsigned grid = (unsigned)((std::max<int64_t>(n_rows, ws->K) + 255) / 256);
     hipLaunchKernelGGL(debug_all_rows_kernel, dim3(grid), dim3(256), 0, st, ws->lists + (int64_t)k * ws->npad, ws->counts, ws->K, k,
                        n_rows);
-    hipLaunchKernelGGL(gather_plan_kernel, dim3(1), dim3(64), 0, st, ws->counts, ws->K, estep_i8_pairs_per_chunk(), ws->plan);
+    hipLaunchKernelGGL(gather_plan_kernel, dim3(1), dim3(64), 0, st, ws->counts, ws->K,
+                       GatherPlan{estep_i8_pairs_per_chunk(), ws->plan});
     hipError_t e = launch_estep_i8_proof(ws->D, ws->num_cu, st, ws->xq, ws->xqe, ws->img_i8b, ws->cvec, ws->K, ws->lists, ws->npad,
                                          ws->counts, ws->plan, ws->ub32, ws->lnrho, ws->npad);
     if (e == hipSuccess) e = hipMemcpyAsync(ub_dev, ws->ub32 + (int64_t)k * ws->npad, (size_t)n_rows * sizeof(float),
@@ -344,6 +345,53 @@
     ws->active_lists = ws->blk_fresh = false;
     ws->lag.valid = false;
     return GMMVB_OK;
+}
+
+namespace {
+__global__ void debug_count_kernel(const unsigned long long* __restrict__ masks, int64_t npad, int64_t n_rows, int K,
+                                   int* __restrict__ blk) {
+    const int k = threadIdx.x;
+    if (k >= K) return;
+    const int64_t n0 = (int64_t)blockIdx.x * kSelRows;
+    int c = 0;
+    for (int64_t n = n0; n < n0 + kSelRows && n < n_rows; ++n) c += (int)((masks[(int64_t)(k >> 6) * npad + n] >> (k & 63)) & 1ull);
+    blk[blk_at(k, blockIdx.x, K)] = c;
+}
+}
+
+int gmmvb_debug_lists(gmmvb_workspace* ws, int K, int64_t n_rows, const unsigned long long* masks_dev, unsigned char* lock_dev,
+                      const unsigned char* lcomp_dev, const double* block_total_dev, int* counts_dev, int* lists_dev,
+                      int* bases_dev, void* stream) {
+    if (!ws || !masks_dev || !counts_dev || !lists_dev || !bases_dev || K < 1 || n_rows < 1 || (lock_dev != nullptr) != (lcomp_dev != nullptr))
+        return fail(GMMVB_EINVAL, "bad argument");
+    if (!ws->lists || !ws->rblk || !ws->rmask || K > ws->K || n_rows > ws->max_rows)
+        return fail(GMMVB_ESTATE, "gmmvb_debug_lists: no list buffers for this many components and rows");
+    claim_scratch(ws);
+    hipStream_t st = (hipStream_t)stream;
+    const int nblk = (int)((n_rows + kSelRows - 1) / kSelRows);
+    hipError_t e = hipMemcpy2DAsync(ws->rmask, (size_t)ws->npad * 8, masks_dev, (size_t)n_rows * 8, (size_t)n_rows * 8,
+                                    (size_t)((K + 63) / 64), hipMemcpyDeviceToDevice, st);
+    if (e != hipSuccess) return fail(GMMVB_EHIP, "list building (diagnostic): masks", e);
+    hipLaunchKernelGGL(debug_count_kernel, dim3(nblk), dim3(kSelRows), 0, st, ws->rmask, ws->npad, n_rows, K, ws->rblk);
+    scan_and_fill(ws, st, ws->rmask, ws->rblk, nblk, n_rows, K, block_total_dev, lock_dev, lcomp_dev, GatherPlan{}, true);
+    e = hipGetLastError();
+    if (e == hipSuccess) e = hipMemcpyAsync(counts_dev, ws->counts, (size_t)K * sizeof(int), hipMemcpyDeviceToDevice, st);
+    if (e == hipSuccess)
+        e = hipMemcpy2DAsync(lists_dev, (size_t)n_rows * sizeof(int), ws->lists, (size_t)ws->npad * sizeof(int),
+                             (size_t)n_rows * sizeof(int), (size_t)K, hipMemcpyDeviceToDevice, st);
+    if (e == hipSuccess)
+        e = hipMemcpyAsync(bases_dev, ws->rblk, (size_t)nblk * K * sizeof(int), hipMemcpyDeviceToDevice, st);
+    if (e != hipSuccess) return fail(GMMVB_EHIP, "list building (diagnostic)", e);
+    ws->tmeta_valid = false;
+    drop_settled_rows(ws);
+    ws->e_state = 0;
+    ws->lost_estep = false;
+    ws->bounds_rows = 0;
+    ws->rec_valid = ws->dense_valid = ws->rec_live = false;
+    ws->active_lists = ws->blk_fresh = false;
+    ws->mlists_done = ws->mlists_lost = false;
+    ws->lag.valid = false;
+    return take_hip(ws, "list building (diagnostic)");
 }
 
 int gmmvb_forget(gmmvb_workspace* ws) {
diff --git a/bayesml_amd/csrc/capi_estep.hip b/bayesml_amd/csrc/capi_estep.hip
--- a/bayesml_amd/csrc/capi_estep.hip
+++ b/bayesml_amd/csrc/capi_estep.hip
@@ -38,6 +38,7 @@
     int run_sweep_over_lists();
     int run_sweep_from_best();
     int sweep_bounds(bool proof, bool own_round);
+    bool sweep_is_lazy() const { return !(can_project && ws->opt_project == 2) && ws->tmeta != nullptr; }
     int run_candidates();
     int finish(const char* latch_what);
 };
@@ -132,14 +133,9 @@
 
 hipError_t lists_and_gather(gmmvb_workspace* ws, const EstepArgs& a, int is64, bool vec, int sel_grid, hipStream_t st,
                             const float* thr = nullptr, const double* block_total = nullptr ) {
-    if (thr) {
-        hipError_t em = hipMemsetAsync(ws->exit_ctr, 0, sizeof(unsigned long long), st);
-        if (em != hipSuccess) return em;
-    }
     span_begin(ws, kSpanSelect, st);
-    scan_and_fill(ws, st, ws->masks, ws->blk, sel_grid, a.n_rows, ws->K, block_total);
-    hipLaunchKernelGGL(gather_plan_kernel, dim3(1), dim3(64), 0, st, ws->counts, ws->K,
-                       estep_gather_rows_per_wg(ws->T, is64), ws->plan);
+    scan_and_fill(ws, st, ws->masks, ws->blk, sel_grid, a.n_rows, ws->K, block_total, nullptr, nullptr,
+                  GatherPlan{estep_gather_rows_per_wg(ws->T, is64), ws->plan, thr ? ws->exit_ctr : nullptr});
     hipError_t e = hipGetLastError();
     span_end(ws, st);
     if (e != hipSuccess) return e;
@@ -193,7 +189,8 @@
         estep_i8_proof_work_bytes(ws->K, n_rows) <= ws->scratch->bytes[kBuf_slabs])
         return launch_estep_i8_proof_blocked(ws->D, ws->num_cu, st, ws->xq, ws->xqe, ws->img_i8b, ws->cvec, ws->K, ws->lists,
                                              ws->npad, ws->counts, blk_base, sel_grid, ws->slabs, ub, ws->lnrho, ws->npad);
-    hipLaunchKernelGGL(gather_plan_kernel, dim3(1), dim3(64), 0, st, ws->counts, ws->K, estep_i8_pairs_per_chunk(), ws->plan);
+    hipLaunchKernelGGL(gather_plan_kernel, dim3(1), dim3(64), 0, st, ws->counts, ws->K,
+                       GatherPlan{estep_i8_pairs_per_chunk(), ws->plan});
     return launch_estep_i8_proof(ws->D, ws->num_cu, st, ws->xq, ws->xqe, ws->img_i8b, ws->cvec, ws->K, ws->lists, ws->npad,
                                  ws->counts, ws->plan, ub, ws->lnrho, ws->npad);
 }
@@ -306,7 +303,7 @@
     hipLaunchKernelGGL(rec_select_kernel, dim3(sel_grid), dim3(kSelRows), 0, st, rec, n_rows, ws->K, ws->cvec, ws->masks,
                        ws->npad, ws->blk, ws->epart, ws->opart, ws->rthr);
     if (proof_capable) {
-        scan_and_fill(ws, st, ws->masks, ws->blk, sel_grid, n_rows, ws->K, ws->epart);
+        scan_and_fill(ws, st, ws->masks, ws->blk, sel_grid, n_rows, ws->K, ws->epart, nullptr, nullptr, GatherPlan{}, true);
         span_end(ws, st);
         span_begin(ws, kSpanProof, st);
         e = proof_round(ws, st, ws->blk, sel_grid, n_rows, ws->ub32);
@@ -335,7 +332,6 @@
         name = "estep_sweep_projected";
         projected = true;
     } else if (ws->tmeta) {
-        note_hip(ws, hipMemsetAsync(ws->exit_ctr + 1, 0, sizeof(unsigned long long), st));
         const int run = sweep_run_length(ws->K, ws->opt_sweep_run);
         dispatch_mask_words(ws->K, [&](auto wc) {
             dispatch_sweep_run(run, [&](auto rr) {
@@ -360,10 +356,12 @@
 
 int Pass::run_sweep_over_lists() {
     span_begin(ws, kSpanSelect, st);
+    const GatherPlan gp{estep_gather_rows_per_wg(ws->T, is64), ws->plan, sweep_is_lazy() ? ws->exit_ctr + 1 : nullptr};
     if (!ws->active_lists)
-        scan_and_fill(ws, st, ws->masks, ws->blk, sel_grid, n_rows, ws->K, ws->prev_pass != 0 ? ws->gpart : nullptr);
-    hipLaunchKernelGGL(gather_plan_kernel, dim3(1), dim3(64), 0, st, ws->counts, ws->K, estep_gather_rows_per_wg(ws->T, is64),
-                       ws->plan);
+        scan_and_fill(ws, st, ws->masks, ws->blk, sel_grid, n_rows, ws->K, ws->prev_pass != 0 ? ws->gpart : nullptr, nullptr,
+                      nullptr, gp);
+    else
+        hipLaunchKernelGGL(gather_plan_kernel, dim3(1), dim3(64), 0, st, ws->counts, ws->K, gp);
     span_end(ws, st);
     span_begin(ws, kSpanGather, st);
     hipError_t e = launch_estep_gather_dev(ws->T, is64, vec, 2 * ws->num_cu, st, a, ws->lists, ws->npad, ws->counts, ws->plan);
@@ -376,7 +374,7 @@
         span_begin(ws, kSpanSelect, st);
         hipLaunchKernelGGL(settled_mask_kernel, dim3(sel_grid), dim3(kSelRows), 0, st, ws->lock, ws->masks, ws->lcomp, ws->npad,
                            n_rows, ws->K, ws->rmask, ws->rblk, ws->drift, ws->spart, quiet_was_valid ? ws->tile_quiet() : nullptr);
-        scan_and_fill(ws, st, ws->rmask, ws->rblk, sel_grid, n_rows, ws->K, ws->spart);
+        scan_and_fill(ws, st, ws->rmask, ws->rblk, sel_grid, n_rows, ws->K, ws->spart, nullptr, nullptr, GatherPlan{}, true);
         span_end(ws, st);
         span_begin(ws, kSpanProof, st);
         e = proof_round(ws, st, ws->rblk, sel_grid, n_rows, nullptr);
@@ -393,7 +391,8 @@
         filtered = true;
     }
     if (proof) {
-        scan_and_fill(ws, st, ws->rmask, ws->rblk, sel_grid, n_rows, ws->K, projected ? nullptr : ws->ppart);
+        scan_and_fill(ws, st, ws->rmask, ws->rblk, sel_grid, n_rows, ws->K, projected ? nullptr : ws->ppart, nullptr, nullptr,
+                      GatherPlan{}, true);
         span_end(ws, st);
         span_begin(ws, kSpanProof, st);
         e = proof_round(ws, st, ws->rblk, sel_grid, n_rows, ws->ub32);
@@ -446,9 +445,8 @@
                        settle ? ws->dblk : nullptr, ws->mmask, ws->mblk, ws->spart, ws->gpart, ws->qpart, ws->rthr, ws->lcomp,
                        quiet_swept ? ws->tile_loose() : nullptr, quiet_swept ? ws->tile_quiet() : nullptr, quiet_was_valid ? 1 : 0,
                        (quiet_swept && ws->opt_debug) ? ws->exit_ctr + 3 : nullptr);
-    if (!proof_ran) note_hip(ws, hipMemsetAsync(ws->ctr + 7, 0, sizeof(double), st));
-    hipLaunchKernelGGL(sum_parts_kernel, dim3(proof_ran ? 8 : 7), dim3(1024), 0, st, ws->apart, ws->epart, ws->opart, ws->mpart,
-                       ws->spart, ws->gpart, ws->qpart, ws->ppart, sel_grid, ws->ctr);
+    hipLaunchKernelGGL(sum_parts_kernel, dim3(8), dim3(1024), 0, st, ws->apart, ws->epart, ws->opart, ws->mpart, ws->spart,
+                       ws->gpart, ws->qpart, proof_ran ? ws->ppart : nullptr, sel_grid, ws->ctr, 1);
     e = hipGetLastError();
     span_end(ws, st);
     if (e != hipSuccess) return fail(GMMVB_EHIP, "rec_finish launch", e);
diff --git a/bayesml_amd/csrc/capi_internal.h b/bayesml_amd/csrc/capi_internal.h
--- a/bayesml_amd/csrc/capi_internal.h
+++ b/bayesml_amd/csrc/capi_internal.h
@@ -78,10 +78,21 @@
 }
 static inline void scan_and_fill(gmmvb_workspace* ws, hipStream_t st, const unsigned long long* masks, int* blk, int nblk,
                                  int64_t n_rows, int K, const double* block_total = nullptr, unsigned char* lock = nullptr,
-                                 const unsigned char* lcomp = nullptr) {
-    launch_scan_counts(st, blk, nblk, K, ws->counts, ws->scan_parts);
-    hipLaunchKernelGGL(fill_lists_kernel, dim3(nblk), dim3(kSelRows), 0, st, masks, ws->npad, n_rows, K, blk, ws->lists, ws->npad,
-                       lock, lcomp, block_total);
+                                 const unsigned char* lcomp = nullptr, const GatherPlan& gp = GatherPlan{}, bool bases_out = false) {
+    const FillRuns fr = fill_runs(nblk);
+    if (!fill_parts_fit(nblk, K, ws->npad, ws->K, kLseRows)) {
+        note_hip(ws, hipErrorInvalidValue);
+        return;
+    }
+    int* parts = reinterpret_cast<int*>(ws->dpart);
+    hipLaunchKernelGGL(scan_parts_kernel<kFillRun>, dim3((unsigned)(((int64_t)fr.parts * K + 255) / 256)), dim3(256), 0, st, blk,
+                       nblk, K, fr.parts, parts);
+    hipLaunchKernelGGL(scan_mid_kernel, dim3((K + 7) / 8), dim3(8 * kScanChunks), 0, st, parts, fr.parts, K, ws->counts);
+    dispatch_mask_words(K, [&](auto wc) {
+        hipLaunchKernelGGL((fill_lists_kernel<kFillRun, decltype(wc)::value>), dim3(fr.parts), dim3(kSelRows), 0, st, masks,
+                           ws->npad, n_rows, K, nblk, parts, bases_out ? blk : nullptr, ws->lists, ws->npad, lock, lcomp,
+                           block_total, ws->counts, gp);
+    });
 }
 static inline ProjectArgs project_args(const gmmvb_workspace* ws, int64_t n_rows, unsigned char* lock, unsigned long long* pmask,
                                        int proof_all, int own_fresh) {
diff --git a/bayesml_amd/csrc/capi_readout.hip b/bayesml_amd/csrc/capi_readout.hip
--- a/bayesml_amd/csrc/capi_readout.hip
+++ b/bayesml_amd/csrc/capi_readout.hip
@@ -19,9 +19,8 @@
     }
     hipLaunchKernelGGL(settled_mask_kernel, dim3(sel_grid), dim3(kSelRows), 0, st, ws->lock, ws->masks, ws->lcomp, ws->npad, n_rows,
                        ws->K, ws->rmask, ws->rblk);
-    scan_and_fill(ws, st, ws->rmask, ws->rblk, sel_grid, n_rows, ws->K);
-    hipLaunchKernelGGL(gather_plan_kernel, dim3(1), dim3(64), 0, st, ws->counts, ws->K, estep_gather_rows_per_wg(ws->T, is64),
-                       ws->plan);
+    scan_and_fill(ws, st, ws->rmask, ws->rblk, sel_grid, n_rows, ws->K, nullptr, nullptr, nullptr,
+                  GatherPlan{estep_gather_rows_per_wg(ws->T, is64), ws->plan});
     hipError_t e = launch_estep_gather_dev(ws->T, is64, vec, 2 * ws->num_cu, st, a, ws->lists, ws->npad, ws->counts, ws->plan);
     if (e != hipSuccess) return fail(GMMVB_EHIP, "settled-row evaluation", e);
     hipLaunchKernelGGL(settled_lse_kernel, dim3((unsigned)((n_rows + 255) / 256)), dim3(256), 0, st, ws->lock, ws->masks, ws->lcomp,
diff --git a/bayesml_amd/csrc/records.h b/bayesml_amd/csrc/records.h
--- a/bayesml_amd/csrc/records.h
+++ b/bayesml_amd/csrc/records.h
@@ -946,32 +946,22 @@
     }
 }
 
-static __global__ void gather_plan_kernel(const int* __restrict__ counts, int K, int per_wg, int* __restrict__ first) {
+static __global__ void gather_plan_kernel(const int* __restrict__ counts, int K, GatherPlan gp) {
     __shared__ int sc[1025];
     if (blockIdx.x != 0) return;
     if (K > 1024) {
         if (threadIdx.x != 0) return;
         int total = 0;
         for (int k = 0; k < K; ++k) {
-            first[k] = total;
-            total += (counts[k] + per_wg - 1) / per_wg;
-        }
-        first[K] = total;
+            gp.first[k] = total;
+            total += (counts[k] + gp.per_wg - 1) / gp.per_wg;
+        }
+        gp.first[K] = total;
+        if (gp.zero0) *gp.zero0 = 0ull;
+        if (gp.zero1) *gp.zero1 = 0ull;
         return;
     }
-    for (int k = threadIdx.x; k < K; k += blockDim.x) sc[k] = (counts[k] + per_wg - 1) / per_wg;
-    __syncthreads();
-    if (threadIdx.x == 0) {
-        int total = 0;
-        for (int k = 0; k < K; ++k) {
-            const int c = sc[k];
-            sc[k] = total;
-            total += c;
-        }
-        sc[K] = total;
-    }
-    __syncthreads();
-    for (int k = threadIdx.x; k <= K; k += blockDim.x) first[k] = sc[k];
+    gather_plan_step(counts, K, gp, sc);
 }
 
 static __global__ __launch_bounds__(kSelRows) void rec_finish_kernel(RecArrays rec, const double* __restrict__ lnrho, int64_t npad,
@@ -1312,12 +1302,15 @@
                                                          const double* __restrict__ opart, const double* __restrict__ mpart,
                                                          const double* __restrict__ spart, const double* __restrict__ gpart,
                                                          const double* __restrict__ qpart, const double* __restrict__ ppart,
-                                                         int blocks, double* __restrict__ ctr) {
+                                                         int blocks, double* __restrict__ ctr, int zero_null = 0) {
     __shared__ double part[16];
     const double* src = blockIdx.x == 0 ? apart : (blockIdx.x == 1 ? epart : (blockIdx.x == 2 ? opart :
                         (blockIdx.x == 3 ? mpart : (blockIdx.x == 4 ? spart : (blockIdx.x == 5 ? gpart :
                         (blockIdx.x == 6 ? qpart : ppart))))));
-    if (!src) return;
+    if (!src) {
+        if (zero_null && threadIdx.x == 0) ctr[blockIdx.x] = 0.0;
+        return;
+    }
     double a = 0.0;
     for (int b = threadIdx.x; b < blocks; b += 1024) a += src[b];
 #pragma unroll
diff --git a/bayesml_amd/csrc/workspace_plan.h b/bayesml_amd/csrc/workspace_plan.h
--- a/bayesml_amd/csrc/workspace_plan.h
+++ b/bayesml_amd/csrc/workspace_plan.h
@@ -87,6 +87,19 @@
     if (run == 4) return f(std::integral_constant<int, 4>{});
     if (run == 2) return f(std::integral_constant<int, 2>{});
     return f(std::integral_constant<int, 1>{});
+}
+
+#ifndef GMMVB_FILL_RUN
+#define GMMVB_FILL_RUN 8
+#endif
+constexpr int kFillRun = GMMVB_FILL_RUN;
+struct FillRuns {
+    int run;
+    int parts;
+};
+inline FillRuns fill_runs(int64_t tiles) { return FillRuns{kFillRun, (int)((tiles + kFillRun - 1) / kFillRun)}; }
+inline bool fill_parts_fit(int64_t tiles, int K_lists, int64_t npad, int K, int lse_rows) {
+    return (int64_t)fill_runs(tiles).parts * K_lists * 4 <= (npad + lse_rows - 1) / lse_rows * K * 8;
 }
 
 struct KernelSizes {
diff --git a/include/gmmvb.h b/include/gmmvb.h
--- a/include/gmmvb.h
+++ b/include/gmmvb.h
@@ -145,6 +145,10 @@
 int gmmvb_debug_proof(gmmvb_workspace* ws, int k, int64_t n_rows, float* ub_dev , double* lb_dev ,
                       void* stream);
 
+int gmmvb_debug_lists(gmmvb_workspace* ws, int K, int64_t n_rows, const unsigned long long* masks_dev, unsigned char* lock_dev,
+                      const unsigned char* lcomp_dev, const double* block_total_dev, int* counts_dev, int* lists_dev,
+                      int* bases_dev, void* stream);
+
 int gmmvb_last_sparsity(gmmvb_workspace* ws, void* stream, double* active_pairs, double* evaluated_pairs);
 int gmmvb_last_work(gmmvb_workspace* ws, double* out );
 
```
